# sThalham/PyraPose

Hardware: AMD Instinct MI355X
Metric: images/sec 640x480 fwd+bwd (train step: fwd + losses + bwd + clipnorm-Adam) (higher is better)
Workload: dtype bf16x3+f16c8

## Files before the change

include/pyrapose_hip.h:

```cpp
#ifndef PYRAPOSE_HIP_H
#define PYRAPOSE_HIP_H

#include <stddef.h>
#include <stdint.h>

#ifdef __cplusplus
extern "C" {
#endif

#define PP_OK 0
#define PP_ERR_ARG (-1)
#define PP_ERR_SHAPE (-2)
#define PP_ERR_ALIGN (-3)
#define PP_ERR_NOCTX (-4)
#define PP_ERR_UNSUPPORTED (-5)
#define PP_ERR_COMM (-6)

#define PP_MAX_SEG 5

typedef struct pp_ctx pp_ctx;

int pp_ctx_create(pp_ctx** out, int device, void* hip_stream);
void pp_ctx_destroy(pp_ctx* ctx);
int pp_ctx_set_stream(pp_ctx* ctx, void* hip_stream);
int pp_ctx_set_workspace(pp_ctx* ctx, void* device_buffer, size_t bytes);
int pp_row_block_list(pp_ctx* ctx, const float* x, int rows, int ld, int cols, unsigned char* flags, int* list);
int pp_row_block_list_planes(pp_ctx* ctx, const void* x_hi, const void* x_lo, int rows, int ld, int cols, unsigned char* flags, int* list);
int pp_row_block_list_planes_within(pp_ctx* ctx, const void* x_hi, const void* x_lo, int rows, int ld, int cols, const unsigned char* within,
                                    unsigned char* flags, int* list);
const char* pp_last_error_string(pp_ctx* ctx);
const char* pp_version(void);
int pp_device_info(pp_ctx* ctx, int* n_cu, char* name_host, int name_len);

typedef struct {
  int n_img;
  int n_seg;
  int h[PP_MAX_SEG];
  int w[PP_MAX_SEG];
} pp_rowspace;

typedef struct {
  pp_rowspace in;
  pp_rowspace out;
  int cin, cout;
  int kh, kw, stride;
  int pad_t, pad_l;
  int ld_x, ld_y, ld_w;
} pp_conv_desc;

int pp_conv2d_nhwc_fwd(pp_ctx* ctx, const pp_conv_desc* d, const float* x, const float* w,
                       const float* bias, const float* residual, int ld_res, int relu, float* y);

int pp_conv2d_nhwc_bwd_data(pp_ctx* ctx, const pp_conv_desc* d, const float* dy, const float* w,
                            const float* addend, int ld_add, const float* relu_src, int ld_rs, float* dx);

int pp_conv2d_nhwc_bwd_weight(pp_ctx* ctx, const pp_conv_desc* d, const float* x, const float* dy,
                              float* dw, float* dbias);

int pp_conv_split_weights_bf16x3(pp_ctx* ctx, const pp_conv_desc* d, const float* w, void* fwd_hi, void* fwd_lo,
                                 void* dgrad_hi, void* dgrad_lo);
typedef struct pp_split_job {
  const float* w;
  void* fwd_hi; void* fwd_lo; void* dg_hi; void* dg_lo;
  int taps, cin, cout, ld_w;
  int tile_begin, reserved;
} pp_split_job;
int pp_conv_split_weights_bf16x3_batch(pp_ctx* ctx, int n_jobs, const pp_split_job* jobs_dev, int total_tiles);
int pp_positive_row_blocks(pp_ctx* ctx, const pp_rowspace* rs, int A, int stride, const float* y_true, unsigned char* flags);
int pp_row_block_dilate(pp_ctx* ctx, const pp_conv_desc* d, const unsigned char* in_flags, unsigned char* out_flags);
int pp_split_planes_bf16x3(pp_ctx* ctx, size_t n, const float* src, void* hi, void* lo);
int pp_ctx_set_planes_format(pp_ctx* ctx, int fmt);
int pp_convert_planes(pp_ctx* ctx, size_t n, const void* src_hi, const void* src_lo, int src_fmt, void* dst_hi, void* dst_lo, int dst_fmt,
                      const float* scale2_dev, int scale_index, const void* relu_src_hi);
int pp_grad_scale_from_counts(pp_ctx* ctx, const int* counts_dev, int n_counts, float* scale2_dev);
int pp_grad_scale_from_counts_adj(pp_ctx* ctx, const int* counts_dev, int n_counts, float* scale2_dev, int log2_adjust);
int pp_split_planes_scaled_bf16x3(pp_ctx* ctx, size_t n, const float* src, void* hi, void* lo, const float* scale_dev);
int pp_ctx_set_grad_scale(pp_ctx* ctx, const float* scale2_dev);

typedef struct pp_conv_opts {
  void* capture_hi;
  void* capture_lo;
  const void* add_hi;
  const void* add_lo;
  const void* mask_hi;
  unsigned char* skip_flags;
  int* skip_list;
  const unsigned char* out_flags;
  int* out_list;
  int lazy_out;
  int lazy_in;
} pp_conv_opts;
#ifdef __cplusplus
static_assert(sizeof(pp_conv_opts) == 9 * sizeof(void*) + 2 * sizeof(int), "pp_conv_opts: pointers, then ints, no padding");
#else
_Static_assert(sizeof(pp_conv_opts) == 9 * sizeof(void*) + 2 * sizeof(int), "pp_conv_opts: pointers, then ints, no padding");
#endif

int pp_conv2d_nhwc_fwd_bf16x3(pp_ctx* ctx, const pp_conv_desc* d, const float* x, const void* x_hi, const void* x_lo,
                              const void* w_fwd_hi, const void* w_fwd_lo, const float* bias, const float* residual,
                              int ld_res, int relu, float* y, void* y_hi, void* y_lo, const pp_conv_opts* opts);
int pp_conv2d_nhwc_bwd_data_bf16x3(pp_ctx* ctx, const pp_conv_desc* d, const float* dy, const void* dy_hi,
                                   const void* dy_lo, const void* w_dgrad_hi, const void* w_dgrad_lo,
                                   const float* addend, int ld_add, const float* relu_src, int ld_rs, float* dx,
                                   void* dx_hi, void* dx_lo, const pp_conv_opts* opts);
int pp_conv2d_nhwc_bwd_weight_bf16x3(pp_ctx* ctx, const pp_conv_desc* d, const float* x, const float* dy,
                                     const void* x_hi, const void* x_lo, const void* dy_hi, const void* dy_lo,
                                     float* dw, float* dbias, const pp_conv_opts* opts);

typedef struct pp_comm pp_comm;
int pp_comm_available(void);
int pp_comm_unique_id(pp_ctx* ctx, void* id128);
int pp_comm_init(pp_ctx* ctx, int world, int rank, const void* id128, pp_comm** out);
int pp_comm_destroy(pp_comm* comm);
int pp_allreduce_bucket(pp_ctx* ctx, pp_comm* comm, float* buf, size_t count);
int pp_allreduce_counts(pp_ctx* ctx, pp_comm* comm, int* counts, int n);

int pp_maxpool3x3s2_fwd(pp_ctx* ctx, int n_img, int h, int w, int c, const float* x, int oh, int ow, float* y);
int pp_upsample_nearest_add_fwd(pp_ctx* ctx, int n_img, int sh, int sw, int th, int tw, int c,
                                const float* src, const float* other, float* out);
int pp_upsample_nearest_add_bwd(pp_ctx* ctx, int n_img, int sh, int sw, int th, int tw, int c,
                                const float* dtarget, const float* base, float* dsrc);
int pp_add_n(pp_ctx* ctx, size_t n, const float* a, const float* b, const float* c, float* out);
int pp_relu_fwd(pp_ctx* ctx, size_t n, const float* x, float* y);
typedef struct pp_tview {
  const float* f32;
  const void* hi;
  const void* lo;
} pp_tview;
int pp_add_n_v(pp_ctx* ctx, size_t n, const pp_tview* a, const pp_tview* b, const pp_tview* c, const pp_tview* out);
int pp_relu_fwd_v(pp_ctx* ctx, size_t n, const pp_tview* x, const pp_tview* y);
int pp_upsample_nearest_add_fwd_v(pp_ctx* ctx, int n_img, int sh, int sw, int th, int tw, int c, const pp_tview* src,
                                  const pp_tview* other, const pp_tview* out);
int pp_upsample_nearest_add_bwd_v(pp_ctx* ctx, int n_img, int sh, int sw, int th, int tw, int c, const pp_tview* dtarget,
                                  const pp_tview* base, const pp_tview* dsrc);
int pp_merge_planes_bf16x3(pp_ctx* ctx, size_t n, const void* hi, const void* lo, float* dst);
int pp_planes_stats(pp_ctx* ctx, const void* hi, const void* lo, long long rows, int ld, int cols, const unsigned char* within,
                    unsigned long long* stats5_dev);
int pp_pack_rgb_to_4(pp_ctx* ctx, size_t n_pixels, const float* x3, float* x4);
int pp_preprocess_caffe_u8(pp_ctx* ctx, int n_img, int H, int W, const int* sizes_hw_host, const unsigned char* images_u8,
                           float* x4);
int pp_warp_affine_u8(pp_ctx* ctx, int n_img, int H, int W, int channels, const double* mats_host, int interpolation, int border,
                      int cval, const unsigned char* src, unsigned char* dst);
int pp_resize_scale(int rows, int cols, int min_side, int max_side, double* scale);
int pp_resize_linear_u8(pp_ctx* ctx, int n_img, int SH, int SW, int channels, double scale, int DH, int DW, const unsigned char* src,
                        unsigned char* dst);
enum { PP_PHOTO_NONE = 0, PP_PHOTO_LUT = 1, PP_PHOTO_GRAY = 2, PP_PHOTO_HUESAT = 3, PP_PHOTO_BLEND = 4, PP_PHOTO_CONV = 5, PP_PHOTO_MEDIAN = 6,
       PP_PHOTO_BILATERAL = 7 };
typedef struct pp_photo_op {
  int kind;
  int k;
  int off0, off1;
  float f0, f1;
} pp_photo_op;
size_t pp_photo_workspace_bytes(int n_img, int H, int W);
int pp_photo_augment_u8(pp_ctx* ctx, int n_img, int H, int W, int channels, const int* op_offsets_host, const pp_photo_op* ops_host,
                        const unsigned char* pool_host, size_t pool_bytes, const unsigned char* pool_dev, const unsigned char* src,
                        unsigned char* dst, void* workspace, size_t workspace_bytes);
int pp_pack_rgb_to_4_padded(pp_ctx* ctx, int n_img, int H, int W, int Hp, int Wp, int pad, const float* x3, float* x4p);
int pp_preprocess_caffe_u8_padded(pp_ctx* ctx, int n_img, int H, int W, int Hp, int Wp, int pad, const int* sizes_hw_host,
                                  const unsigned char* images_u8, float* x4p);
int pp_stem7x7s2_fwd_bf16x3(pp_ctx* ctx, int n_img, int H, int W, int Hp, int Wp, const float* x4p, const void* w_hi,
                            const void* w_lo, int cout, const float* bias, int relu, float* y, int ld_y);

int pp_export_head(pp_ctx* ctx, const pp_rowspace* rs, int n_anchor, int n_val, const float* src, int ld,
                   int apply_sigmoid, float* out);

int pp_count_positives(pp_ctx* ctx, size_t rows_box, const float* y_box, size_t rows_cls, int c_cls,
                       const float* y_cls, size_t rows_mask, int c_mask, const float* y_mask, int* counts);
int pp_sigmoid_focal_fwd_bwd(pp_ctx* ctx, const pp_rowspace* rs, int n_anchor, int n_class,
                             const float* logits, int ld, const float* y_true, float alpha, float gamma,
                             const int* count, float loss_weight, float* loss_sum, float* dlogits);
int pp_orth_smoothl1_fwd_bwd(pp_ctx* ctx, const pp_rowspace* rs, int n_anchor, const float* pred, int ld,
                             const float* y_true, float weight, float sigma, const int* count,
                             float loss_weight, float* loss_sum, float* dpred);

typedef struct {
  long long offset;
  long long count;
// ... 118 lines not shown
```

pyrapose_amd/_lib.py:

```python
import ctypes as C
import os

_HERE = os.path.dirname(os.path.abspath(__file__))
LIB_PATH = os.path.join(_HERE, os.environ.get("PP_LIB") or "libpyrapose_hip.so")

PP_MAX_SEG = 5


class RowSpace(C.Structure):
    _fields_ = [("n_img", C.c_int), ("n_seg", C.c_int), ("h", C.c_int * PP_MAX_SEG), ("w", C.c_int * PP_MAX_SEG)]

    @classmethod
    def make(cls, n_img, shapes):
        rs = cls()
        rs.n_img = int(n_img)
        rs.n_seg = len(shapes)
        for i, (h, w) in enumerate(shapes):
            rs.h[i] = int(h)
            rs.w[i] = int(w)
        return rs

    def rows(self):
        return sum(self.n_img * self.h[i] * self.w[i] for i in range(self.n_seg))

    def shapes(self):
        return [(self.h[i], self.w[i]) for i in range(self.n_seg)]


class ConvDesc(C.Structure):
    _fields_ = [("in_", RowSpace), ("out", RowSpace), ("cin", C.c_int), ("cout", C.c_int), ("kh", C.c_int),
                ("kw", C.c_int), ("stride", C.c_int), ("pad_t", C.c_int), ("pad_l", C.c_int), ("ld_x", C.c_int),
                ("ld_y", C.c_int), ("ld_w", C.c_int)]


class ParamDesc(C.Structure):
    _fields_ = [("offset", C.c_longlong), ("count", C.c_longlong), ("ld", C.c_int), ("trainable", C.c_int),
                ("scale_off", C.c_longlong), ("l2", C.c_float)]


class SplitJob(C.Structure):
    _fields_ = [("w", C.c_void_p), ("fwd_hi", C.c_void_p), ("fwd_lo", C.c_void_p), ("dg_hi", C.c_void_p), ("dg_lo", C.c_void_p),
                ("taps", C.c_int), ("cin", C.c_int), ("cout", C.c_int), ("ld_w", C.c_int), ("tile_begin", C.c_int), ("reserved", C.c_int)]


class TView(C.Structure):
    _fields_ = [("f32", C.c_void_p), ("hi", C.c_void_p), ("lo", C.c_void_p)]


class ConvOpts(C.Structure):
    _fields_ = [("capture_hi", C.c_void_p), ("capture_lo", C.c_void_p), ("add_hi", C.c_void_p), ("add_lo", C.c_void_p),
                ("mask_hi", C.c_void_p), ("skip_flags", C.c_void_p), ("skip_list", C.c_void_p), ("out_flags", C.c_void_p),
                ("out_list", C.c_void_p), ("lazy_out", C.c_int), ("lazy_in", C.c_int)]


def _load():
    if not os.path.exists(LIB_PATH):
        raise ImportError(
            "pyrapose_amd: %s not found. Build it with `python -c 'import __graft_entry__ as g; g.build()'` "
            "or `make -C pyrapose_amd/csrc`. There is no CPU fallback." % LIB_PATH)
    try:
        return C.CDLL(LIB_PATH)
    except OSError as e:
        raise ImportError("pyrapose_amd: cannot load %s: %s" % (LIB_PATH, e))


lib = _load()
if hasattr(lib, "pp_ctx_set_split_capture"):
    raise ImportError("pyrapose_amd: %s predates pp_conv_opts (it still exports pp_ctx_set_split_capture): rebuild it" % LIB_PATH)

_p = C.c_void_p
_i = C.c_int
_f = C.c_float
_d = C.c_double
_ll = C.c_longlong
_sz = C.c_size_t

_SIGS = {
    "pp_ctx_create": (_i, [C.POINTER(_p), _i, _p]),
    "pp_ctx_destroy": (None, [_p]),
    "pp_ctx_set_stream": (_i, [_p, _p]),
    "pp_last_error_string": (C.c_char_p, [_p]),
    "pp_version": (C.c_char_p, []),
    "pp_device_info": (_i, [_p, C.POINTER(_i), C.c_char_p, _i]),
    "pp_conv2d_nhwc_fwd": (_i, [_p, C.POINTER(ConvDesc), _p, _p, _p, _p, _i, _i, _p]),
    "pp_conv2d_nhwc_bwd_data": (_i, [_p, C.POINTER(ConvDesc), _p, _p, _p, _i, _p, _i, _p]),
    "pp_conv2d_nhwc_bwd_weight": (_i, [_p, C.POINTER(ConvDesc), _p, _p, _p, _p]),
    "pp_conv_split_weights_bf16x3": (_i, [_p, C.POINTER(ConvDesc), _p, _p, _p, _p, _p]),
    "pp_split_planes_bf16x3": (_i, [_p, _sz, _p, _p, _p]),
    "pp_ctx_set_planes_format": (_i, [_p, _i]),
    "pp_convert_planes": (_i, [_p, _sz, _p, _p, _i, _p, _p, _i, _p, _i, _p]),
    "pp_split_planes_scaled_bf16x3": (_i, [_p, _sz, _p, _p, _p, _p]),
    "pp_grad_scale_from_counts": (_i, [_p, _p, _i, _p]),
    "pp_grad_scale_from_counts_adj": (_i, [_p, _p, _i, _p, _i]),
    "pp_ctx_set_grad_scale": (_i, [_p, _p]),
    "pp_planes_stats": (_i, [_p, _p, _p, _ll, _i, _i, _p, _p]),
    "pp_comm_available": (_i, []),
    "pp_comm_unique_id": (_i, [_p, _p]),
    "pp_comm_init": (_i, [_p, _i, _i, _p, C.POINTER(_p)]),
    "pp_comm_destroy": (_i, [_p]),
    "pp_allreduce_bucket": (_i, [_p, _p, _p, C.c_size_t]),
    "pp_allreduce_counts": (_i, [_p, _p, _p, _i]),
    "pp_ctx_set_workspace": (_i, [_p, _p, C.c_size_t]),
    "pp_row_block_list": (_i, [_p, _p, _i, _i, _i, _p, _p]),
    "pp_positive_row_blocks": (_i, [_p, _p, _i, _i, _p, _p]),
    "pp_row_block_dilate": (_i, [_p, _p, _p, _p]),
    "pp_row_block_list_planes": (_i, [_p, _p, _p, _i, _i, _i, _p, _p]),
    "pp_row_block_list_planes_within": (_i, [_p, _p, _p, _i, _i, _i, _p, _p, _p]),
    "pp_add_n_v": (_i, [_p, _sz, C.POINTER(TView), C.POINTER(TView), C.POINTER(TView), C.POINTER(TView)]),
    "pp_relu_fwd_v": (_i, [_p, _sz, C.POINTER(TView), C.POINTER(TView)]),
    "pp_upsample_nearest_add_fwd_v": (_i, [_p, _i, _i, _i, _i, _i, _i, C.POINTER(TView), C.POINTER(TView), C.POINTER(TView)]),
    "pp_upsample_nearest_add_bwd_v": (_i, [_p, _i, _i, _i, _i, _i, _i, C.POINTER(TView), C.POINTER(TView), C.POINTER(TView)]),
    "pp_merge_planes_bf16x3": (_i, [_p, _sz, _p, _p, _p]),
    "pp_warp_affine_u8": (_i, [_p, _i, _i, _i, _i, C.POINTER(_d), _i, _i, _i, _p, _p]),
    "pp_photo_workspace_bytes": (_sz, [_i, _i, _i]),
    "pp_photo_augment_u8": (_i, [_p, _i, _i, _i, _i, _p, _p, _p, _sz, _p, _p, _p, _p, _sz]),
    "pp_resize_scale": (_i, [_i, _i, _i, _i, C.POINTER(_d)]),
    "pp_resize_linear_u8": (_i, [_p, _i, _i, _i, _i, _d, _i, _i, _p, _p]),
    "pp_conv_split_weights_bf16x3_batch": (_i, [_p, _i, _p, _i]),
    "pp_conv2d_nhwc_fwd_bf16x3": (_i, [_p, C.POINTER(ConvDesc), _p, _p, _p, _p, _p, _p, _p, _i, _i, _p, _p, _p, C.POINTER(ConvOpts)]),
    "pp_conv2d_nhwc_bwd_data_bf16x3": (_i, [_p, C.POINTER(ConvDesc), _p, _p, _p, _p, _p, _p, _i, _p, _i, _p, _p, _p, C.POINTER(ConvOpts)]),
    "pp_conv2d_nhwc_bwd_weight_bf16x3": (_i, [_p, C.POINTER(ConvDesc), _p, _p, _p, _p, _p, _p, _p, _p, C.POINTER(ConvOpts)]),
    "pp_maxpool3x3s2_fwd": (_i, [_p, _i, _i, _i, _i, _p, _i, _i, _p]),
    "pp_upsample_nearest_add_fwd": (_i, [_p, _i, _i, _i, _i, _i, _i, _p, _p, _p]),
    "pp_upsample_nearest_add_bwd": (_i, [_p, _i, _i, _i, _i, _i, _i, _p, _p, _p]),
    "pp_add_n": (_i, [_p, _sz, _p, _p, _p, _p]),
    "pp_relu_fwd": (_i, [_p, C.c_size_t, _p, _p]),
    "pp_preprocess_caffe_u8": (_i, [_p, _i, _i, _i, C.POINTER(C.c_int), _p, _p]),
    "pp_preprocess_caffe_u8_padded": (_i, [_p, _i, _i, _i, _i, _i, _i, C.POINTER(C.c_int), _p, _p]),
    "pp_pack_rgb_to_4_padded": (_i, [_p, _i, _i, _i, _i, _i, _i, _p, _p]),
    "pp_stem7x7s2_fwd_bf16x3": (_i, [_p, _i, _i, _i, _i, _i, _p, _p, _p, _i, _p, _i, _p, _i]),
    "pp_pack_rgb_to_4": (_i, [_p, _sz, _p, _p]),
    "pp_export_head": (_i, [_p, C.POINTER(RowSpace), _i, _i, _p, _i, _i, _p]),
    "pp_count_positives": (_i, [_p, _sz, _p, _sz, _i, _p, _sz, _i, _p, _p]),
    "pp_sigmoid_focal_fwd_bwd": (_i, [_p, C.POINTER(RowSpace), _i, _i, _p, _i, _p, _f, _f, _p, _f, _p, _p]),
    "pp_orth_smoothl1_fwd_bwd": (_i, [_p, C.POINTER(RowSpace), _i, _p, _i, _p, _f, _f, _p, _f, _p, _p]),
    "pp_optimizer_create": (_i, [_p, C.POINTER(_p), C.POINTER(ParamDesc), _i, _ll]),
    "pp_optimizer_destroy": (None, [_p]),
    "pp_grad_global_norm": (_i, [_p, _p, _p, _p, _p, _p, _p]),
    "pp_adam_step_clipnorm": (_i, [_p, _p, _p, _p, _p, _p, _p, _p, _p, _f, _f, _f, _f, _f, _ll]),
    "pp_generate_base_anchors_host": (_i, [_i, C.POINTER(_f), _i, C.POINTER(_f), _i, C.POINTER(_d)]),
    "pp_anchors_shift_f64": (_i, [_p, _i, C.POINTER(_i), C.POINTER(_i), C.POINTER(_i), _i, C.POINTER(_d), _p]),
    "pp_anchors_shift_f32": (_i, [_p, _i, C.POINTER(_i), C.POINTER(_i), C.POINTER(_i), _i, C.POINTER(_d), _p]),
    "pp_compute_overlap_f64": (_i, [_p, _i, _p, _i, _p, _p]),
    "pp_compute_gt_annotations": (_i, [_p, _i, _p, _i, _p, _d, _d, _p, _p]),
    "pp_anchor_targets": (_i, [_p, _i, _p, _i, C.POINTER(_i), _p, _p, _p, _p, _p, _i, _i, C.POINTER(_i), C.POINTER(_i), _i, _d, _d,
                               _i, _i, _p, _p, _p]),
    "pp_project_box3d_host": (_i, [C.POINTER(_d), C.POINTER(_d), C.POINTER(_d), C.POINTER(_d)]),
    "pp_pil_nearest_index_host": (_i, [_i, _i, C.POINTER(_i)]),
    "pp_box3d_decode": (_i, [_p, _i, _i, _p, _p, _p]),
    "pp_score_threshold_compact": (_i, [_p, _i, _i, _i, _p, _f, _i, _p, _p]),
    "pp_filter_workspace_bytes": (_sz, [_i, _i, _i]),
    "pp_pose_error_workspace_bytes": (_sz, [_i, _i]),
    "pp_filter_detections": (_i, [_p, _i, _i, _p, _p, _p, _f, _f, _i, _p, _p, _p, _p, _p]),
    "pp_pose_add_f64": (_i, [_p, _i, _i, _p, _p, _p, _p, _p, _p, _p]),
    "pp_pose_adi_f64": (_i, [_p, _i, _i, _p, _p, _p, _p, _p, _p, _p]),
    "pp_filter_detections_batch": (_i, [_p, _i, _i, _i, _p, _p, _p, _f, _f, _i, _p, _p, _p, _p, _p]),
    "pp_render_workspace_bytes": (_sz, [_i, _i, _i, _i, _i]),
    "pp_render_depth_f32": (_i, [_p, _i, _i, _p, _i, _p, _p, _p, _p, _i, _i, _d, _d, _p, _sz, _p]),
    "pp_vsd_workspace_bytes": (_sz, [_i, _i, _i]),
    "pp_vsd_f64": (_i, [_p, _i, _i, _i, _p, _ll, _p, _p, _p, _d, _d, _i, _p, _p, _p, _p]),
    "pp_pose_reproj_f64": (_i, [_p, _i, _i, _p, _p, _p, _p, _p, _p, _p, _p]),
    "pp_pnp_ransac_workspace_bytes": (_sz, [_i, _i]),
    "pp_pnp_ransac_f64": (_i, [_p, _i, _p, _i, _p, _p, _p, _i, _d, C.c_ulonglong, _i, _p, _p, _p, _p, _p, _p]),
    "pp_cloud_from_depth_workspace_bytes": (_sz, [_i, _i]),
    "pp_cloud_from_depth_f64": (_i, [_p, _i, _i, _p, _p, _i, _i, _p, _p, _d, _d, _d, _d, _d, _i, _p, _p, _p]),
    "pp_voxel_workspace_bytes": (_sz, [_i]),
    "pp_voxel_keys_f64": (_i, [_p, _i, _p, _d, _p, _p]),
    "pp_voxel_means_f64": (_i, [_p, _i, _p, _p, _p, _i, _p, _p, _p]),
    "pp_estimate_normals_workspace_bytes": (_sz, [_i, _i]),
    "pp_estimate_normals_f64": (_i, [_p, _i, _p, _d, _i, _p, _p, _p]),
    "pp_icp_workspace_bytes": (_sz, [_i, _i]),
    "pp_icp_f64": (_i, [_p, _i, _p, _p, _i, _p, _p, _p, _p, _d, _i, _d, _d, _i, _p, _sz, _p, _p, _p, _p, _p, _p, _p]),
    "pp_vote_stats_workspace_bytes": (_sz, [_i, _i]),
    "pp_vote_stats_f64": (_i, [_p, _i, _p, _i, _p, _i, _p, _p, _i, _d, _p, _p, _p, _p, _p, _p, _p]),
    "pp_pnp_refine_weighted_workspace_bytes": (_sz, [_i, _i]),
    "pp_pnp_refine_weighted_f64": (_i, [_p, _i, _p, _i, _p, _p, _p, _p, _p, _p, _i, _d, _d, _d, _p, _p, _p, _p, _p, _p, _p, _p, _p]),
}

EXPORTS = sorted(_SIGS)

MISSING = []
for _name, (_res, _args) in _SIGS.items():
    try:
        _fn = getattr(lib, _name)
    except AttributeError:
        if not os.environ.get("PP_LIB"):
            raise
        MISSING.append(_name)
        continue
    _fn.restype = _res
    _fn.argtypes = _args


def check(rc, ctx=None, what=""):
    if rc == 0:
        return
    msg = ""
    if ctx is not None:
        s = lib.pp_last_error_string(ctx)
        msg = s.decode("utf-8", "replace") if s else ""
    if rc < 0:
        raise ValueError("%s failed (%d): %s" % (what or "pyrapose_hip", rc, msg))
    raise RuntimeError("%s failed (hipError %d): %s" % (what or "pyrapose_hip", rc, msg))
```

pyrapose_amd/csrc/conv3.hip:

```cpp
#include "conv_common.h"
#include "conv4.h"

#define PP_CAT_(a, b) a##b
#define PP_CAT(a, b) PP_CAT_(a, b)
#if PP_FMT == 1
#define PP_API(name) PP_CAT(name, _fmt1)
#else
#define PP_API(name) PP_CAT(name, _fmt0)
#endif
namespace {
#include "planes_fmt.h"

#include "conv3_shared.h"

#ifndef PP_EPI_GF
#define PP_EPI_GF 4
#endif

template <int TM, int TN, bool AP, bool OP>
__global__ __launch_bounds__(256, (TM * TN >= 8) ? 2 : ((TM * TN == 4) ? 3 : 4)) void igemm3_kernel(
    const IgemmParams p, const float* __restrict__ g_src, const uint4* __restrict__ g_ahi, const uint4* __restrict__ g_alo,
    const uint4* __restrict__ g_whi, const uint4* __restrict__ g_wlo,
    const float* __restrict__ g_bias, const float* __restrict__ g_addend, const float* __restrict__ g_mask,
    float* __restrict__ g_out, uint2* __restrict__ g_ohi, uint2* __restrict__ g_olo, int w_rows, int w_ld8) {
  constexpr int BM = 64 * TM, BN = 64 * TN, BK = 32, NO = BK / 8;
  constexpr int SMEM_U4 = 2 * NO * (BM + BN);
  __shared__ __attribute__((aligned(16))) uint4 smem[SMEM_U4];
  uint4* Ahi = smem;
  uint4* Alo = Ahi + NO * BM;
  uint4* Bhi = Alo + NO * BM;
  uint4* Blo = Bhi + NO * BN;

  const int tid = threadIdx.x, lane = tid & 63, wave = tid >> 6;
  const int wm = wave >> 1, wn = wave & 1;
  const int lb = xcd_remap((int)blockIdx.x, (int)gridDim.x);
  const int tile_n = lb % p.n_tiles_n, tile_m = lb / p.n_tiles_n;
  const int m0 = tile_m * BM, n0 = tile_n * BN;

  const int oct = tid & 3, r0 = tid >> 2;
  RowPos rows[TM];
#pragma unroll
  for (int i = 0; i < TM; ++i) rows[i] = decode_row(p, m0 + r0 + 64 * i);
  long long a_off[TM];
  bool a_ok[TM];

  const int n_taps = p.kh * p.kw;
  const int n_steps = n_taps * (p.Cred / BK);

  float4 ra[TM][2];
  uint4 rah[TM], ral[TM];
  uint4 rbh[TN], rbl[TN];
  int tap = 0, ty = 0, tx = 0, red0 = 0;

  auto set_tap = [&]() {
#pragma unroll
    for (int i = 0; i < TM; ++i) a_ok[i] = tap_offset(p, rows[i], ty, tx, &a_off[i]);
  };
  auto load_step = [&]() {
#pragma unroll
    for (int i = 0; i < TM; ++i) {
      if (AP) {
        if (a_ok[i]) {
          const long long o8 = 2 * (((a_off[i] + red0) >> 3) + oct);
          rah[i] = g_ahi[o8];
          ral[i] = g_alo[o8];
        } else {
          rah[i] = make_uint4(0u, 0u, 0u, 0u);
          ral[i] = make_uint4(0u, 0u, 0u, 0u);
        }
      } else if (a_ok[i]) {
        const float4* s4 = reinterpret_cast<const float4*>(g_src + a_off[i] + red0 + 8 * oct);
        ra[i][0] = s4[0];
        ra[i][1] = s4[1];
      } else {
        ra[i][0] = make_float4(0.f, 0.f, 0.f, 0.f);
        ra[i][1] = make_float4(0.f, 0.f, 0.f, 0.f);
      }
    }
#pragma unroll
    for (int i = 0; i < TN; ++i) {
      const int n = n0 + r0 + 64 * i;
      if (n < w_rows) {
        const long long off = ((long long)tap * w_rows + n) * w_ld8 + (red0 >> 3) + oct;
        rbh[i] = g_whi[off];
        rbl[i] = g_wlo[off];
      } else {
        rbh[i] = make_uint4(0u, 0u, 0u, 0u);
        rbl[i] = make_uint4(0u, 0u, 0u, 0u);
      }
    }
  };
  auto advance = [&]() {
    red0 += BK;
    if (red0 >= p.Cred) {
      red0 = 0;
      ++tap;
      ++tx;
      if (tx == p.kw) { tx = 0; ++ty; }
      set_tap();
    }
  };
  auto store_step = [&]() {
#pragma unroll
    for (int i = 0; i < TM; ++i) {
      uint4 hi, lo;
      if (AP) {
        hi = rah[i];
        lo = ral[i];
      } else {
        split8(ra[i][0], ra[i][1], &hi, &lo);
      }
      const int slot = oct * BM + ((r0 + 64 * i + 2 * oct) & (BM - 1));
      Ahi[slot] = hi;
      Alo[slot] = lo;
    }
#pragma unroll
    for (int i = 0; i < TN; ++i) {
      const int slot = oct * BN + ((r0 + 64 * i + 2 * oct) & (BN - 1));
      Bhi[slot] = rbh[i];
      Blo[slot] = rbl[i];
    }
  };

  floatx16 acc[TM][TN];
#pragma unroll
  for (int a = 0; a < TM; ++a)
#pragma unroll
    for (int b = 0; b < TN; ++b)
#pragma unroll
      for (int r = 0; r < 16; ++r) acc[a][b][r] = 0.f;

  const int il = lane & 31, h = lane >> 5;

  set_tap();
  load_step();
  store_step();
  __syncthreads();

  for (int step = 0; step < n_steps; ++step) {
    const bool more = step + 1 < n_steps;
    if (more) {
      advance();
      load_step();
    }
    mma_step<TM, TN, BM, BN, 0>(acc, Ahi, Alo, Bhi, Blo, wm * 32 * TM + il, wn * 32 * TN + il, h);
    __syncthreads();
    if (more) {
      store_step();
      __syncthreads();
    }
  }

  epilogue3<TM, TN, OP>(p, acc, smem, m0, n0, tid, wm, wn, il, h, g_bias, g_addend, g_mask, g_out, g_ohi, g_olo);
}

template <int TM, int TN, bool AP, bool OP, bool SC = false, bool RL = false>
__global__ __launch_bounds__(256, (TM * TN >= 8) ? 2 : ((TM * TN == 4) ? 3 : 4)) void igemm3f_kernel(
    const IgemmParams p, const void* __restrict__ g_a0, const void* __restrict__ g_a1, unsigned a_bytes,
    const void* __restrict__ g_whi, const void* __restrict__ g_wlo, unsigned w_bytes,
    const float* __restrict__ g_bias, const float* __restrict__ g_addend, const float* __restrict__ g_mask,
    float* __restrict__ g_out, uint2* __restrict__ g_ohi, uint2* __restrict__ g_olo, int w_rows, int w_ld8, int splits,
    float* __restrict__ g_ws, const int* __restrict__ g_rl = nullptr, const unsigned char* __restrict__ g_srcflags = nullptr) {
  constexpr int BM = 64 * TM, BN = 64 * TN, BK = 32, NO = BK / 8;
  constexpr int SMEM_U4 = 2 * NO * (BM + BN);
  constexpr int ES = 4;
  __shared__ __attribute__((aligned(16))) uint4 smem[SMEM_U4];
  uint4* Ahi = smem;
  uint4* Alo = Ahi + NO * BM;
  uint4* Bhi = Alo + NO * BM;
  uint4* Blo = Bhi + NO * BN;

  const int tid = threadIdx.x, lane = tid & 63, wave = tid >> 6;
  const int wm = wave >> 1, wn = wave & 1;
  int n_wg = (int)gridDim.x;
  if (RL) {
    n_wg = ((g_rl[0] + BM / 32 - 1) / (BM / 32)) * p.n_tiles_n * splits;
    if ((int)blockIdx.x >= n_wg) return;
  }
  const int lbs = xcd_remap((int)blockIdx.x, n_wg);
  const int split = lbs % splits, lb = lbs / splits;
  const int tile_n = lb % p.n_tiles_n, tile_m = lb / p.n_tiles_n;
  const int m0 = tile_m * BM, n0 = tile_n * BN;
  int rl_blk[BM / 32];
  if (RL) {
    const int count = g_rl[0];
#pragma unroll
    for (int j = 0; j < BM / 32; ++j) {
      const int e = tile_m * (BM / 32) + j;
      rl_blk[j] = e < count ? g_rl[1 + e] * 32 : ((p.M + 31) & ~31);
    }
  }
  const int oct = tid & 3, r0 = tid >> 2;
  const int n_taps = p.kh * p.kw;
  const int steps_per_tap = p.Cred / BK;
  const int all_steps = n_taps * steps_per_tap;
  const int s_begin = (int)((long long)all_steps * split / splits), s_end = (int)((long long)all_steps * (split + 1) / splits);

  const __amdgpu_buffer_rsrc_t rs_a0 = __builtin_amdgcn_make_buffer_rsrc(const_cast<void*>(g_a0), 0, a_bytes, 0x00020000);
  const __amdgpu_buffer_rsrc_t rs_a1 = __builtin_amdgcn_make_buffer_rsrc(const_cast<void*>(AP ? g_a1 : g_a0), 0, AP ? a_bytes - 16 : a_bytes, 0x00020000);
  const __amdgpu_buffer_rsrc_t rs_wh = __builtin_amdgcn_make_buffer_rsrc(const_cast<void*>(g_whi), 0, w_bytes, 0x00020000);
  const __amdgpu_buffer_rsrc_t rs_wl = __builtin_amdgcn_make_buffer_rsrc(const_cast<void*>(g_wlo), 0, w_bytes, 0x00020000);

  int a_base[TM], a_pitch[TM];
  unsigned a_valid[TM];
#pragma unroll
  for (int i = 0; i < TM; ++i) {
    const int t_row = r0 + 64 * i;
    const RowPos r = decode_row(p, RL ? rl_blk[t_row >> 5] + (t_row & 31) : m0 + t_row);
    a_base[i] = ((r.rowbase + r.ybase * r.SW + r.xbase) * p.ld_src + 8 * oct) * ES;
    a_pitch[i] = p.tsign * r.SW * p.ld_src * ES;
    unsigned v = 0;
    int t = 0;
    for (int ty = 0; ty < p.kh; ++ty)
      for (int tx = 0; tx < p.kw; ++tx, ++t) {
        const int sy = r.ybase + ty * p.tsign, sx = r.xbase + tx * p.tsign;
        bool ok = r.ok && (unsigned)sy < (unsigned)r.SH && (unsigned)sx < (unsigned)r.SW;
        if (RL && g_srcflags && ok) ok = g_srcflags[(r.rowbase + sy * r.SW + sx) >> 5] != 0;
        if (ok) v |= 1u << t;
      }
    a_valid[i] = v;
  }
  const int x_pitch = p.tsign * p.ld_src * ES;
  int b_base[TN];
#pragma unroll
  for (int i = 0; i < TN; ++i) {
    const int n = n0 + r0 + 64 * i;
    b_base[i] = n < w_rows ? (n * w_ld8 + oct) * 16 : PP_BUF_OOB;
  }
  const int b_tap = w_rows * w_ld8 * 16;

  float4 ra[TM][2];
  uint4 rah[TM], ral[TM];
  uint4 rbh[TN], rbl[TN];
  int tap = s_begin / steps_per_tap, red0 = (s_begin - tap * steps_per_tap) * BK;
  int ty = tap / p.kw, tx = tap - ty * p.kw;

  auto load_step = [&]() {
    const int a_uni = tx * x_pitch + red0 * ES;
#pragma unroll
    for (int i = 0; i < TM; ++i) {
      int vo = a_base[i] + __mul24(ty, a_pitch[i]) + a_uni;
      vo = ((a_valid[i] >> tap) & 1u) ? vo : PP_BUF_OOB;
      if (AP) {
        rah[i] = buf_load16(rs_a0, vo, 0);
        ral[i] = buf_load16(rs_a1, vo, 0);
      } else {
        const uint4 q0 = buf_load16(rs_a0, vo, 0), q1 = buf_load16(rs_a0, vo + 16, 0);
        ra[i][0] = *reinterpret_cast<const float4*>(&q0);
        ra[i][1] = *reinterpret_cast<const float4*>(&q1);
      }
    }
    const int b_uni = ((p.w_ty0 + p.w_tstep * ty) * p.w_kw + p.w_tx0 + p.w_tstep * tx) * b_tap + (red0 >> 3) * 16;
#pragma unroll
    for (int i = 0; i < TN; ++i) {
      rbh[i] = buf_load16(rs_wh, b_base[i], b_uni);
      rbl[i] = buf_load16(rs_wl, b_base[i], b_uni);
    }
  };
  auto advance = [&](bool more) {
    red0 += BK;
    const bool wrap = red0 >= p.Cred;
    red0 = wrap ? 0 : red0;
    tap += wrap ? 1 : 0;
    tx += wrap ? 1 : 0;
    const bool wx = tx == p.kw;
    tx = wx ? 0 : tx;
    ty += wx ? 1 : 0;
    red0 = more ? red0 : 0;
    tap = more ? tap : 0;
    tx = more ? tx : 0;
    ty = more ? ty : 0;
  };
  auto split_step = [&]() {
    if (!AP) {
#pragma unroll
      for (int i = 0; i < TM; ++i) split8(ra[i][0], ra[i][1], &rah[i], &ral[i]);
    }
  };
  auto store_step = [&]() {
#pragma unroll
    for (int i = 0; i < TM; ++i) {
      const int slot = oct * BM + ((r0 + 64 * i + 2 * oct) & (BM - 1));
      Ahi[slot] = rah[i];
      Alo[slot] = ral[i];
    }
#pragma unroll
    for (int i = 0; i < TN; ++i) {
      const int slot = oct * BN + ((r0 + 64 * i + 2 * oct) & (BN - 1));
      Bhi[slot] = rbh[i];
      Blo[slot] = rbl[i];
    }
  };

  floatx16 acc[TM][TN];
#pragma unroll
  for (int a = 0; a < TM; ++a)
#pragma unroll
    for (int b = 0; b < TN; ++b)
#pragma unroll
      for (int r = 0; r < 16; ++r) acc[a][b][r] = 0.f;

  const int il = lane & 31, h = lane >> 5;

  load_step();
  split_step();
  store_step();
  __syncthreads();

  for (int step = s_begin; step < s_end; ++step) {
    advance(step + 1 < s_end);
    load_step();
    __builtin_amdgcn_sched_barrier(0);
    mma_step<TM, TN, BM, BN, 2>(acc, Ahi, Alo, Bhi, Blo, wm * 32 * TM + il, wn * 32 * TN + il, h);
    split_step();
    __syncthreads();
    store_step();
    __syncthreads();
  }
  if (splits > 1) {
    float* slice = g_ws + (long long)split * (RL ? (((long long)p.M + 31) & ~31ll) : (long long)p.M) * p.ld_out;
#pragma unroll
    for (int a = 0; a < TM; ++a)
#pragma unroll
      for (int r = 0; r < 16; ++r) {
        const int trow = wm * 32 * TM + a * 32 + (r & 3) + 8 * (r >> 2) + 4 * h;
        const int m = m0 + trow;
        const bool row_ok = RL ? (rl_blk[trow >> 5] < p.M) : (m < p.M);
#pragma unroll
        for (int b = 0; b < TN; ++b) {
          const int co = n0 + wn * 32 * TN + b * 32 + il;
          if (row_ok && co < ((p.Nout + 3) & ~3)) slice[(long long)m * p.ld_out + co] = acc[a][b][r];
        }
      }
    return;
  }
  epilogue3<TM, TN, OP, PP_EPI_GF, SC, false, RL>(p, acc, smem, m0, n0, tid, wm, wn, il, h, g_bias, g_addend, g_mask, g_out, g_ohi, g_olo, rl_blk);
}

template <int TM, int TN, bool CAP, bool AP = false, bool OP = false>
__global__ __launch_bounds__(256, (TM * TN >= 8) ? 2 : ((TM * TN == 4) ? 3 : 4)) void igemm3x_kernel(
    const IgemmParams p, const void* __restrict__ g_a, const void* __restrict__ g_a1, unsigned a_bytes, const void* __restrict__ g_whi,
    const void* __restrict__ g_wlo, unsigned w_bytes, const float* __restrict__ g_bias, const float* __restrict__ g_addend,
    const float* __restrict__ g_mask, float* __restrict__ g_out, uint2* __restrict__ g_ohi, uint2* __restrict__ g_olo, int w_rows, int w_ld8,
    int splits, float* __restrict__ g_ws, void* __restrict__ g_chi, void* __restrict__ g_clo, const unsigned char* __restrict__ g_flags,
    int skip_halo) {
  static_assert(!(CAP && AP), "split capture is for f32 operands");
  constexpr int ES = 4;
  constexpr int BM = 64 * TM, BN = 64 * TN, BK = 32, NO = BK / 8;
  constexpr int AP1 = NO * BM + 1;
  constexpr int SMEM_U4 = 2 * AP1 + 2 * NO * BN;
  __shared__ __attribute__((aligned(16))) uint4 smem[SMEM_U4];
  uint4* Ahi = smem;
  uint4* Alo = Ahi + AP1;
  uint4* Bhi = Alo + AP1;
  uint4* Blo = Bhi + NO * BN;

  const int tid = threadIdx.x, lane = tid & 63, wave = tid >> 6;
  const int wm = wave >> 1, wn = wave & 1;
  const int lbs = xcd_remap((int)blockIdx.x, (int)gridDim.x);
  const int split = lbs % splits, lb = lbs / splits;
  const int tile_n = lb % p.n_tiles_n, tile_m = lb / p.n_tiles_n;
  const int m0 = p.m_off + tile_m * (BM - 2) - 1, n0 = tile_n * BN;
  const int oct = tid & 3, r0 = tid >> 2;
  const int il = lane & 31, h = lane >> 5;
  const int n_chunks = p.Cred / BK;
  const int all_groups = p.kh * n_chunks;
  const int g_begin = (int)((long long)all_groups * split / splits);
  int g_end = (int)((long long)all_groups * (split + 1) / splits);
  if (g_flags) {
    int lo = m0 - skip_halo, hi = m0 + BM - 1 + skip_halo;
    lo = lo < 0 ? 0 : lo;
    hi = hi > p.M - 1 ? p.M - 1 : hi;
    int any = 0;
    for (int b = lo >> 5; b <= (hi >> 5); ++b) any |= g_flags[b];
    g_end = any ? g_end : g_begin;
  }

  const __amdgpu_buffer_rsrc_t rs_a = __builtin_amdgcn_make_buffer_rsrc(const_cast<void*>(g_a), 0, a_bytes, 0x00020000);
  const __amdgpu_buffer_rsrc_t rs_a1 = __builtin_amdgcn_make_buffer_rsrc(const_cast<void*>(AP ? g_a1 : g_a), 0, AP ? a_bytes - 16 : a_bytes, 0x00020000);
  const __amdgpu_buffer_rsrc_t rs_wh = __builtin_amdgcn_make_buffer_rsrc(const_cast<void*>(g_whi), 0, w_bytes, 0x00020000);
  const __amdgpu_buffer_rsrc_t rs_wl = __builtin_amdgcn_make_buffer_rsrc(const_cast<void*>(g_wlo), 0, w_bytes, 0x00020000);

  int s_base[TM], s_pitch[TM];
#pragma unroll
  for (int i = 0; i < TM; ++i) {
    const int q = m0 + r0 + 64 * i;
    const RowPos r = decode_row(p, q < 0 ? 0 : q);
    const bool ok = q >= 0 && r.ok;
    const int x = r.xbase - p.off_x;
    s_base[i] = ((r.rowbase + r.ybase * r.SW + x) * p.ld_src + 8 * oct) * ES;
    int v = 0;
    for (int ty = 0; ty < p.kh; ++ty)
      if (ok && (unsigned)(r.ybase + ty * p.tsign) < (unsigned)r.SH) v |= 1 << ty;
    s_pitch[i] = (p.tsign * r.SW * p.ld_src * ES) | v;
  }
  unsigned f_valid[(TM + 1) / 2];
#pragma unroll
  for (int a = 0; a < (TM + 1) / 2; ++a) f_valid[a] = 0;
#pragma unroll
  for (int a = 0; a < TM; ++a) {
    const int q = m0 + wm * 32 * TM + a * 32 + il;
    const RowPos r = decode_row(p, q < 0 ? 0 : q);
    unsigned v = 0;
    int t = 0;
    for (int ty = 0; ty < p.kh; ++ty)
      for (int tx = 0; tx < 3; ++tx, ++t) {
        const int sy = r.ybase + ty * p.tsign, sx = r.xbase + tx * p.tsign;
        if (q >= 0 && r.ok && (unsigned)sy < (unsigned)r.SH && (unsigned)sx < (unsigned)r.SW) v |= 1u << t;
      }
    f_valid[a >> 1] |= v << (16 * (a & 1));
  }
  int b_base[TN];
#pragma unroll
  for (int i = 0; i < TN; ++i) {
    const int n = n0 + r0 + 64 * i;
    b_base[i] = n < w_rows ? (n * w_ld8 + oct) * 16 : PP_BUF_OOB;
  }
  const int b_tap = w_rows * w_ld8 * 16;

  float4 ra[TM][2];
  uint4 rah[TM], ral[TM];
  uint4 rbh[TN], rbl[TN];
  const bool ty_inner = p.x_ty_inner != 0;
  int ty = ty_inner ? g_begin % p.kh : g_begin / n_chunks;
  int chunk = ty_inner ? g_begin / p.kh : g_begin - ty * n_chunks;

  auto load_a = [&]() {
#pragma unroll
    for (int i = 0; i < TM; ++i) {
      int vo = s_base[i] + __mul24(ty, s_pitch[i] & ~15) + chunk * (BK * ES);
      vo = ((s_pitch[i] >> ty) & 1) ? vo : PP_BUF_OOB;
      if (AP) {
        rah[i] = buf_load16(rs_a, vo, 0);
        ral[i] = buf_load16(rs_a1, vo, 0);
      } else {
        const uint4 q0 = buf_load16(rs_a, vo, 0), q1 = buf_load16(rs_a, vo + 16, 0);
        ra[i][0] = *reinterpret_cast<const float4*>(&q0);
        ra[i][1] = *reinterpret_cast<const float4*>(&q1);
      }
    }
  };
  auto load_b = [&](int tx) {
    const int b_uni = ((p.w_ty0 + ty) * p.w_kw + tx) * b_tap + chunk * (BK / 8 * 16);
#pragma unroll
    for (int i = 0; i < TN; ++i) {
      rbh[i] = buf_load16(rs_wh, b_base[i], b_uni);
      rbl[i] = buf_load16(rs_wl, b_base[i], b_uni);
    }
  };
  auto split_a = [&]() {
    if (!AP) {
#pragma unroll
      for (int i = 0; i < TM; ++i) split8(ra[i][0], ra[i][1], &rah[i], &ral[i]);
    }
  };
  auto store_a = [&]() {
#pragma unroll
    for (int i = 0; i < TM; ++i) {
      const int slot = oct * BM + ((r0 + 64 * i + 2 * oct) & (BM - 1));
      Ahi[slot] = rah[i];
      Alo[slot] = ral[i];
    }
  };
  const int ty_c = -p.off_y * p.tsign;
  auto capture = [&]() {
    if constexpr (CAP) {
      const __amdgpu_buffer_rsrc_t rs_ch = __builtin_amdgcn_make_buffer_rsrc(g_chi, 0, a_bytes, 0x00020000);
      const __amdgpu_buffer_rsrc_t rs_cl = __builtin_amdgcn_make_buffer_rsrc(g_clo, 0, a_bytes - 16, 0x00020000);
      if (ty == ty_c && chunk % p.n_tiles_n == tile_n) {
#pragma unroll
        for (int i = 0; i < TM; ++i) {
          const int row = r0 + 64 * i;
          const int vo = s_base[i] + __mul24(ty, s_pitch[i] & ~15) + chunk * (BK * 4);
          const bool ok = ((s_pitch[i] >> ty) & 1) && row >= 1 && row <= BM - 2;
          const int co = ok ? vo : PP_BUF_OOB;
          buf_store16(rs_ch, rah[i], co);
          buf_store16(rs_cl, ral[i], co);
        }
      }
    }
  };
  auto store_b = [&]() {
#pragma unroll
    for (int i = 0; i < TN; ++i) {
      const int slot = oct * BN + ((r0 + 64 * i + 2 * oct) & (BN - 1));
      Bhi[slot] = rbh[i];
      Blo[slot] = rbl[i];
    }
  };

  floatx16 acc[TM][TN];
#pragma unroll
  for (int a = 0; a < TM; ++a)
#pragma unroll
    for (int b = 0; b < TN; ++b)
#pragma unroll
      for (int r = 0; r < 16; ++r) acc[a][b][r] = 0.f;

  auto mma_tile = [&](int c_ty, auto tx_c) {
    constexpr int TX = decltype(tx_c)::value;
    const int dx = p.off_x + TX * p.tsign;
    const unsigned tap_bits = (1u << (c_ty * 3 + TX)) * 0x10001u;
    unsigned okm[(TM + 1) / 2];
#pragma unroll
    for (int a = 0; a < (TM + 1) / 2; ++a) okm[a] = f_valid[a] & tap_bits;
    unsigned a_ok = 0;
#pragma unroll
    for (int a = 0; a < TM; ++a) a_ok |= (((okm[a >> 1] >> (16 * (a & 1))) & 0xffffu) != 0 ? 1u : 0u) << a;
    mma_step<TM, TN, BM, BN, 1>(acc, Ahi, Alo, Bhi, Blo, wm * 32 * TM + il + dx, wn * 32 * TN + il, h, a_ok, NO * BM);
  };

  std::integral_constant<int, 0> t0;
  std::integral_constant<int, 1> t1;
  std::integral_constant<int, 2> t2;
  if (threadIdx.x == 0) {
    Ahi[NO * BM] = make_uint4(0u, 0u, 0u, 0u);
    Alo[NO * BM] = make_uint4(0u, 0u, 0u, 0u);
  }
  load_a();
  load_b(0);
  split_a();
  store_a();
  store_b();
  __syncthreads();
  for (int g = g_begin; g < g_end; ++g) {
    const int c_ty = ty;
    capture();
    load_b(1);
    __builtin_amdgcn_sched_barrier(0);
    mma_tile(c_ty, t0);
    __syncthreads();
    store_b();
    __syncthreads();
    load_b(2);
    __builtin_amdgcn_sched_barrier(0);
    mma_tile(c_ty, t1);
    __syncthreads();
    store_b();
    __syncthreads();
    {
      const bool more = g + 1 < g_end;
      if (ty_inner) {
        ty += 1;
        const bool wt = ty == p.kh;
        ty = wt ? 0 : ty;
        chunk += wt ? 1 : 0;
      } else {
        chunk += 1;
        const bool wc = chunk == n_chunks;
        chunk = wc ? 0 : chunk;
        ty += wc ? 1 : 0;
      }
      chunk = more ? chunk : 0;
      ty = more ? ty : 0;
    }
    load_b(0);
    load_a();
    __builtin_amdgcn_sched_barrier(0);
    mma_tile(c_ty, t2);
    split_a();
    __syncthreads();
    store_b();
    store_a();
    __syncthreads();
  }
  if (splits > 1) {
    float* slice = g_ws + (long long)split * (p.M - p.m_off) * p.ld_out;
#pragma unroll
    for (int a = 0; a < TM; ++a)
#pragma unroll
      for (int r = 0; r < 16; ++r) {
        const int row = wm * 32 * TM + a * 32 + (r & 3) + 8 * (r >> 2) + 4 * h;
        const int m = m0 + row;
#pragma unroll
        for (int b = 0; b < TN; ++b) {
          const int co = n0 + wn * 32 * TN + b * 32 + il;
          if (row >= 1 && row <= BM - 2 && m < p.M && co < ((p.Nout + 3) & ~3)) slice[(long long)(m - p.m_off) * p.ld_out + co] = acc[a][b][r];
        }
      }
    return;
  }
  epilogue3<TM, TN, OP, 4, false, true>(p, acc, smem, m0, n0, tid, wm, wn, il, h, g_bias, g_addend, g_mask, g_out, g_ohi, g_olo);
}

template <bool OP, int VAR = 0, int NWM = 4>
__global__ __launch_bounds__(128 * NWM, NWM == 4 ? 1 : 2) void igemm4x_kernel(
    const IgemmParams p, const void* __restrict__ g_a, const void* __restrict__ g_a1, unsigned a_bytes, const void* __restrict__ g_whi,
    const void* __restrict__ g_wlo, unsigned w_bytes, const float* __restrict__ g_bias, const float* __restrict__ g_addend,
    const float* __restrict__ g_mask, float* __restrict__ g_out, uint2* __restrict__ g_ohi, uint2* __restrict__ g_olo, int w_rows, int w_ld8) {
  constexpr int TM = 2, TN = 2, NW = 2 * NWM, BM = 32 * TM * NWM, BN = 128, BK = 32, NO = BK / 8, ES = 4;
  constexpr int BST = NWM == 4 ? 3 : 2;
  constexpr int BI = 128 / (16 * NW);
  constexpr int A_STAGE = 8 * BM + 2, B_STAGE = 2 * NO * BN;
  __shared__ __attribute__((aligned(16))) uint4 sA0[A_STAGE];
  __shared__ __attribute__((aligned(16))) uint4 sA1[A_STAGE];
  __shared__ __attribute__((aligned(16))) uint4 sB0[B_STAGE];
  __shared__ __attribute__((aligned(16))) uint4 sB1[B_STAGE];
  __shared__ __attribute__((aligned(16))) uint4 sB2[BST == 3 ? B_STAGE : 1];
  auto stA = [&](auto k) -> uint4* {
    if constexpr (decltype(k)::value == 0) return sA0; else return sA1;
  };
  auto stB = [&](auto k) -> uint4* {
    if constexpr (decltype(k)::value == 0) return sB0; else return sB1;
  };

  const int tid = threadIdx.x, lane = tid & 63, wave = __builtin_amdgcn_readfirstlane(tid >> 6);
  const int wm = wave >> 1, wn = wave & 1;
  const int lb = xcd_remap((int)blockIdx.x, (int)gridDim.x);
  const int tile_n = lb % p.n_tiles_n, tile_m = lb / p.n_tiles_n;
  const int m0 = tile_m * (BM - 2) - 1, n0 = tile_n * BN;
  const int il = lane & 31, h = lane >> 5;
  const int n_chunks = p.Cred / BK;
  const int G = p.kh * n_chunks;

  const __amdgpu_buffer_rsrc_t rs_a = __builtin_amdgcn_make_buffer_rsrc(const_cast<void*>(g_a), 0, a_bytes, 0x00020000);
  (void)g_a1;
  const __amdgpu_buffer_rsrc_t rs_wh = __builtin_amdgcn_make_buffer_rsrc(const_cast<void*>(g_whi), 0, w_bytes, 0x00020000);
  const __amdgpu_buffer_rsrc_t rs_wl = __builtin_amdgcn_make_buffer_rsrc(const_cast<void*>(g_wlo), 0, w_bytes, 0x00020000);

  int s_base[4], s_pitch[4];
#pragma unroll
  for (int c = 0; c < 4; ++c) {
    const int j = 32 * wave + 8 * c + (lane >> 3);
    const int piece = (lane & 7) ^ ((j >> 1) & 7);
    const int q = m0 + j;
    const RowPos r = decode_row(p, q < 0 ? 0 : q);
    const bool ok = q >= 0 && r.ok;
    const int x = r.xbase - p.off_x;
    s_base[c] = (r.rowbase + r.ybase * r.SW + x) * p.ld_src * ES + 16 * piece;
    int v = 0;
    for (int ty = 0; ty < 3; ++ty)
      if (ok && (unsigned)(r.ybase + ty * p.tsign) < (unsigned)r.SH) v |= 1 << ty;
    s_pitch[c] = (p.tsign * r.SW * p.ld_src * ES) | v;
  }
  int b_dma[BI];
#pragma unroll
  for (int i = 0; i < BI; ++i) {
    const int b_row = 16 * (BI * wave + i) + (lane >> 2);
    const int b_n = n0 + b_row;
    b_dma[i] = b_n < w_rows ? (b_n * w_ld8 + ((lane & 3) ^ ((b_row >> 2) & 3))) * 16 : PP_BUF_OOB;
  }
  const int b_tap = w_rows * w_ld8 * 16;

  unsigned f_valid = 0;
#pragma unroll
  for (int a = 0; a < TM; ++a) {
    const int q = m0 + wm * 32 * TM + a * 32 + il;
    const RowPos r = decode_row(p, q < 0 ? 0 : q);
    unsigned v = 0;
    int t = 0;
    for (int ty = 0; ty < 3; ++ty)
      for (int tx = 0; tx < 3; ++tx, ++t) {
        const int sy = r.ybase + ty * p.tsign, sx = r.xbase + tx * p.tsign;
        if (q >= 0 && r.ok && (unsigned)sy < (unsigned)r.SH && (unsigned)sx < (unsigned)r.SW) v |= 1u << t;
      }
    f_valid |= v << (16 * (a & 1));
  }

  auto dma_a = [&](int g, uint4* st) {
    const int ty = g % 3, chunk = g / 3;
    uint4* const dst = st + 8 * 32 * wave;
#pragma unroll
    for (int c = 0; c < 4; ++c) {
      int vo = s_base[c] + __mul24(ty, s_pitch[c] & ~15) + chunk * (BK * ES);
      vo = ((s_pitch[c] >> ty) & 1) ? vo : PP_BUF_OOB;
      dma16(rs_a, dst + 64 * c, vo, 0);
    }
  };
  auto dma_b = [&](int g, int tx, uint4* st) {
    const int ty = g % 3, chunk = g / 3;
    const int b_uni = ((p.w_ty0 + ty) * p.w_kw + tx) * b_tap + chunk * (BK / 8 * 16);
#pragma unroll
    for (int i = 0; i < BI; ++i) {
      uint4* const hi = st + 4 * 16 * (BI * wave + i);
      dma16(rs_wh, hi, b_dma[i], b_uni);
      dma16(rs_wl, hi + NO * BN, b_dma[i], b_uni);
    }
  };

  floatx16 acc[TM][TN];
#pragma unroll
  for (int a = 0; a < TM; ++a)
#pragma unroll
    for (int b = 0; b < TN; ++b)
#pragma unroll
      for (int r = 0; r < 16; ++r) acc[a][b][r] = 0.f;

  auto mma_tile = [&](int c_ty, int TX, const uint4* Ahi, const uint4* Bhi) {
    const int dx = p.off_x + TX * p.tsign;
    const unsigned tap_bits = (1u << (c_ty * 3 + TX)) * 0x10001u;
    const unsigned okm = f_valid & tap_bits;
    unsigned a_ok = 0;
#pragma unroll
    for (int a = 0; a < TM; ++a) a_ok |= (((okm >> (16 * (a & 1))) & 0xffffu) != 0 ? 1u : 0u) << a;
    if (VAR & 2) __builtin_amdgcn_s_setprio(1);
    mma_step<TM, TN, BM, BN, (VAR & 4) ? 2 : ((VAR & 1) ? 0 : 1), 1>(acc, Ahi, Ahi, Bhi, Bhi + NO * BN, wm * 32 * TM + il + dx, wn * 32 * TN + il, h, a_ok, 8 * BM);
    if (VAR & 2) __builtin_amdgcn_s_setprio(0);
  };
  std::integral_constant<int, 0> c0;
  std::integral_constant<int, 1> c1;
  auto tap_end = [&](auto n) {
    constexpr int N = decltype(n)::value;
    if constexpr (N == 0) asm volatile("s_waitcnt vmcnt(0)" ::: "memory");
    else if constexpr (N == 2) asm volatile("s_waitcnt vmcnt(2)" ::: "memory");
    else if constexpr (N == 4) asm volatile("s_waitcnt vmcnt(4)" ::: "memory");
    else if constexpr (N == 6) asm volatile("s_waitcnt vmcnt(6)" ::: "memory");
    else static_assert(N == 0, "tap_end: count");
    __builtin_amdgcn_s_barrier();
    asm volatile("" ::: "memory");
  };
  auto group = [&](int g, auto k) {
    constexpr int K = decltype(k)::value;
    const int c_ty = g % 3;
    const int gn = g + 1 < G ? g + 1 : 0;
    uint4* const Ahi = stA(std::integral_constant<int, K & 1>{});
    if constexpr (BST == 3) {
      dma_a(gn, stA(std::integral_constant<int, (K + 1) & 1>{}));
      dma_b(g, 2, sB2);
      mma_tile(c_ty, 0, Ahi, sB0);
      tap_end(std::integral_constant<int, 6>{});
      dma_b(gn, 0, sB0);
      mma_tile(c_ty, 1, Ahi, sB1);
      tap_end(std::integral_constant<int, 2>{});
      dma_b(gn, 1, sB1);
      mma_tile(c_ty, 2, Ahi, sB2);
      tap_end(std::integral_constant<int, 2>{});
    } else {
      constexpr int U = 3 * K;
      dma_b(g, 1, stB(std::integral_constant<int, (U + 1) & 1>{}));
      dma_a(gn, stA(std::integral_constant<int, (K + 1) & 1>{}));
      mma_tile(c_ty, 0, Ahi, stB(std::integral_constant<int, U & 1>{}));
      tap_end(std::integral_constant<int, 4>{});
      dma_b(g, 2, stB(std::integral_constant<int, U & 1>{}));
      mma_tile(c_ty, 1, Ahi, stB(std::integral_constant<int, (U + 1) & 1>{}));
      tap_end(std::integral_constant<int, 0>{});
      dma_b(gn, 0, stB(std::integral_constant<int, (U + 1) & 1>{}));
      mma_tile(c_ty, 2, Ahi, stB(std::integral_constant<int, U & 1>{}));
      tap_end(std::integral_constant<int, 0>{});
    }
  };

  if (tid == 0) {
    sA0[8 * BM] = make_uint4(0u, 0u, 0u, 0u);
    sA0[8 * BM + 1] = make_uint4(0u, 0u, 0u, 0u);
    sA1[8 * BM] = make_uint4(0u, 0u, 0u, 0u);
    sA1[8 * BM + 1] = make_uint4(0u, 0u, 0u, 0u);
  }
  if ((VAR & 8) && NWM == 4 && wave >= 4) __builtin_amdgcn_s_setprio(1);
  dma_a(0, sA0);
  dma_b(0, 0, sB0);
  if constexpr (BST == 3) {
    dma_b(0, 1, sB1);
    tap_end(std::integral_constant<int, 2>{});
  } else {
    tap_end(std::integral_constant<int, 0>{});
  }
  for (int g = 0; g < G; g += 2) {
    group(g, c0);
    if (g + 1 >= G) break;
    group(g + 1, c1);
  }
  asm volatile("s_waitcnt vmcnt(0)" ::: "memory");
  __syncthreads();
  epilogue3<TM, TN, OP, 4, false, true, false, NWM, 128 * NWM, (NWM == 2 ? 1 : 0)>(p, acc, sA0, m0, n0, tid, wm, wn, il, h, g_bias, g_addend, g_mask, g_out, g_ohi, g_olo);
}

__device__ __forceinline__ void finish4(const IgemmParams& p, float4 v, long long mo, int co, bool with_addend, const float* __restrict__ g_addend,
                                        const float* __restrict__ g_mask, float* __restrict__ g_out, void* __restrict__ g_ohi,
                                        void* __restrict__ g_olo) {
  if (with_addend) {
    if (p.add_hi) {
      const float4 a = planes_ld4(p.add_hi, p.add_lo, (mo * p.ld_add + co) >> 2);
      v.x += a.x; v.y += a.y; v.z += a.z; v.w += a.w;
    } else if (g_addend) {
      const float4 a = *reinterpret_cast<const float4*>(g_addend + mo * p.ld_add + co);
      v.x += a.x; v.y += a.y; v.z += a.z; v.w += a.w;
    }
  }
  if (p.mask_hi || g_mask) {
    const float4 k = p.mask_hi ? hi_ld4(p.mask_hi, (mo * p.ld_mask + co) >> 2) : *reinterpret_cast<const float4*>(g_mask + mo * p.ld_mask + co);
    v.x = k.x > 0.f ? v.x : 0.f; v.y = k.y > 0.f ? v.y : 0.f; v.z = k.z > 0.f ? v.z : 0.f; v.w = k.w > 0.f ? v.w : 0.f;
  }
  if (p.relu) { v.x = fmaxf(v.x, 0.f); v.y = fmaxf(v.y, 0.f); v.z = fmaxf(v.z, 0.f); v.w = fmaxf(v.w, 0.f); }
  if (g_out) *reinterpret_cast<float4*>(g_out + mo * p.ld_out + co) = v;
  if (g_ohi) planes_st4(g_ohi, g_olo, (mo * p.ld_out + co) >> 2, v);
}

__global__ void class_fill_kernel(const IgemmParams p, const float* __restrict__ g_addend, const float* __restrict__ g_mask,
                                  float* __restrict__ g_out, void* __restrict__ g_ohi, void* __restrict__ g_olo) {
  const int n4 = (p.Nout + 3) >> 2;
  const long long total = (long long)p.M * n4;
  const int hw = p.seg[0].OH * p.seg[0].OW;
  for (long long i = blockIdx.x * (long long)blockDim.x + threadIdx.x; i < total; i += (long long)gridDim.x * blockDim.x) {
    const int m = (int)(i / n4), co = 4 * (int)(i - (long long)m * n4);
    const int n = m / hw, rem = m - n * hw, yq = rem / p.seg[0].OW, xq = rem - yq * p.seg[0].OW;
    const long long mo = (long long)(n * p.sc_H + 2 * yq + p.sc_cy) * p.sc_W + 2 * xq + p.sc_cx;
    finish4(p, make_float4(0.f, 0.f, 0.f, 0.f), mo, co, true, g_addend, g_mask, g_out, g_ohi, g_olo);
  }
}

__global__ void splitk_finish_kernel(const IgemmParams p, int splits, const float* __restrict__ ws, const float* __restrict__ g_bias,
                                     const float* __restrict__ g_addend, const float* __restrict__ g_mask, float* __restrict__ g_out,
                                     void* __restrict__ g_ohi, void* __restrict__ g_olo) {
  const int n4 = (p.Nout + 3) >> 2;
  const int rows = p.M - p.m_off;
  const long long total = (long long)rows * n4, slice = (long long)rows * p.ld_out;
  for (long long i = blockIdx.x * (long long)blockDim.x + threadIdx.x; i < total; i += (long long)gridDim.x * blockDim.x) {
    const int mr = (int)(i / n4), co = 4 * (int)(i - (long long)mr * n4);
    const int m = p.m_off + mr;
    const float* w = ws + (long long)mr * p.ld_out + co;
    float4 v = *reinterpret_cast<const float4*>(w);
    for (int s = 1; s < splits; ++s) {
      const float4 q = *reinterpret_cast<const float4*>(w + s * slice);
      v.x += q.x; v.y += q.y; v.z += q.z; v.w += q.w;
    }
    if (g_bias) { const float4 b = *reinterpret_cast<const float4*>(g_bias + co); v.x += b.x; v.y += b.y; v.z += b.z; v.w += b.w; }
    finish4(p, v, (long long)m, co, true, g_addend, g_mask, g_out, g_ohi, g_olo);
  }
}

__global__ void rl_splitk_finish_kernel(const IgemmParams p, int splits, const float* __restrict__ ws, const int* __restrict__ g_rl,
                                        const float* __restrict__ g_bias, const float* __restrict__ g_addend, const float* __restrict__ g_mask,
                                        float* __restrict__ g_out, void* __restrict__ g_ohi, void* __restrict__ g_olo) {
  const int j = blockIdx.x;
  if (j >= g_rl[0]) return;
  const int n4 = (p.Nout + 3) >> 2;
  const long long slice = (((long long)p.M + 31) & ~31ll) * p.ld_out;
  const int m0 = g_rl[1 + j] * 32, nr = min(32, p.M - m0);
  for (int i = threadIdx.x; i < nr * n4; i += blockDim.x) {
    const int r = i / n4, co = 4 * (i - r * n4);
    const float* w = ws + ((long long)j * 32 + r) * p.ld_out + co;
    float4 v = *reinterpret_cast<const float4*>(w);
    for (int s = 1; s < splits; ++s) {
      const float4 q = *reinterpret_cast<const float4*>(w + s * slice);
      v.x += q.x; v.y += q.y; v.z += q.z; v.w += q.w;
    }
    if (g_bias) { const float4 b = *reinterpret_cast<const float4*>(g_bias + co); v.x += b.x; v.y += b.y; v.z += b.z; v.w += b.w; }
    finish4(p, v, (long long)(m0 + r), co, true, g_addend, g_mask, g_out, g_ohi, g_olo);
  }
}

__global__ void split_planes_kernel(size_t n8, const float4* __restrict__ src, uint4* __restrict__ hi, uint4* __restrict__ lo,
                                    const float* __restrict__ scale) {
  const float sc = scale ? *scale : 1.f;
  for (size_t i = blockIdx.x * (size_t)blockDim.x + threadIdx.x; i < n8; i += (size_t)gridDim.x * blockDim.x) {
    uint4 h, l;
    float4 a = src[2 * i], b = src[2 * i + 1];
    a.x *= sc; a.y *= sc; a.z *= sc; a.w *= sc;
    b.x *= sc; b.y *= sc; b.z *= sc; b.w *= sc;
    split8(a, b, &h, &l);
    hi[2 * i] = h;
    lo[2 * i] = l;
  }
}

__global__ void grad_scale_kernel(const int* __restrict__ counts, int n_counts, float* __restrict__ scale2, int base_log2) {
  if (threadIdx.x == 0 && blockIdx.x == 0) {
    int n = 0x7fffffff;
    for (int i = 0; i < n_counts; ++i) n = counts[i] < n ? counts[i] : n;
    n = n < 1 ? 1 : n;
    int e = 0;
    while ((n >> (e + 1)) != 0) ++e;
    const float s = __uint_as_float((unsigned)(127 + base_log2 + e) << 23);
    scale2[0] = s;
    scale2[1] = 1.f / s;
  }
}

__global__ void row_block_flags_kernel(const float* __restrict__ x, int rows, int ld, int cols4, unsigned char* __restrict__ flags) {
  const int blk = blockIdx.x, r0 = blk * 32;
  const int nr = rows - r0 < 32 ? rows - r0 : 32;
  int any = 0;
  for (int i = threadIdx.x; i < nr * cols4; i += blockDim.x) {
    const int r = i / cols4, c = i - r * cols4;
    const float4 v = *reinterpret_cast<const float4*>(x + (long long)(r0 + r) * ld + 4 * c);
    any |= (v.x != 0.f) | (v.y != 0.f) | (v.z != 0.f) | (v.w != 0.f);
  }
  any = __syncthreads_or(any);
  if (threadIdx.x == 0) flags[blk] = any ? 1 : 0;
}

__global__ void row_block_flags_planes_kernel(const uint2* __restrict__ hi, const uint2* __restrict__ lo, int rows, int ld4, int cols4,
                                              unsigned char* __restrict__ flags, const unsigned char* __restrict__ within) {
  const int blk = blockIdx.x, r0 = blk * 32;
  if (within && !within[blk]) {
    if (threadIdx.x == 0) flags[blk] = 0;
    return;
  }
  const int nr = rows - r0 < 32 ? rows - r0 : 32;
  int any = 0;
  for (int i = threadIdx.x; i < nr * cols4; i += blockDim.x) {
    const int r = i / cols4, c = i - r * cols4;
    const long long o = pk4((long long)(r0 + r) * ld4 + c);
    const uint2 h = hi[o], l = lo[o];
    any |= fmt_any_nonzero(h.x | h.y, l.x | l.y) ? 1 : 0;
  }
  any = __syncthreads_or(any);
  if (threadIdx.x == 0) flags[blk] = any ? 1 : 0;
}

__global__ void row_block_compact_kernel(const unsigned char* __restrict__ flags, int n_blocks, int* __restrict__ list) {
  __shared__ int wave_cnt[4];
  __shared__ int base;
  const int tid = threadIdx.x, lane = tid & 63, wave = tid >> 6;
  if (tid == 0) base = 0;
  __syncthreads();
  for (int i0 = 0; i0 < n_blocks; i0 += 256) {
    const int i = i0 + tid;
    const bool f = i < n_blocks && flags[i] != 0;
    const unsigned long long m = __ballot(f);
    const int before = __popcll(m & ((1ull << lane) - 1ull));
    if (lane == 0) wave_cnt[wave] = __popcll(m);
    __syncthreads();
    int off = base;
    for (int w = 0; w < wave; ++w) off += wave_cnt[w];
    if (f) list[1 + off + before] = i;
    __syncthreads();
    if (tid == 0) base += wave_cnt[0] + wave_cnt[1] + wave_cnt[2] + wave_cnt[3];
    __syncthreads();
  }
  if (tid == 0) list[0] = base;
}

}
extern "C" int PP_API(pp_row_block_list)(pp_ctx* ctx, const float* x, int rows, int ld, int cols, unsigned char* flags, int* list) {
  PP_REQUIRE_CTX(ctx);
  PP_CHECK_ARG(ctx, x && flags && list && rows > 0 && cols > 0 && cols <= ld && ld % 4 == 0 && pp_is_aligned16(x), PP_ERR_ARG,
               "pp_row_block_list: bad tensor (ld %% 4 == 0, 16-byte aligned)");
  const int nb = (rows + 31) / 32, cols4 = (cols + 3) / 4;
  PP_CHECK_ARG(ctx, 4 * cols4 <= ld, PP_ERR_SHAPE, "pp_row_block_list: cols rounded up to 4 exceed ld");
  hipLaunchKernelGGL(row_block_flags_kernel, dim3((unsigned)nb), dim3(256), 0, ctx->stream, x, rows, ld, cols4, flags);
  hipLaunchKernelGGL(row_block_compact_kernel, dim3(1), dim3(256), 0, ctx->stream, (const unsigned char*)flags, nb, list);
  PP_CHECK_LAUNCH(ctx, "pp_row_block_list");
  return PP_OK;
}
namespace {

}
extern "C" int PP_API(pp_row_block_list_planes_within)(pp_ctx* ctx, const void* x_hi, const void* x_lo, int rows, int ld, int cols,
                                               const unsigned char* within, unsigned char* flags, int* list);
namespace {
}
extern "C" int PP_API(pp_row_block_list_planes)(pp_ctx* ctx, const void* x_hi, const void* x_lo, int rows, int ld, int cols, unsigned char* flags,
                                        int* list) {
  return PP_API(pp_row_block_list_planes_within)(ctx, x_hi, x_lo, rows, ld, cols, nullptr, flags, list);
}
namespace {

}
extern "C" int PP_API(pp_row_block_list_planes_within)(pp_ctx* ctx, const void* x_hi, const void* x_lo, int rows, int ld, int cols,
                                               const unsigned char* within, unsigned char* flags, int* list) {
  PP_REQUIRE_CTX(ctx);
  PP_CHECK_ARG(ctx, x_hi && x_lo && flags && list && rows > 0 && cols > 0 && cols <= ld && ld % 8 == 0 && pp_is_packed(x_hi, x_lo), PP_ERR_ARG,
               "pp_row_block_list_planes: bad tensor (ld %% 8 == 0, packed planes)");
  const int nb = (rows + 31) / 32, cols4 = (cols + 3) / 4;
  PP_CHECK_ARG(ctx, 4 * cols4 <= ld, PP_ERR_SHAPE, "pp_row_block_list_planes: cols rounded up to 4 exceed ld");
  hipLaunchKernelGGL(row_block_flags_planes_kernel, dim3((unsigned)nb), dim3(256), 0, ctx->stream, (const uint2*)x_hi, (const uint2*)x_lo, rows,
                     ld / 4, cols4, flags, within);
  hipLaunchKernelGGL(row_block_compact_kernel, dim3(1), dim3(256), 0, ctx->stream, (const unsigned char*)flags, nb, list);
  PP_CHECK_LAUNCH(ctx, "pp_row_block_list_planes");
  return PP_OK;
}
namespace {

static int split_planes_impl(pp_ctx* ctx, size_t n, const float* src, void* hi, void* lo, const float* scale);
}
extern "C" int PP_API(pp_split_planes_bf16x3)(pp_ctx* ctx, size_t n, const float* src, void* hi, void* lo) {
  return split_planes_impl(ctx, n, src, hi, lo, nullptr);
}
namespace {
}
extern "C" int PP_API(pp_split_planes_scaled_bf16x3)(pp_ctx* ctx, size_t n, const float* src, void* hi, void* lo, const float* scale_dev) {
  return split_planes_impl(ctx, n, src, hi, lo, scale_dev);
}
namespace {
}
extern "C" int PP_API(pp_grad_scale_from_counts_adj)(pp_ctx* ctx, const int* counts_dev, int n_counts, float* scale2_dev, int log2_adjust) {
  PP_REQUIRE_CTX(ctx);
  PP_CHECK_ARG(ctx, counts_dev && scale2_dev && n_counts >= 1 && n_counts <= 16 && log2_adjust >= -16 && log2_adjust <= 16, PP_ERR_ARG,
               "pp_grad_scale_from_counts: bad arguments");
  static const int base_log2 = []() { const char* e = getenv("PP_GSCALE_LOG2"); const int v = e ? atoi(e) : 8; return v < -20 ? -20 : (v > 30 ? 30 : v); }();
  hipLaunchKernelGGL(grad_scale_kernel, dim3(1), dim3(64), 0, ctx->stream, counts_dev, n_counts, scale2_dev, base_log2 + log2_adjust);
  PP_CHECK_LAUNCH(ctx, "pp_grad_scale_from_counts");
  return PP_OK;
}
extern "C" int PP_API(pp_grad_scale_from_counts)(pp_ctx* ctx, const int* counts_dev, int n_counts, float* scale2_dev) {
  return PP_API(pp_grad_scale_from_counts_adj)(ctx, counts_dev, n_counts, scale2_dev, 0);
}
namespace {
static int split_planes_impl(pp_ctx* ctx, size_t n, const float* src, void* hi, void* lo, const float* scale) {
  PP_REQUIRE_CTX(ctx);
  PP_CHECK_ARG(ctx, src && hi && lo && n % 8 == 0, PP_ERR_ARG, "pp_split_planes_bf16x3: n must be a multiple of 8");
  PP_CHECK_ARG(ctx, pp_is_aligned16(src) && pp_is_packed(hi, lo), PP_ERR_ALIGN, "pp_split_planes_bf16x3: alignment / packed planes (lo = hi + 16 bytes)");
  if (n == 0) return PP_OK;
  size_t blocks = (n / 8 + 255) / 256;
  const size_t cap = (size_t)(ctx->n_cu > 0 ? ctx->n_cu : 256) * 8;
  if (blocks > cap) blocks = cap;
  hipLaunchKernelGGL(split_planes_kernel, dim3((unsigned)blocks), dim3(256), 0, ctx->stream, n / 8, (const float4*)src, (uint4*)hi, (uint4*)lo, scale);
  PP_CHECK_LAUNCH(ctx, "pp_split_planes_bf16x3");
  return PP_OK;
}

__device__ __forceinline__ void split_weights_tile(int tap, int ci0, int co0, int cin, int cout, int ld_w, const float* __restrict__ w,
                                                   unsigned short* __restrict__ fwd_hi, unsigned short* __restrict__ fwd_lo, int cout_rows,
                                                   unsigned short* __restrict__ dg_hi, unsigned short* __restrict__ dg_lo, int dg_ld) {
  __shared__ unsigned short t_hi[32][33], t_lo[32][33];
  const int tx = threadIdx.x, ty = threadIdx.y;
  for (int j = ty; j < 32; j += 8) {
    const int ci = ci0 + j, co = co0 + tx;
    float v = 0.f;
    if (ci < cin && co < cout) v = w[((long long)tap * cin + ci) * ld_w + co];
    unsigned short uh, ul;
    fmt_encode_weight(v, &uh, &ul);
    t_hi[j][tx] = uh;
    t_lo[j][tx] = ul;
    if (dg_hi && ci < cin && co < dg_ld) {
      const long long o = ((long long)tap * cin + ci) * dg_ld + co;
      dg_hi[o] = uh;
      dg_lo[o] = ul;
    }
  }
  __syncthreads();
  if (fwd_hi) {
    for (int j = ty; j < 32; j += 8) {
      const int co = co0 + j, ci = ci0 + tx;
      if (co < cout_rows && ci < cin) {
        const long long o = ((long long)tap * cout_rows + co) * cin + ci;
        fwd_hi[o] = t_hi[tx][j];
        fwd_lo[o] = t_lo[tx][j];
      }
    }
  }
}

__global__ void split_weights_kernel(int taps, int cin, int cout, int ld_w, const float* __restrict__ w,
                                     unsigned short* __restrict__ fwd_hi, unsigned short* __restrict__ fwd_lo, int cout_rows,
                                     unsigned short* __restrict__ dg_hi, unsigned short* __restrict__ dg_lo, int dg_ld) {
  split_weights_tile(blockIdx.z, blockIdx.y * 32, blockIdx.x * 32, cin, cout, ld_w, w, fwd_hi, fwd_lo, cout_rows, dg_hi, dg_lo, dg_ld);
}

__global__ void split_weights_batch_kernel(int n_jobs, const pp_split_job* __restrict__ jobs) {
  int lo = 0, hi = n_jobs - 1;
  while (lo < hi) {
    const int mid = (lo + hi + 1) >> 1;
    if (jobs[mid].tile_begin <= (int)blockIdx.x) lo = mid; else hi = mid - 1;
  }
  const pp_split_job j = jobs[lo];
  const int dg_ld = (j.cout + 31) / 32 * 32;
  const int tiles_co = dg_ld / 32, tiles_ci = j.cin / 32;
  int t = (int)blockIdx.x - j.tile_begin;
  const int co_t = t % tiles_co;
  t /= tiles_co;
  const int ci_t = t % tiles_ci, tap = t / tiles_ci;
  split_weights_tile(tap, ci_t * 32, co_t * 32, j.cin, j.cout, j.ld_w, j.w, (unsigned short*)j.fwd_hi, (unsigned short*)j.fwd_lo, j.cout,
                     (unsigned short*)j.dg_hi, (unsigned short*)j.dg_lo, dg_ld);
}

}
extern "C" int PP_API(pp_conv_split_weights_bf16x3_batch)(pp_ctx* ctx, int n_jobs, const pp_split_job* jobs_dev, int total_tiles) {
  PP_REQUIRE_CTX(ctx);
  PP_CHECK_ARG(ctx, n_jobs >= 0 && total_tiles >= 0 && (n_jobs == 0 || jobs_dev), PP_ERR_ARG, "pp_conv_split_weights_bf16x3_batch: bad arguments");
  if (n_jobs == 0 || total_tiles == 0) return PP_OK;
  hipLaunchKernelGGL(split_weights_batch_kernel, dim3((unsigned)total_tiles), dim3(32, 8), 0, ctx->stream, n_jobs, jobs_dev);
  PP_CHECK_LAUNCH(ctx, "pp_conv_split_weights_bf16x3_batch");
  return PP_OK;
}
namespace {

}
extern "C" int PP_API(pp_conv_split_weights_bf16x3)(pp_ctx* ctx, const pp_conv_desc* d, const float* w, void* fwd_hi, void* fwd_lo,
                                            void* dg_hi, void* dg_lo) {
  PP_REQUIRE_CTX(ctx);
  int rc = check_desc(ctx, d, "pp_conv_split_weights_bf16x3");
  if (rc) return rc;
  PP_CHECK_ARG(ctx, w && ((fwd_hi && fwd_lo) || (dg_hi && dg_lo)), PP_ERR_ARG, "pp_conv_split_weights_bf16x3: null tensor");
  PP_CHECK_ARG(ctx, d->cin % 32 == 0, PP_ERR_SHAPE, "pp_conv_split_weights_bf16x3: cin %d must be a multiple of 32", d->cin);
  const int taps = d->kh * d->kw;
  const int dg_ld = (d->cout + 31) / 32 * 32;
  dim3 grid((unsigned)((dg_ld + 31) / 32), (unsigned)((d->cin + 31) / 32), (unsigned)taps);
  hipLaunchKernelGGL(split_weights_kernel, grid, dim3(32, 8), 0, ctx->stream, taps, d->cin, d->cout, d->ld_w, w,
                     (unsigned short*)fwd_hi, (unsigned short*)fwd_lo, d->cout, (unsigned short*)dg_hi, (unsigned short*)dg_lo, dg_ld);
  PP_CHECK_LAUNCH(ctx, "pp_conv_split_weights_bf16x3");
  return PP_OK;
}
namespace {

static bool igemm3_fast_ok(const IgemmParams& p, bool planes, int w_rows, int w_ld8) {
  static const bool fast_on = []() { const char* e = getenv("PP_CONV3_FAST"); return !(e && e[0] == '0'); }();
  const long long a_bytes = p.src_rows * (long long)p.ld_src * 4;
  (void)planes;
  const long long w_bytes = (long long)p.w_taps * w_rows * w_ld8 * 16;
  int max_sw = 0;
  for (int i = 0; i < p.n_seg; ++i) max_sw = p.seg[i].SW > max_sw ? p.seg[i].SW : max_sw;
  return fast_on && p.div == 1 && p.kh * p.kw <= 31 && a_bytes < (1ll << 31) && w_bytes < (1ll << 31) &&
         (long long)max_sw * p.ld_src * 4 < (1ll << 23) && p.src_rows > 0;
}

static bool igemm3x_ok(const IgemmParams& p, bool planes_in, bool planes_out, int w_rows, int w_ld8) {
  static const bool x_on = []() { const char* e = getenv("PP_CONV3_XREUSE"); return !(e && e[0] == '0'); }();
  bool same = x_on && igemm3_fast_ok(p, planes_in, w_rows, w_ld8) && !p.sc_on && p.kw == 3 && p.mul == 1 && p.div == 1 &&
              (p.src != nullptr || planes_in) && (!planes_in || p.ld_src % 8 == 0) && p.w_tstep == 1 && p.w_tx0 == 0;
  (void)planes_out;
  for (int i = 0; i < p.n_seg && same; ++i)
    same = p.seg[i].OH == p.seg[i].SH && p.seg[i].OW == p.seg[i].SW && p.seg[i].row_begin == p.seg[i].src_row_begin;
  return same;
}

__global__ void rl_dilate_kernel(const IgemmParams p, const unsigned char* __restrict__ in_flags, unsigned char* __restrict__ out_flags,
                                 int n_blocks) {
  const int b = blockIdx.x * blockDim.x + threadIdx.x;
  if (b >= n_blocks) return;
  const int r_lo = 32 * b, r_hi = min(32 * b + 31, p.M - 1);
  int any = 0;
  for (int s = 0; s < p.n_seg; ++s) {
    const int seg_lo = p.seg[s].row_begin, seg_hi = (s + 1 < p.n_seg ? p.seg[s + 1].row_begin : p.M) - 1;
    if (r_hi < seg_lo || r_lo > seg_hi) continue;
    const int W = p.seg[s].OW;
    for (int j = -1; j <= 1; ++j) {
      int lo = r_lo - 1 + j * W, hi = r_hi + 1 + j * W;
      lo = lo < 0 ? 0 : lo;
      hi = hi > p.M - 1 ? p.M - 1 : hi;
      for (int q = lo >> 5; q <= (hi >> 5); ++q) any |= in_flags[q];
    }
  }
  out_flags[b] = any ? 1 : 0;
}

__global__ void rl_fill_kernel(const IgemmParams p, const unsigned char* __restrict__ live, const float* __restrict__ g_addend,
                               const float* __restrict__ g_mask, float* __restrict__ g_out, void* __restrict__ g_ohi, void* __restrict__ g_olo) {
  const int b = blockIdx.x;
  if (live[b]) return;
  const int n4 = (p.Nout + 3) >> 2;
  const int r0 = 32 * b, nr = min(32, p.M - r0);
  if (g_ohi && !g_out && !g_addend && p.Nout == p.ld_out && (p.ld_out & 7) == 0 && (p.add_hi == nullptr || (p.ld_add & 7) == 0) &&
      (p.mask_hi == nullptr || (p.ld_mask & 7) == 0)) {
    const int n8 = nr * (p.ld_out >> 3);
    uint4* dst = reinterpret_cast<uint4*>(g_ohi) + 2 * (long long)r0 * (p.ld_out >> 3);
    const uint4 z4 = make_uint4(0u, 0u, 0u, 0u);
    for (int i = threadIdx.x; i < n8; i += blockDim.x) {
      uint4 oh = z4, ol = z4;
      if (p.add_hi) {
        const int r = i / (p.ld_out >> 3), g8 = i - r * (p.ld_out >> 3);
        const uint4* a = reinterpret_cast<const uint4*>(p.add_hi) + 2 * ((long long)(r0 + r) * (p.ld_add >> 3) + g8);
        oh = a[0];
        ol = a[1];
        if (p.mask_hi) {
          const uint4 k = reinterpret_cast<const uint4*>(p.mask_hi)[2 * ((long long)(r0 + r) * (p.ld_mask >> 3) + g8)];
          const unsigned kk[4] = {k.x, k.y, k.z, k.w};
          unsigned hh[4] = {oh.x, oh.y, oh.z, oh.w}, ll[4] = {ol.x, ol.y, ol.z, ol.w};
#pragma unroll
          for (int j = 0; j < 4; ++j) {
            const unsigned lo_ok = ((kk[j] & 0x8000u) == 0u && (kk[j] & 0x7fffu) != 0u) ? 0x0000ffffu : 0u;
            const unsigned hi_ok = ((kk[j] & 0x80000000u) == 0u && (kk[j] & 0x7fff0000u) != 0u) ? 0xffff0000u : 0u;
            hh[j] &= (lo_ok | hi_ok);
            ll[j] &= (lo_ok | hi_ok);
          }
          oh = make_uint4(hh[0], hh[1], hh[2], hh[3]);
          ol = make_uint4(ll[0], ll[1], ll[2], ll[3]);
        }
      }
      dst[2 * i] = oh;
      dst[2 * i + 1] = ol;
    }
    return;
  }
  for (int i = threadIdx.x; i < nr * n4; i += blockDim.x) {
    const int r = i / n4, co = 4 * (i - r * n4);
    const long long m = r0 + r;
    const float4 z = make_float4(0.f, 0.f, 0.f, 0.f);
    if (g_addend || p.add_hi) {
      finish4(p, z, m, co, true, g_addend, g_mask, g_out, g_ohi, g_olo);
    } else {
      if (g_out) *reinterpret_cast<float4*>(g_out + m * p.ld_out + co) = z;
      if (g_ohi) {
        reinterpret_cast<uint2*>(g_ohi)[pk4((m * p.ld_out + co) >> 2)] = make_uint2(0u, 0u);
        reinterpret_cast<uint2*>(g_olo)[pk4((m * p.ld_out + co) >> 2)] = make_uint2(0u, 0u);
      }
    }
  }
}

__global__ void row_block_compact_kernel(const unsigned char* __restrict__ flags, int n_blocks, int* __restrict__ list);

template <int TM, int TN>
static void launch_igemm3_rowlist(hipStream_t st, IgemmParams& p, const void* ahi, const void* alo, const void* whi, const void* wlo, int w_rows,
                                  int w_ld8, void* ohi, void* olo, const unsigned char* dy_flags, unsigned char* out_flags, int* out_list,
                                  float* ws, size_t ws_bytes, bool fill = true) {
  constexpr int BM = 64 * TM, BN = 64 * TN;
  const int nb = (p.M + 31) / 32;
  static const int want_splits = []() { const char* e = getenv("PP_SPARSE_DGRAD_SPLITS"); return e ? atoi(e) : 2; }();
  const int n_steps = p.kh * p.kw * (p.Cred / 32);
  int splits = 1;
  if (ws && want_splits > 1 && (ohi || p.out)) {
    const long long slice_bytes = (long long)nb * 32 * p.ld_out * 4;
    splits = want_splits;
    while (splits > 1 && (n_steps / splits < 24 || slice_bytes * splits > (long long)ws_bytes)) --splits;
  }
  if (dy_flags) hipLaunchKernelGGL(rl_dilate_kernel, dim3((unsigned)((nb + 255) / 256)), dim3(256), 0, st, p, dy_flags, out_flags, nb);
  hipLaunchKernelGGL(row_block_compact_kernel, dim3(1), dim3(256), 0, st, (const unsigned char*)out_flags, nb, out_list);
  p.n_tiles_n = (p.Nout + BN - 1) / BN;
  const int n_tiles_m = (nb + BM / 32 - 1) / (BM / 32);
  const long long a_bytes = p.src_rows * (long long)p.ld_src * 4, w_bytes = (long long)p.w_taps * w_rows * w_ld8 * 16;
  const dim3 grid((unsigned)(n_tiles_m * p.n_tiles_n * splits));
  if (ahi && !ohi)
    hipLaunchKernelGGL((igemm3f_kernel<TM, TN, true, false, false, true>), grid, dim3(256), 0, st, p, ahi, alo, (unsigned)a_bytes, whi, wlo,
                       (unsigned)w_bytes, p.bias, p.addend, p.mask_src, p.out, (uint2*)nullptr, (uint2*)nullptr, w_rows, w_ld8, splits,
                       splits > 1 ? ws : (float*)nullptr, (const int*)out_list, dy_flags);
  else if (ahi)
    hipLaunchKernelGGL((igemm3f_kernel<TM, TN, true, true, false, true>), grid, dim3(256), 0, st, p, ahi, alo, (unsigned)a_bytes, whi, wlo,
                       (unsigned)w_bytes, p.bias, p.addend, p.mask_src, p.out, (uint2*)ohi, (uint2*)olo, w_rows, w_ld8, splits,
                       splits > 1 ? ws : (float*)nullptr, (const int*)out_list, dy_flags);
  else
    hipLaunchKernelGGL((igemm3f_kernel<TM, TN, false, false, false, true>), grid, dim3(256), 0, st, p, (const void*)p.src, nullptr,
                       (unsigned)a_bytes, whi, wlo, (unsigned)w_bytes, p.bias, p.addend, p.mask_src, p.out, (uint2*)nullptr, (uint2*)nullptr,
                       w_rows, w_ld8, splits, splits > 1 ? ws : (float*)nullptr, (const int*)out_list, dy_flags);
  if (splits > 1)
    hipLaunchKernelGGL(rl_splitk_finish_kernel, dim3((unsigned)nb), dim3(256), 0, st, p, splits, (const float*)ws, (const int*)out_list, p.bias,
                       p.addend, p.mask_src, p.out, ohi, olo);
  const bool in_place = (ohi != nullptr && p.add_hi == (const void*)ohi && p.ld_add == p.ld_out && !p.out && !p.addend && !p.mask_hi &&
                         !p.mask_src && !p.relu) ||
                        (p.out != nullptr && p.addend == p.out && p.ld_add == p.ld_out && !ohi && !p.add_hi && !p.mask_hi && !p.mask_src && !p.relu);
  if (fill && !in_place)
    hipLaunchKernelGGL(rl_fill_kernel, dim3((unsigned)nb), dim3(256), 0, st, p, (const unsigned char*)out_flags, p.addend, p.mask_src, p.out, ohi,
                       olo);
}

static void split_capture_pass(hipStream_t st, const IgemmParams& p, void* chi, void* clo) {
  const size_t n8 = (size_t)(p.src_rows * (long long)p.ld_src / 8);
  size_t blocks = (n8 + 255) / 256;
  if (blocks > 8192) blocks = 8192;
  hipLaunchKernelGGL(split_planes_kernel, dim3((unsigned)blocks), dim3(256), 0, st, n8, (const float4*)p.src, (uint4*)chi, (uint4*)clo, (const float*)nullptr);
}

template <int TM, int TN>
static void launch_igemm3(hipStream_t st, IgemmParams& p, const void* ahi, const void* alo, const void* whi, const void* wlo, int w_rows,
                          int w_ld8, void* ohi, void* olo, int splits, float* ws, void* chi = nullptr, void* clo = nullptr,
                          const unsigned char* flags = nullptr, float* ws_any = nullptr, size_t ws_any_bytes = 0, int n_cu = 256) {
  constexpr int BM = 64 * TM, BN = 64 * TN;
  p.n_tiles_n = (p.Nout + BN - 1) / BN;
  const int n_tiles_m = (p.M + BM - 1) / BM;
  const dim3 grid((unsigned)(n_tiles_m * p.n_tiles_n * splits));
  const bool fast = igemm3_fast_ok(p, ahi != nullptr, w_rows, w_ld8);
  const long long a_bytes = p.src_rows * (long long)p.ld_src * 4;
  const long long w_bytes = (long long)p.w_taps * w_rows * w_ld8 * 16;
  if (p.sc_on) {
    if (ahi)
      hipLaunchKernelGGL((igemm3f_kernel<TM, TN, true, true, true>), grid, dim3(256), 0, st, p, ahi, alo, (unsigned)a_bytes, whi, wlo,
                         (unsigned)w_bytes, p.bias, p.addend, p.mask_src, p.out, (uint2*)ohi, (uint2*)olo, w_rows, w_ld8, 1, nullptr);
    else
      hipLaunchKernelGGL((igemm3f_kernel<TM, TN, false, false, true>), grid, dim3(256), 0, st, p, (const void*)p.src, nullptr, (unsigned)a_bytes,
                         whi, wlo, (unsigned)w_bytes, p.bias, p.addend, p.mask_src, p.out, (uint2*)nullptr, (uint2*)nullptr, w_rows, w_ld8, 1,
                         nullptr);
    return;
  }
  {
    if (igemm3x_ok(p, ahi != nullptr, ohi != nullptr, w_rows, w_ld8) && (TM <= 2 || (ahi != nullptr && !chi))) {
      const int n_tiles_mx = (p.M + BM - 3) / (BM - 2);
      int skip_halo = 0;
      for (int i = 0; i < p.n_seg; ++i) skip_halo = p.seg[i].SW + 1 > skip_halo ? p.seg[i].SW + 1 : skip_halo;
      const dim3 gridx((unsigned)(n_tiles_mx * p.n_tiles_n * splits));
      static const int x_order = []() { const char* e = getenv("PP_CONV3_X_ORDER"); return e ? atoi(e) : 1; }();
      p.x_ty_inner = x_order;
      const bool op = ohi != nullptr && splits == 1;
      if constexpr (TM <= 2) {
        if (chi) {
          hipLaunchKernelGGL((igemm3x_kernel<TM, TN, true>), gridx, dim3(256), 0, st, p, (const void*)p.src, nullptr, (unsigned)a_bytes, whi, wlo,
                             (unsigned)w_bytes, p.bias, p.addend, p.mask_src, p.out, (uint2*)nullptr, (uint2*)nullptr, w_rows, w_ld8, splits,
                             ws, chi, clo, flags, skip_halo);
          return;
        }
      }
      if constexpr (TM == 2 && TN == 2) {
        const char* const dma_env = getenv("PP_CONV3_DMA");
        const bool dma_on = !(dma_env && dma_env[0] == '0');
        if (dma_on && ahi && op && !flags && splits == 1 && p.kh == 3 && x_order == 1 && w_rows % 128 == 0 && p.Cred % 32 == 0) {
          constexpr int BM4 = 256;
          const int n_tiles_m4 = (p.M + BM4 - 3) / (BM4 - 2);
          const int ntn = (p.Nout + 127) / 128;
          static const int dma_min = []() { const char* e = getenv("PP_CONV3_DMA_MIN"); return e ? atoi(e) : 512; }();
          static const int dma_frac = []() { const char* e = getenv("PP_CONV3_DMA_FRAC"); return e ? atoi(e) : 1000; }();
          const int n_blk = n_tiles_m4 * ntn;
          const bool one_and_a_bit = n_blk > n_cu && n_blk < 2 * n_cu && (n_blk - n_cu) * 100 >= dma_frac * n_cu;
          if (n_blk >= dma_min || one_and_a_bit) {
            static const bool tail_on = []() { const char* e = getenv("PP_CONV3_DMA_TAIL"); return !(e && e[0] == '0'); }();
            int full_rt = n_tiles_m4;
            const int rounds = (n_tiles_m4 * ntn) / n_cu;
            static const int tail_frac = []() { const char* e = getenv("PP_CONV3_DMA_TAIL_FRAC"); return e ? atoi(e) : 60; }();
            const int last = (n_tiles_m4 * ntn) % n_cu;
            if (tail_on && last != 0 && last * 100 < tail_frac * n_cu && rounds >= 2 && ws_any != nullptr) full_rt = rounds * n_cu / ntn;
            const int m_split = full_rt * (BM4 - 2);
            int tail_splits = 0;
            if (full_rt < n_tiles_m4) {
              const int rem = p.M - m_split;
              const int n_rt = (rem + BM - 3) / (BM - 2);
              const int groups = p.kh * (p.Cred / 32);
              int sp = (3 * n_cu + n_rt * ntn - 1) / (n_rt * ntn);
              while (sp > 1 && (groups / sp < 4 || (size_t)sp * rem * p.ld_out * 4 > ws_any_bytes)) --sp;
              if (sp > 1) tail_splits = sp;
              else full_rt = n_tiles_m4;
            }
            p.n_tiles_n = ntn;
            const char* const e_var = getenv("PP_CONV3_DMA_VAR");
            const int var = e_var ? atoi(e_var) : 1;
            auto go4 = [&](auto v) {
              hipLaunchKernelGGL((igemm4x_kernel<true, decltype(v)::value>), dim3((unsigned)(full_rt * ntn)), dim3(512), 0, st, p, ahi, alo,
                                 (unsigned)a_bytes, whi, wlo, (unsigned)w_bytes, p.bias, p.addend, p.mask_src, p.out, (uint2*)ohi, (uint2*)olo, w_rows,
                                 w_ld8);
            };
            if (var == 0) go4(std::integral_constant<int, 0>{});
            else if (var == 2) go4(std::integral_constant<int, 2>{});
            else if (var == 3) go4(std::integral_constant<int, 3>{});
            else if (var == 4) go4(std::integral_constant<int, 4>{});
            else if (var == 9) go4(std::integral_constant<int, 9>{});
            else go4(std::integral_constant<int, 1>{});
            if (tail_splits > 1) {
              IgemmParams q = p;
              q.m_off = full_rt * (BM4 - 2);
              const int rem = q.M - q.m_off;
              const int n_rt = (rem + BM - 3) / (BM - 2);
              hipLaunchKernelGGL((igemm3x_kernel<TM, TN, false, true, false>), dim3((unsigned)(n_rt * ntn * tail_splits)), dim3(256), 0, st, q, ahi,
                                 alo, (unsigned)a_bytes, whi, wlo, (unsigned)w_bytes, q.bias, q.addend, q.mask_src, q.out, (uint2*)nullptr,
                                 (uint2*)nullptr, w_rows, w_ld8, tail_splits, ws_any, nullptr, nullptr, (const unsigned char*)nullptr, skip_halo);
              const long long total = (long long)rem * ((q.Nout + 3) >> 2);
              long long blocks = (total + 255) / 256;
              if (blocks > (long long)n_cu * 8) blocks = (long long)n_cu * 8;
              hipLaunchKernelGGL(splitk_finish_kernel, dim3((unsigned)blocks), dim3(256), 0, st, q, tail_splits, (const float*)ws_any, q.bias, q.addend,
                                 q.mask_src, q.out, ohi, olo);
            }
            return;
          }
          const char* const e_dma2 = getenv("PP_CONV3_DMA2");
          const bool dma2_on = e_dma2 && e_dma2[0] == '1';
          static const int dma2_min = []() { const char* e = getenv("PP_CONV3_DMA2_MIN"); return e ? atoi(e) : 512; }();
          if (dma2_on && n_tiles_mx * ntn >= dma2_min) {
            p.n_tiles_n = ntn;
            hipLaunchKernelGGL((igemm4x_kernel<true, 1, 2>), dim3((unsigned)(n_tiles_mx * ntn)), dim3(256), 0, st, p, ahi, alo, (unsigned)a_bytes, whi,
                               wlo, (unsigned)w_bytes, p.bias, p.addend, p.mask_src, p.out, (uint2*)ohi, (uint2*)olo, w_rows, w_ld8);
            return;
          }
        }
      }
      if (ahi && op)
        hipLaunchKernelGGL((igemm3x_kernel<TM, TN, false, true, true>), gridx, dim3(256), 0, st, p, ahi, alo, (unsigned)a_bytes, whi, wlo,
                           (unsigned)w_bytes, p.bias, p.addend, p.mask_src, p.out, (uint2*)ohi, (uint2*)olo, w_rows, w_ld8, splits, ws, nullptr,
                           nullptr, flags, skip_halo);
      else if (ahi)
        hipLaunchKernelGGL((igemm3x_kernel<TM, TN, false, true, false>), gridx, dim3(256), 0, st, p, ahi, alo, (unsigned)a_bytes, whi, wlo,
                           (unsigned)w_bytes, p.bias, p.addend, p.mask_src, p.out, (uint2*)nullptr, (uint2*)nullptr, w_rows, w_ld8, splits, ws,
                           nullptr, nullptr, flags, skip_halo);
      else if constexpr (TM <= 2) {
        if (op)
          hipLaunchKernelGGL((igemm3x_kernel<TM, TN, false, false, true>), gridx, dim3(256), 0, st, p, (const void*)p.src, nullptr,
                             (unsigned)a_bytes, whi, wlo, (unsigned)w_bytes, p.bias, p.addend, p.mask_src, p.out, (uint2*)ohi, (uint2*)olo,
                             w_rows, w_ld8, splits, ws, nullptr, nullptr, flags, skip_halo);
        else
          hipLaunchKernelGGL((igemm3x_kernel<TM, TN, false>), gridx, dim3(256), 0, st, p, (const void*)p.src, nullptr, (unsigned)a_bytes, whi,
                             wlo, (unsigned)w_bytes, p.bias, p.addend, p.mask_src, p.out, (uint2*)nullptr, (uint2*)nullptr, w_rows, w_ld8, splits,
                             ws, nullptr, nullptr, flags, skip_halo);
      }
      return;
    }
  }
  if (chi) split_capture_pass(st, p, chi, clo);
  if (splits > 1) ohi = olo = nullptr;
  auto go = [&](auto ap, auto op) {
    constexpr bool AP = decltype(ap)::value, OP = decltype(op)::value;
    if (fast)
      hipLaunchKernelGGL((igemm3f_kernel<TM, TN, AP, OP>), grid, dim3(256), 0, st, p, AP ? ahi : (const void*)p.src, AP ? alo : nullptr,
                         (unsigned)a_bytes, whi, wlo, (unsigned)w_bytes, p.bias, p.addend, p.mask_src, p.out, (uint2*)ohi, (uint2*)olo,
                         w_rows, w_ld8, splits, ws);
    else
      hipLaunchKernelGGL((igemm3_kernel<TM, TN, AP, OP>), grid, dim3(256), 0, st, p, p.src, (const uint4*)(AP ? ahi : nullptr),
                         (const uint4*)(AP ? alo : nullptr), (const uint4*)whi, (const uint4*)wlo, p.bias, p.addend, p.mask_src, p.out,
                         (uint2*)ohi, (uint2*)olo, w_rows, w_ld8);
  };
  if (ahi && ohi) go(std::true_type{}, std::true_type{});
  else if (ahi) go(std::true_type{}, std::false_type{});
  else if (ohi) go(std::false_type{}, std::true_type{});
  else go(std::false_type{}, std::false_type{});
}

static void pick_tile3(const pp_ctx* ctx, int M, int Nout, int ld_out, int n_steps, bool may_split, bool x_ok, int* tm, int* tn, int* splits) {
  static const int cand[5][2] = {{4, 2}, {2, 2}, {1, 2}, {2, 1}, {1, 1}};
  static const double eff[5] = {1.1, 1.0, 0.9, 0.9, 0.8};
  static const int slots[5] = {2, 3, 4, 4, 4};
  static const int split_cand[8] = {1, 2, 3, 4, 6, 8, 12, 16};
  const int cus = ctx->n_cu > 0 ? ctx->n_cu : 256;
  const long long ws_bytes = (long long)ctx->ws_bytes;
  double best = 1e300;
  *splits = 1;
  for (int i = 0; i < 5; ++i) {
    const int bm = 64 * cand[i][0], bn = 64 * cand[i][1];
    const long long blocks = (long long)((M + bm - 1) / bm) * ((Nout + bn - 1) / bn);
    for (int si = 0; si < (may_split ? 8 : 1); ++si) {
      const int sp = split_cand[si];
      if (sp > 1 && (n_steps / sp < 8 || (long long)sp * M * ld_out * 4 > ws_bytes)) break;
      const double steps = (double)((n_steps + sp - 1) / sp) + 8.0;
      double t = est_rounds(blocks * sp, slots[i], cus) * steps * cand[i][0] * cand[i][1] / eff[i];
      if (sp > 1) {
        const double us = (double)M * Nout * (8.0 * sp + 12.0) / 4.0e6 + 4.0;
        t += us / 2.1 * 4.0;
      }
      if (t < best * 0.97) {
        best = t;
        *tm = cand[i][0];
        *tn = cand[i][1];
        *splits = sp;
      }
    }
  }
  static const bool x4 = []() { const char* e = getenv("PP_CONV3_X4"); return e && e[0] == '1'; }();
  if (x_ok && *tm == 4 && *splits == 1 && !x4) {
    *tm = 2;
    *tn = 2;
  }
  const char* e = getenv("PP_CONV3_TILE");
  if (e && e[0] && e[1] == ',' && e[2]) {
    *tm = e[0] - '0';
    *tn = e[2] - '0';
  }
  if (const char* es = getenv("PP_CONV3_SPLITS")) {
    const int v = atoi(es);
    if (v >= 1 && (v == 1 || (may_split && n_steps / v >= 1 && (long long)v * M * ld_out * 4 <= ws_bytes))) *splits = v;
  }
}

static void dispatch3(pp_ctx* ctx, IgemmParams& p, const void* ahi, const void* alo, const void* whi, const void* wlo, int w_rows,
                      int w_ld8, void* ohi, void* olo, void* chi = nullptr, void* clo = nullptr, const unsigned char* flags = nullptr) {
  int tm, tn, splits;
  const int n_steps = p.kh * p.kw * (p.Cred / 32);
  {
    const char* const e_on = getenv("PP_CONV4P");
    const char* const e_nst = getenv("PP_CONV4P_NST");
    const char* const e_sp = getenv("PP_CONV4P_SPLITS");
    const bool p_on = e_on && e_on[0] == '1';
    const int p_nst = e_nst && atoi(e_nst) == 3 ? 3 : 4;
    const int p_splits = e_sp ? atoi(e_sp) : 0;
    const long long a_bytes = p.src_rows * (long long)p.ld_src * 4, w_bytes = (long long)p.w_taps * w_rows * w_ld8 * 16;
    if (p_on && p.kh == 1 && p.kw == 1 && ahi && !chi && !flags && !p.sc_on && p.div == 1 && p.Cred % 32 == 0 && p.ld_src % 8 == 0 &&
        a_bytes < (1ll << 31) && w_bytes < (1ll << 31) && p.src_rows > 0 && (ohi || p.out)) {
      const int n_cu = ctx->n_cu > 0 ? ctx->n_cu : 256;
      const long long tiles = (long long)((p.M + 127) / 128) * ((p.Nout + 127) / 128);
      int sp = 1;
      if (tiles * 4 < (long long)n_cu * 3 && ctx->ws != nullptr) {
        sp = (int)(n_cu / tiles);
        while (sp > 1 && (n_steps / sp < 4 || (long long)sp * p.M * p.ld_out * 4 > (long long)ctx->ws_bytes)) --sp;
      }
      if (p_splits >= 1 && (p_splits == 1 || (ctx->ws != nullptr && n_steps / p_splits >= 1 && (long long)p_splits * p.M * p.ld_out * 4 <= (long long)ctx->ws_bytes)))
        sp = p_splits;
      if (getenv("PP_CONV_DEBUG"))
        fprintf(stderr, "igemm4p M %d N %d steps %d -> %lld tiles x %d splits on %d CUs, %d stages\n", p.M, p.Nout, n_steps, tiles, sp, n_cu, p_nst);
      PP_API(pp4_launch_igemm4p)(ctx->stream, p, ahi, whi, wlo, w_rows, w_ld8, ohi, olo, sp, sp > 1 ? ctx->ws : nullptr, n_cu, p_nst);
      if (sp > 1) {
        const long long total = (long long)p.M * ((p.Nout + 3) >> 2);
        long long blocks = (total + 255) / 256;
        if (blocks > (long long)n_cu * 8) blocks = (long long)n_cu * 8;
        hipLaunchKernelGGL(splitk_finish_kernel, dim3((unsigned)blocks), dim3(256), 0, ctx->stream, p, sp, ctx->ws, p.bias, p.addend, p.mask_src, p.out,
                           ohi, olo);
      }
      return;
    }
  }
  const bool may_split = ctx->ws != nullptr && (ohi || p.out != nullptr) && !p.sc_on && igemm3_fast_ok(p, ahi != nullptr, w_rows, w_ld8);
  pick_tile3(ctx, p.M, p.Nout, p.ld_out, n_steps, may_split, igemm3x_ok(p, ahi != nullptr, ohi != nullptr, w_rows, w_ld8), &tm, &tn, &splits);
  if (getenv("PP_CONV_DEBUG"))
    fprintf(stderr, "igemm3 M %d N %d steps %d -> tile %dx%d splits %d (may_split %d: ws %d planes_out %d out %d)\n", p.M, p.Nout, n_steps, 64 * tm,
            64 * tn, splits, (int)may_split, (int)(ctx->ws != nullptr), (int)(ohi != nullptr), (int)(p.out != nullptr));
  float* ws = splits > 1 ? ctx->ws : nullptr;
  if (tm == 4) launch_igemm3<4, 2>(ctx->stream, p, ahi, alo, whi, wlo, w_rows, w_ld8, ohi, olo, splits, ws, chi, clo, flags);
  else if (tm == 2 && tn == 2)
    launch_igemm3<2, 2>(ctx->stream, p, ahi, alo, whi, wlo, w_rows, w_ld8, ohi, olo, splits, ws, chi, clo, flags, ctx->ws, (size_t)ctx->ws_bytes,
                        ctx->n_cu > 0 ? ctx->n_cu : 256);
  else if (tm == 1 && tn == 2) launch_igemm3<1, 2>(ctx->stream, p, ahi, alo, whi, wlo, w_rows, w_ld8, ohi, olo, splits, ws, chi, clo, flags);
  else if (tm == 2 && tn == 1) launch_igemm3<2, 1>(ctx->stream, p, ahi, alo, whi, wlo, w_rows, w_ld8, ohi, olo, splits, ws, chi, clo, flags);
  else launch_igemm3<1, 1>(ctx->stream, p, ahi, alo, whi, wlo, w_rows, w_ld8, ohi, olo, splits, ws, chi, clo, flags);
  if (splits > 1) {
    const long long total = (long long)p.M * ((p.Nout + 3) >> 2);
    long long blocks = (total + 255) / 256;
    const long long cap = (long long)(ctx->n_cu > 0 ? ctx->n_cu : 256) * 8;
    if (blocks > cap) blocks = cap;
    hipLaunchKernelGGL(splitk_finish_kernel, dim3((unsigned)blocks), dim3(256), 0, ctx->stream, p, splits, ctx->ws, p.bias, p.addend, p.mask_src,
                       p.out, ohi, olo);
  }
}

}
extern "C" int PP_API(pp_conv2d_nhwc_fwd_bf16x3)(pp_ctx* ctx, const pp_conv_desc* d, const float* x, const void* x_hi, const void* x_lo,
                                         const void* w_hi, const void* w_lo, const float* bias, const float* residual, int ld_res,
                                         int relu, float* y, void* y_hi, void* y_lo, const pp_conv_opts* opts) {
  PP_REQUIRE_CTX(ctx);
  int rc = pp_conv_opts_take(ctx, opts, PP_OPT_CAPTURE | PP_OPT_ADD | PP_OPT_OUT, "pp_conv2d_nhwc_fwd_bf16x3");
  if (rc) return rc;
  void *const chi = opts->capture_hi, *const clo = opts->capture_lo;
  const void *const ep_ah = opts->add_hi, *const ep_al = opts->add_lo;
  rc = check_desc(ctx, d, "pp_conv2d_nhwc_fwd_bf16x3");
  PP_CHECK_ARG(ctx, !(ep_ah && residual), PP_ERR_ARG, "pp_conv2d_nhwc_fwd_bf16x3: residual given both as f32 and as planes");
  PP_CHECK_ARG(ctx, !ep_ah || (ld_res % 4 == 0 && ld_res >= ((d->cout + 3) & ~3)), PP_ERR_SHAPE, "pp_conv2d_nhwc_fwd_bf16x3: residual planes");
  if (rc) return rc;
  PP_CHECK_ARG(ctx, !chi || (x && !x_hi && pp_is_packed(chi, clo)), PP_ERR_ARG, "pp_conv2d_nhwc_fwd_bf16x3: split capture needs the f32 operand");
  PP_CHECK_ARG(ctx, (x || (x_hi && x_lo)) && w_hi && w_lo && (y || (y_hi && y_lo)), PP_ERR_ARG, "pp_conv2d_nhwc_fwd_bf16x3: null tensor");
  PP_CHECK_ARG(ctx, (x_hi == nullptr) == (x_lo == nullptr), PP_ERR_ARG, "pp_conv2d_nhwc_fwd_bf16x3: x_hi and x_lo go together");
  PP_CHECK_ARG(ctx, d->cin % 32 == 0 && d->ld_x % 8 == 0, PP_ERR_SHAPE, "pp_conv2d_nhwc_fwd_bf16x3: cin %d must be a multiple of 32, ld_x of 8", d->cin);
  PP_CHECK_ARG(ctx, pp_is_packed(x_hi, x_lo) && pp_is_packed(y_hi, y_lo), PP_ERR_ALIGN,
               "pp_conv2d_nhwc_fwd_bf16x3: planes must be packed (lo = hi + 16 bytes, 16-byte aligned)");
  PP_CHECK_ARG(ctx, !y_hi || (d->cout % 8 == 0 && d->ld_y % 8 == 0), PP_ERR_SHAPE, "pp_conv2d_nhwc_fwd_bf16x3: output planes need cout, ld_y %% 8 == 0");
  PP_CHECK_ARG(ctx, !ep_ah || (ld_res % 8 == 0 && d->cout % 8 == 0), PP_ERR_SHAPE, "pp_conv2d_nhwc_fwd_bf16x3: residual planes need cout, ld_res %% 8 == 0");
  PP_CHECK_ARG(ctx, (!x || pp_is_aligned16(x)) && pp_is_aligned16(w_hi) && pp_is_aligned16(w_lo) && (!y || pp_is_aligned16(y)), PP_ERR_ALIGN,
               "pp_conv2d_nhwc_fwd_bf16x3: tensors must be 16-byte aligned");
  PP_CHECK_ARG(ctx, !residual || (ld_res % 4 == 0 && ld_res >= ((d->cout + 3) & ~3) && pp_is_aligned16(residual)), PP_ERR_SHAPE,
               "pp_conv2d_nhwc_fwd_bf16x3: residual");
  PP_CHECK_ARG(ctx, !bias || pp_is_aligned16(bias), PP_ERR_ALIGN, "pp_conv2d_nhwc_fwd_bf16x3: bias alignment");
  IgemmParams p;
  memset(&p, 0, sizeof(p));
  p.src = x; p.out = y; p.bias = bias; p.addend = residual; p.mask_src = nullptr;
  p.add_hi = ep_ah; p.add_lo = ep_al;
  p.ld_src = d->ld_x; p.ld_w = d->ld_w; p.ld_out = d->ld_y; p.ld_add = ld_res; p.ld_mask = 0;
  p.relu = relu;
  p.n_seg = d->in.n_seg;
  fill_segs(ctx, d, true, p.seg, &p.M, &p.src_rows);
  p.Cred = d->cin; p.Nout = d->cout; p.w_tap_rows = d->cin;
  p.kh = d->kh; p.kw = d->kw;
  p.mul = d->stride; p.tsign = 1; p.off_y = -d->pad_t; p.off_x = -d->pad_l; p.div = 1;
  p.w_ty0 = 0; p.w_tx0 = 0; p.w_tstep = 1; p.w_kw = d->kw; p.w_taps = d->kh * d->kw;
  PP_CHECK_ARG(ctx, (y_hi == nullptr) == (y_lo == nullptr) && (!y_hi || (d->ld_y % 4 == 0 && pp_is_aligned16(y_hi) && pp_is_aligned16(y_lo))),
               PP_ERR_ARG, "pp_conv2d_nhwc_fwd_bf16x3: output planes");
  if (opts->out_flags) {
    bool ok = x_hi != nullptr && ((y != nullptr) != (y_hi != nullptr)) && !chi && !residual && !ep_ah && d->stride == 1 && d->kh == 3 && d->kw == 3 && d->pad_t == 1 &&
              d->pad_l == 1 && igemm3_fast_ok(p, true, d->cout, d->cin / 8);
    for (int i = 0; i < p.n_seg && ok; ++i)
      ok = p.seg[i].OH == p.seg[i].SH && p.seg[i].OW == p.seg[i].SW && p.seg[i].row_begin == p.seg[i].src_row_begin;
    PP_CHECK_ARG(ctx, ok, PP_ERR_SHAPE, "pp_conv2d_nhwc_fwd_bf16x3: out_flags needs a 3x3 stride-1 'same' conv on plane-stored input");
    launch_igemm3_rowlist<2, 2>(ctx->stream, p, x_hi, x_lo, w_hi, w_lo, d->cout, d->cin / 8, y_hi, y_lo, nullptr,
                                const_cast<unsigned char*>(opts->out_flags) , opts->out_list, ctx->ws,
                                ctx->ws_bytes, false);
    PP_CHECK_LAUNCH(ctx, "pp_conv2d_nhwc_fwd_bf16x3");
    return PP_OK;
  }
  dispatch3(ctx, p, x_hi, x_lo, w_hi, w_lo, d->cout, d->cin / 8, y_hi, y_lo, chi, clo);
  PP_CHECK_LAUNCH(ctx, "pp_conv2d_nhwc_fwd_bf16x3");
  return PP_OK;
}
namespace {

}
extern "C" int PP_API(pp_row_block_dilate)(pp_ctx* ctx, const pp_conv_desc* d, const unsigned char* in_flags, unsigned char* out_flags) {
  PP_REQUIRE_CTX(ctx);
  int rc = check_desc(ctx, d, "pp_row_block_dilate");
  if (rc) return rc;
  PP_CHECK_ARG(ctx, in_flags && out_flags && in_flags != out_flags, PP_ERR_ARG, "pp_row_block_dilate: two distinct flag buffers");
  IgemmParams p;
  memset(&p, 0, sizeof(p));
  p.n_seg = d->in.n_seg;
  fill_segs(ctx, d, true, p.seg, &p.M, &p.src_rows);
  bool same = d->stride == 1 && d->kh == 3 && d->kw == 3;
  for (int i = 0; i < p.n_seg && same; ++i) same = p.seg[i].OH == p.seg[i].SH && p.seg[i].OW == p.seg[i].SW && p.seg[i].row_begin == p.seg[i].src_row_begin;
  PP_CHECK_ARG(ctx, same, PP_ERR_SHAPE, "pp_row_block_dilate: 3x3 stride-1 conv on an unchanged grid");
  const int nb = (p.M + 31) / 32;
  hipLaunchKernelGGL(rl_dilate_kernel, dim3((unsigned)((nb + 255) / 256)), dim3(256), 0, ctx->stream, p, in_flags, out_flags, nb);
  PP_CHECK_LAUNCH(ctx, "pp_row_block_dilate");
  return PP_OK;
}
namespace {

}
extern "C" int PP_API(pp_stem7x7s2_fwd_bf16x3)(pp_ctx* ctx, int n_img, int H, int W, int Hp, int Wp, const float* x4p, const void* w_hi,
                                       const void* w_lo, int cout, const float* bias, int relu, float* y, int ld_y) {
  PP_REQUIRE_CTX(ctx);
  PP_CHECK_ARG(ctx, x4p && w_hi && w_lo && y && pp_is_aligned16(x4p) && pp_is_aligned16(y) && pp_is_aligned16(w_hi) && pp_is_aligned16(w_lo),
               PP_ERR_ARG, "pp_stem7x7s2_fwd_bf16x3: null / unaligned tensor");
  PP_CHECK_ARG(ctx, n_img > 0 && H > 0 && W > 0 && Hp >= H + 6 && Wp >= W + 8 && Wp % 2 == 0 && cout > 0 && ld_y % 4 == 0 && ld_y >= ((cout + 3) & ~3),
               PP_ERR_SHAPE, "pp_stem7x7s2_fwd_bf16x3: bad geometry");
  const int OH = (H + 6 - 7) / 2 + 1, OW = (W + 6 - 7) / 2 + 1;
  IgemmParams p;
  memset(&p, 0, sizeof(p));
  p.src = x4p; p.out = y; p.bias = bias;
  p.ld_src = 4; p.ld_out = ld_y;
  p.relu = relu;
  p.n_seg = 1;
  p.seg[0].row_begin = 0; p.seg[0].src_row_begin = 0;
  p.seg[0].OH = OH; p.seg[0].OW = OW; p.seg[0].SH = Hp; p.seg[0].SW = Wp;
  p.M = n_img * OH * OW;
  p.src_rows = (long long)n_img * Hp * Wp;
  p.Cred = 32; p.Nout = cout; p.w_tap_rows = 32;
  p.kh = 7; p.kw = 1;
  p.mul = 2; p.tsign = 1; p.off_y = 0; p.off_x = 0; p.div = 1;
  p.w_ty0 = 0; p.w_tx0 = 0; p.w_tstep = 1; p.w_kw = 1; p.w_taps = 7;
  PP_CHECK_ARG(ctx, igemm3_fast_ok(p, false, cout, 4), PP_ERR_SHAPE, "pp_stem7x7s2_fwd_bf16x3: frame too large for 31-bit offsets");
  dispatch3(ctx, p, nullptr, nullptr, w_hi, w_lo, cout, 4, nullptr, nullptr);
  PP_CHECK_LAUNCH(ctx, "pp_stem7x7s2_fwd_bf16x3");
  return PP_OK;
}
namespace {

}
extern "C" int PP_API(pp_conv2d_nhwc_bwd_data_bf16x3)(pp_ctx* ctx, const pp_conv_desc* d, const float* dy, const void* dy_hi, const void* dy_lo,
                                              const void* w_hi, const void* w_lo, const float* addend, int ld_add,
                                              const float* relu_src, int ld_rs, float* dx, void* dx_hi, void* dx_lo,
                                              const pp_conv_opts* opts) {
  PP_REQUIRE_CTX(ctx);
  int rc = pp_conv_opts_take(ctx, opts, PP_OPT_CAPTURE | PP_OPT_ADD | PP_OPT_MASK | PP_OPT_SKIP | PP_OPT_LAZY_OUT | PP_OPT_LAZY_IN,
                             "pp_conv2d_nhwc_bwd_data_bf16x3");
  if (rc) return rc;
  void *const chi = opts->capture_hi, *const clo = opts->capture_lo;
  unsigned char* const skip_flags = opts->skip_flags;
  const bool skip_scratch_ok = skip_flags != nullptr && opts->skip_list != nullptr;
  const void *const ep_ah = opts->add_hi, *const ep_al = opts->add_lo, *const ep_mh = opts->mask_hi;
  rc = check_desc(ctx, d, "pp_conv2d_nhwc_bwd_data_bf16x3");
  PP_CHECK_ARG(ctx, !(ep_ah && addend) && !(ep_mh && relu_src), PP_ERR_ARG,
               "pp_conv2d_nhwc_bwd_data_bf16x3: addend / relu_src given both as f32 and as planes");
  PP_CHECK_ARG(ctx, (!ep_ah || (ld_add >= d->cin && ld_add % 4 == 0)) && (!ep_mh || (ld_rs >= d->cin && ld_rs % 4 == 0)), PP_ERR_SHAPE,
               "pp_conv2d_nhwc_bwd_data_bf16x3: addend / relu_src planes");
  if (rc) return rc;
  PP_CHECK_ARG(ctx, !chi || (dy && !dy_hi && pp_is_packed(chi, clo)), PP_ERR_ARG, "pp_conv2d_nhwc_bwd_data_bf16x3: split capture needs the f32 operand");
  PP_CHECK_ARG(ctx, (dy || (dy_hi && dy_lo)) && w_hi && w_lo && (dx || (dx_hi && dx_lo)), PP_ERR_ARG, "pp_conv2d_nhwc_bwd_data_bf16x3: null tensor");
  PP_CHECK_ARG(ctx, (dy_hi == nullptr) == (dy_lo == nullptr) && d->ld_y % 8 == 0, PP_ERR_ARG, "pp_conv2d_nhwc_bwd_data_bf16x3: planes / ld_y");
  PP_CHECK_ARG(ctx, pp_is_packed(dy_hi, dy_lo) && pp_is_packed(dx_hi, dx_lo), PP_ERR_ALIGN,
               "pp_conv2d_nhwc_bwd_data_bf16x3: planes must be packed (lo = hi + 16 bytes, 16-byte aligned)");
  PP_CHECK_ARG(ctx, (!dx_hi || (d->cin % 8 == 0 && d->ld_x % 8 == 0)) && (!ep_ah || ld_add % 8 == 0) && (!ep_mh || ld_rs % 8 == 0), PP_ERR_SHAPE,
               "pp_conv2d_nhwc_bwd_data_bf16x3: planes need channel counts and leading dimensions %% 8 == 0");
  const int cred = (d->cout + 31) / 32 * 32;
  PP_CHECK_ARG(ctx, d->cin % 16 == 0 && d->ld_y >= cred && d->ld_y % 4 == 0, PP_ERR_SHAPE,
               "pp_conv2d_nhwc_bwd_data_bf16x3: dy needs ld_y >= %d (cout rounded up to 32, zero padded)", cred);
  PP_CHECK_ARG(ctx, (!dy || pp_is_aligned16(dy)) && pp_is_aligned16(w_hi) && pp_is_aligned16(w_lo) && (!dx || pp_is_aligned16(dx)), PP_ERR_ALIGN,
               "pp_conv2d_nhwc_bwd_data_bf16x3: tensors must be 16-byte aligned");
  PP_CHECK_ARG(ctx, (!addend || (ld_add >= d->cin && ld_add % 4 == 0 && pp_is_aligned16(addend))) &&
                        (!relu_src || (ld_rs >= d->cin && ld_rs % 4 == 0 && pp_is_aligned16(relu_src))),
               PP_ERR_SHAPE, "pp_conv2d_nhwc_bwd_data_bf16x3: addend / relu_src");
  IgemmParams p;
  memset(&p, 0, sizeof(p));
  p.src = dy; p.out = dx; p.bias = nullptr; p.addend = addend; p.mask_src = relu_src;
  p.add_hi = ep_ah; p.add_lo = ep_al; p.mask_hi = ep_mh;
  p.ld_src = d->ld_y; p.ld_w = d->ld_w; p.ld_out = d->ld_x; p.ld_add = ld_add; p.ld_mask = ld_rs;
  p.relu = 0;
  p.n_seg = d->in.n_seg;
  fill_segs(ctx, d, false, p.seg, &p.M, &p.src_rows);
  p.Cred = cred; p.Nout = d->cin; p.w_tap_rows = d->cin;
  p.kh = d->kh; p.kw = d->kw;
  p.mul = 1; p.tsign = -1; p.off_y = d->pad_t; p.off_x = d->pad_l; p.div = d->stride;
  p.w_ty0 = 0; p.w_tx0 = 0; p.w_tstep = 1; p.w_kw = d->kw; p.w_taps = d->kh * d->kw;
  PP_CHECK_ARG(ctx, (dx_hi == nullptr) == (dx_lo == nullptr) && (!dx_hi || (d->ld_x % 4 == 0 && pp_is_aligned16(dx_hi) && pp_is_aligned16(dx_lo))),
               PP_ERR_ARG, "pp_conv2d_nhwc_bwd_data_bf16x3: output planes");
  static const bool s2_classes = []() { const char* e = getenv("PP_CONV3_S2CLASSES"); return !(e && e[0] == '0'); }();
  const bool all_f32 = dy && dx && !dy_hi && !dx_hi, all_planes = dy_hi && dx_hi && !dx;
  static const int rl_mode = []() { const char* e = getenv("PP_SPARSE_DGRAD"); return e ? atoi(e) : 22; }();
  bool rl_ok = skip_flags && skip_scratch_ok && rl_mode && (all_f32 || all_planes) && !chi && d->stride == 1 && d->kh == 3 && d->kw == 3 &&
               d->pad_t == 1 && d->pad_l == 1 && p.bias == nullptr && igemm3_fast_ok(p, all_planes, d->cin, cred / 8);
  for (int i = 0; i < p.n_seg && rl_ok; ++i)
    rl_ok = p.seg[i].OH == p.seg[i].SH && p.seg[i].OW == p.seg[i].SW && p.seg[i].row_begin == p.seg[i].src_row_begin;
  PP_CHECK_ARG(ctx, !opts->lazy_in || rl_ok, PP_ERR_ARG,
               "pp_conv2d_nhwc_bwd_data_bf16x3: dy was declared lazy (unwritten outside its flagged blocks) but the listed-block launch "
               "does not apply to this call");
  if (skip_scratch_ok && !rl_ok)
    PP_HIP(ctx, hipMemsetAsync(skip_flags + (p.M + 31) / 32, 1, (size_t)((p.M + 31) / 32), ctx->stream));
  if (d->stride == 2 && s2_classes && (all_f32 || all_planes) && d->in.n_seg == 1) {
    IgemmParams q = p;
    q.div = 1;
    const int H = d->in.h[0], W = d->in.w[0];
    bool ok = true;
    IgemmParams cls[4];
    for (int c = 0; c < 4 && ok; ++c) {
      const int cy = c >> 1, cx = c & 1;
      IgemmParams& r = cls[c];
      r = q;
      const int ty0 = (cy + d->pad_t) & 1, tx0 = (cx + d->pad_l) & 1;
      r.kh = ty0 < d->kh ? (d->kh - ty0 + 1) / 2 : 0;
      r.kw = tx0 < d->kw ? (d->kw - tx0 + 1) / 2 : 0;
      r.off_y = (cy + d->pad_t - ty0) / 2;
      r.off_x = (cx + d->pad_l - tx0) / 2;
      r.w_ty0 = ty0; r.w_tx0 = tx0; r.w_tstep = 2; r.w_kw = d->kw;
      if (r.kh == 0 || r.kw == 0) r.kh = r.kw = 0;
      r.seg[0].OH = (H - cy + 1) / 2;
      r.seg[0].OW = (W - cx + 1) / 2;
      r.M = d->in.n_img * r.seg[0].OH * r.seg[0].OW;
      r.sc_on = 1; r.sc_H = H; r.sc_W = W; r.sc_cy = cy; r.sc_cx = cx;
      if (r.M > 0 && r.kh > 0 && !(igemm3_fast_ok(r, all_planes, d->cin, cred / 8) && r.M < (1 << 24))) ok = false;
    }
    if (ok) {
      if (chi) split_capture_pass(ctx->stream, p, chi, clo);
      for (int c = 0; c < 4; ++c) {
        if (cls[c].M <= 0) continue;
        if (cls[c].kh > 0) {
          dispatch3(ctx, cls[c], dy_hi, dy_lo, w_hi, w_lo, d->cin, cred / 8, dx_hi, dx_lo);
        } else {
          const long long total = (long long)cls[c].M * ((cls[c].Nout + 3) >> 2);
          long long blocks = (total + 255) / 256;
          const long long cap = (long long)(ctx->n_cu > 0 ? ctx->n_cu : 256) * 8;
          if (blocks > cap) blocks = cap;
          hipLaunchKernelGGL(class_fill_kernel, dim3((unsigned)blocks), dim3(256), 0, ctx->stream, cls[c], addend, relu_src, dx, dx_hi, dx_lo);
        }
      }
      PP_CHECK_LAUNCH(ctx, "pp_conv2d_nhwc_bwd_data_bf16x3");
      return PP_OK;
    }
  }
  if (rl_ok) {
    const int nb = (p.M + 31) / 32;
    unsigned char* out_flags = skip_flags + nb;
    int* out_list = opts->skip_list + nb + 1;
    if (rl_mode == 22)
      launch_igemm3_rowlist<2, 2>(ctx->stream, p, dy_hi, dy_lo, w_hi, w_lo, d->cin, cred / 8, dx_hi, dx_lo, skip_flags, out_flags, out_list, ctx->ws,
                                  ctx->ws_bytes, !opts->lazy_out);
    else
      launch_igemm3_rowlist<1, 2>(ctx->stream, p, dy_hi, dy_lo, w_hi, w_lo, d->cin, cred / 8, dx_hi, dx_lo, skip_flags, out_flags, out_list, ctx->ws,
                                  ctx->ws_bytes, !opts->lazy_out);
    PP_CHECK_LAUNCH(ctx, "pp_conv2d_nhwc_bwd_data_bf16x3");
    return PP_OK;
  }
  dispatch3(ctx, p, dy_hi, dy_lo, w_hi, w_lo, d->cin, cred / 8, dx_hi, dx_lo, chi, clo, skip_flags);
  PP_CHECK_LAUNCH(ctx, "pp_conv2d_nhwc_bwd_data_bf16x3");
  return PP_OK;
}
namespace {

typedef short shortx4 __attribute__((ext_vector_type(4)));


template <int TM, int TN, bool AP>
__global__ __launch_bounds__(256, (TM * TN == 4) ? 2 : 3) void wgrad3_kernel(const Wgrad3Params p, const float* __restrict__ g_src,
                                                                            const float* __restrict__ g_dy,
                                                                            const uint4* __restrict__ g_xhi, const uint4* __restrict__ g_xlo,
                                                                            const uint4* __restrict__ g_dhi, const uint4* __restrict__ g_dlo,
                                                                            float* __restrict__ g_dw, float* __restrict__ g_dbias) {
  constexpr int BM = 64 * TM, BN = 64 * TN, BK = 32;
  constexpr int PA = BM + 32, PB = BN + 32;
  __shared__ __attribute__((aligned(16))) unsigned short smem[2 * BK * (PA + PB)];
  unsigned short* Xhi = smem;
  unsigned short* Xlo = Xhi + BK * PA;
  unsigned short* Ghi = Xlo + BK * PA;
  unsigned short* Glo = Ghi + BK * PB;

  const int tid = threadIdx.x, lane = tid & 63, wave = tid >> 6;
  const float inv_g = p.inv_scale ? *p.inv_scale : 1.f;
  const int wm = wave >> 1, wn = wave & 1;
  int b = xcd_remap((int)blockIdx.x, (int)gridDim.x);
  const int tile_n = b % p.n_tiles_n;
  b /= p.n_tiles_n;
  const int tile_k = b % p.n_tiles_k;
  const int split = b / p.n_tiles_k;
  const int tap = tile_k / p.k_tiles_per_tap;
  const int ci0 = (tile_k - tap * p.k_tiles_per_tap) * BM;
  const int ty = tap / p.kw, tx = tap - ty * p.kw;
  const int n0 = tile_n * BN;
  const int m_begin = split * p.rows_per_split;
  const int m_end = min(p.M, m_begin + p.rows_per_split);
  const int n_steps = (m_end - m_begin + BK - 1) / BK;

  const int prow = tid >> 3, q8 = tid & 7;
  constexpr int QA = BM / 32, QB = BN / 32;
  struct WRow { int m, n, y, x, seg_end, sb, OH, OW, SH, SW; } w;
  auto decode = [&](int m) {
    w.m = m;
    int rbeg = p.seg[0].row_begin;
    w.sb = p.seg[0].src_row_begin; w.OH = p.seg[0].OH; w.OW = p.seg[0].OW; w.SH = p.seg[0].SH; w.SW = p.seg[0].SW;
    w.seg_end = p.n_seg > 1 ? p.seg[1].row_begin : p.M;
    for (int s = 1; s < p.n_seg; ++s) {
      if (m >= p.seg[s].row_begin) {
        rbeg = p.seg[s].row_begin; w.sb = p.seg[s].src_row_begin; w.OH = p.seg[s].OH; w.OW = p.seg[s].OW;
        w.SH = p.seg[s].SH; w.SW = p.seg[s].SW;
        w.seg_end = (s + 1 < p.n_seg) ? p.seg[s + 1].row_begin : p.M;
      }
    }
    const int local = m < p.M ? m - rbeg : 0;
    const int hw = w.OH * w.OW;
    w.n = local / hw;
    const int rem = local - w.n * hw;
    w.y = rem / w.OW;
    w.x = rem - w.y * w.OW;
  };
  decode(m_begin + prow);

  constexpr int OA = (BM / 64 > 0) ? BM / 64 : 1, OB = (BN / 64 > 0) ? BN / 64 : 1;
  float4 ra[QA], rb[QB];
  uint4 pah[OA], pal[OA], pbh[OB], pbl[OB];
  float4 bsum[QB];
#pragma unroll
  for (int j = 0; j < QB; ++j) bsum[j] = make_float4(0.f, 0.f, 0.f, 0.f);
  const bool do_bias = (g_dbias != nullptr) && (tile_k == 0);

  auto load_step = [&]() {
    const int sy = w.y * p.stride + ty - p.pad_t;
    const int sx = w.x * p.stride + tx - p.pad_l;
    const bool in_rng = w.m < m_end;
    const bool ok = in_rng && ((unsigned)sy < (unsigned)w.SH) && ((unsigned)sx < (unsigned)w.SW);
    const long long xrow = (long long)(w.sb + w.n * w.SH * w.SW + sy * w.SW + sx) * p.ld_src + ci0;
    if (AP) {
#pragma unroll
      for (int j = 0; j < OA; ++j) {
        const long long o8 = 2 * ((xrow >> 3) + q8 + 8 * j);
        pah[j] = ok ? g_xhi[o8] : make_uint4(0u, 0u, 0u, 0u);
        pal[j] = ok ? g_xlo[o8] : make_uint4(0u, 0u, 0u, 0u);
      }
#pragma unroll
      for (int j = 0; j < OB; ++j) {
        const int c = n0 + 8 * (q8 + 8 * j);
        const bool okb = in_rng && c < p.ld_dy;
        const long long o8 = 2 * ((((long long)w.m * p.ld_dy + n0) >> 3) + q8 + 8 * j);
        pbh[j] = okb ? g_dhi[o8] : make_uint4(0u, 0u, 0u, 0u);
        pbl[j] = okb ? g_dlo[o8] : make_uint4(0u, 0u, 0u, 0u);
      }
    } else {
      const float* src = g_src + xrow;
#pragma unroll
      for (int j = 0; j < QA; ++j)
        ra[j] = ok ? *reinterpret_cast<const float4*>(src + 4 * (q8 + 8 * j)) : make_float4(0.f, 0.f, 0.f, 0.f);
      const float* dyr = g_dy + (long long)w.m * p.ld_dy + n0;
#pragma unroll
      for (int j = 0; j < QB; ++j) {
        const int c = n0 + 4 * (q8 + 8 * j);
        rb[j] = (in_rng && c < p.ld_dy) ? *reinterpret_cast<const float4*>(dyr + 4 * (q8 + 8 * j)) : make_float4(0.f, 0.f, 0.f, 0.f);
      }
    }
    const int m2 = w.m + BK;
    if (m2 >= w.seg_end) {
      decode(m2);
    } else {
      w.m = m2;
      w.x += BK;
      while (w.x >= w.OW) { w.x -= w.OW; ++w.y; }
      while (w.y >= w.OH) { w.y -= w.OH; ++w.n; }
    }
  };
  auto store_step = [&]() {
    if (AP) {
#pragma unroll
      for (int j = 0; j < OA; ++j) {
        const int off = prow * PA + 8 * (q8 + 8 * j);
        if (8 * (q8 + 8 * j) < BM) {
          *reinterpret_cast<uint4*>(Xhi + off) = pah[j];
          *reinterpret_cast<uint4*>(Xlo + off) = pal[j];
        }
      }
#pragma unroll
      for (int j = 0; j < OB; ++j) {
        const int off = prow * PB + 8 * (q8 + 8 * j);
        if (8 * (q8 + 8 * j) < BN) {
          *reinterpret_cast<uint4*>(Ghi + off) = pbh[j];
          *reinterpret_cast<uint4*>(Glo + off) = pbl[j];
          if (do_bias) {
            const unsigned int hw[4] = {pbh[j].x, pbh[j].y, pbh[j].z, pbh[j].w}, lw[4] = {pbl[j].x, pbl[j].y, pbl[j].z, pbl[j].w};
            float v[8];
#pragma unroll
            for (int e = 0; e < 4; ++e) fmt_value2(hw[e], lw[e], &v[2 * e], &v[2 * e + 1]);
            bsum[2 * j].x += v[0]; bsum[2 * j].y += v[1]; bsum[2 * j].z += v[2]; bsum[2 * j].w += v[3];
            bsum[2 * j + 1].x += v[4]; bsum[2 * j + 1].y += v[5]; bsum[2 * j + 1].z += v[6]; bsum[2 * j + 1].w += v[7];
          }
        }
      }
      return;
    }
#pragma unroll
    for (int j = 0; j < QA; ++j) {
      uint2 hi, lo;
      split4(ra[j], &hi, &lo);
      const int off = prow * PA + 4 * (q8 + 8 * j);
      *reinterpret_cast<uint2*>(Xhi + off) = hi;
      *reinterpret_cast<uint2*>(Xlo + off) = lo;
    }
// ... 511 lines not shown
```

pyrapose_amd/csrc/ctx.hip:

```cpp
#include <stdlib.h>

#include "pp_internal.h"

extern "C" const char* pp_version(void) { return "pyrapose_hip 0.7 (gfx950; convolutions on packed planes in two formats -- bf16 pairs / bf16x3 and P16 / f16c8 (f16 + block-scaled e5m2 MFMA) -- and exact f32 MFMA; sparse 3D-box backward, pose tail, device augmentation)"; }

extern "C" int pp_ctx_create(pp_ctx** out, int device, void* hip_stream) {
  if (!out) return PP_ERR_ARG;
  *out = nullptr;
  int n_dev = 0;
  hipError_t e = hipGetDeviceCount(&n_dev);
  if (e != hipSuccess) return (int)e;
  if (device < 0 || device >= n_dev) return PP_ERR_ARG;
  pp_ctx* c = (pp_ctx*)calloc(1, sizeof(pp_ctx));
  if (!c) return PP_ERR_ARG;
  c->device = device;
  c->stream = (hipStream_t)hip_stream;
  hipDeviceProp_t prop;
  e = hipGetDeviceProperties(&prop, device);
  if (e != hipSuccess) {
    free(c);
    return (int)e;
  }
  c->n_cu = prop.multiProcessorCount;
  snprintf(c->name, sizeof(c->name), "%s (%s)", prop.name, prop.gcnArchName);
  c->err[0] = 0;
  *out = c;
  return PP_OK;
}

extern "C" void pp_ctx_destroy(pp_ctx* ctx) { free(ctx); }

extern "C" int pp_ctx_set_stream(pp_ctx* ctx, void* hip_stream) {
  PP_REQUIRE_CTX(ctx);
  ctx->stream = (hipStream_t)hip_stream;
  return PP_OK;
}

extern "C" int pp_ctx_set_workspace(pp_ctx* ctx, void* zeroed, size_t bytes) {
  PP_REQUIRE_CTX(ctx);
  PP_CHECK_ARG(ctx, (zeroed == nullptr) == (bytes == 0) && pp_is_aligned16(zeroed), PP_ERR_ARG, "pp_ctx_set_workspace: bad buffer");
  ctx->ws = (float*)zeroed;
  ctx->ws_bytes = bytes;
  return PP_OK;
}

extern "C" int pp_ctx_set_planes_format(pp_ctx* ctx, int fmt) {
  PP_REQUIRE_CTX(ctx);
  PP_CHECK_ARG(ctx, fmt == 0 || fmt == 1, PP_ERR_ARG, "pp_ctx_set_planes_format: 0 (bf16 pairs) or 1 (P16)");
  ctx->planes_fmt = fmt;
  return PP_OK;
}

extern "C" int pp_ctx_set_grad_scale(pp_ctx* ctx, const float* scale2_dev) {
  PP_REQUIRE_CTX(ctx);
  ctx->grad_scale = scale2_dev;
  return PP_OK;
}

extern "C" const char* pp_last_error_string(pp_ctx* ctx) { return ctx ? ctx->err : "no context"; }

extern "C" int pp_device_info(pp_ctx* ctx, int* n_cu, char* name, int name_len) {
  PP_REQUIRE_CTX(ctx);
  if (n_cu) *n_cu = ctx->n_cu;
  if (name && name_len > 0) {
    strncpy(name, ctx->name, (size_t)name_len - 1);
    name[name_len - 1] = 0;
  }
  return PP_OK;
}
```

pyrapose_amd/csrc/pp_internal.h:

```cpp
#pragma once
#include <hip/hip_runtime.h>
#include <stdarg.h>
#include <stdio.h>
#include <string.h>

#include "pyrapose_hip.h"

struct pp_ctx {
  int device;
  hipStream_t stream;
  int n_cu;
  char name[128];
  char err[512];
  float* ws;
  size_t ws_bytes;
  int planes_fmt;
  const float* grad_scale;
};

static inline int pp_fail(pp_ctx* ctx, int code, const char* fmt, ...) {
  if (ctx) {
    va_list ap;
    va_start(ap, fmt);
    vsnprintf(ctx->err, sizeof(ctx->err), fmt, ap);
    va_end(ap);
  }
  return code;
}

#define PP_REQUIRE_CTX(ctx) \
  do {                      \
    if (!(ctx)) return PP_ERR_NOCTX; \
  } while (0)

#define PP_CHECK_ARG(ctx, cond, code, ...)            \
  do {                                                \
    if (!(cond)) return pp_fail(ctx, code, __VA_ARGS__); \
  } while (0)

#define PP_CHECK_LAUNCH(ctx, what)                                                   \
  do {                                                                               \
    hipError_t e__ = hipGetLastError();                                              \
    if (e__ != hipSuccess)                                                           \
      return pp_fail(ctx, (int)e__, "%s: launch failed: %s", what, hipGetErrorString(e__)); \
  } while (0)

#define PP_HIP(ctx, call)                                                                        \
  do {                                                                                           \
    hipError_t e__ = (call);                                                                     \
    if (e__ != hipSuccess) return pp_fail(ctx, (int)e__, "%s: %s", #call, hipGetErrorString(e__)); \
  } while (0)

static inline long long pp_rowspace_rows(const pp_rowspace* rs) {
  long long r = 0;
  for (int s = 0; s < rs->n_seg; ++s) r += (long long)rs->n_img * rs->h[s] * rs->w[s];
  return r;
}

static inline int pp_rowspace_ok(const pp_rowspace* rs) {
  if (rs->n_img <= 0 || rs->n_seg <= 0 || rs->n_seg > PP_MAX_SEG) return 0;
  for (int s = 0; s < rs->n_seg; ++s)
    if (rs->h[s] <= 0 || rs->w[s] <= 0) return 0;
  return pp_rowspace_rows(rs) < (1ll << 31);
}

static inline int pp_is_aligned16(const void* p) { return (((uintptr_t)p) & 15u) == 0; }
static inline int pp_is_packed(const void* hi, const void* lo) {
  return (hi == nullptr && lo == nullptr) || (hi != nullptr && (const char*)lo == (const char*)hi + 16 && pp_is_aligned16(hi));
}

enum { PP_OPT_CAPTURE = 1, PP_OPT_ADD = 2, PP_OPT_MASK = 4, PP_OPT_SKIP = 8, PP_OPT_LAZY_OUT = 16, PP_OPT_LAZY_IN = 32, PP_OPT_OUT = 64 };
static inline int pp_conv_opts_take(pp_ctx* ctx, const pp_conv_opts*& o, unsigned takes, const char* who) {
  static const pp_conv_opts none = {};
  if (!o) o = &none;
  const struct { unsigned group; bool set; const char* name; } fields[] = {
      {PP_OPT_CAPTURE, o->capture_hi != nullptr, "capture_hi"}, {PP_OPT_CAPTURE, o->capture_lo != nullptr, "capture_lo"},
      {PP_OPT_ADD, o->add_hi != nullptr, "add_hi"},             {PP_OPT_ADD, o->add_lo != nullptr, "add_lo"},
      {PP_OPT_MASK, o->mask_hi != nullptr, "mask_hi"},          {PP_OPT_SKIP, o->skip_flags != nullptr, "skip_flags"},
      {PP_OPT_SKIP, o->skip_list != nullptr, "skip_list"},      {PP_OPT_OUT, o->out_flags != nullptr, "out_flags"},
      {PP_OPT_OUT, o->out_list != nullptr, "out_list"},         {PP_OPT_LAZY_OUT, o->lazy_out != 0, "lazy_out"},
      {PP_OPT_LAZY_IN, o->lazy_in != 0, "lazy_in"}};
  for (const auto& f : fields) PP_CHECK_ARG(ctx, !f.set || (takes & f.group), PP_ERR_ARG, "%s: pp_conv_opts.%s is not an option of this call", who, f.name);
  PP_CHECK_ARG(ctx, (o->capture_hi == nullptr) == (o->capture_lo == nullptr) && pp_is_aligned16(o->capture_hi) && pp_is_aligned16(o->capture_lo),
               PP_ERR_ARG, "%s: pp_conv_opts.capture_hi and capture_lo go together, 16-byte aligned", who);
  PP_CHECK_ARG(ctx, (o->add_hi == nullptr) == (o->add_lo == nullptr), PP_ERR_ARG, "%s: pp_conv_opts.add_hi and add_lo go together", who);
  PP_CHECK_ARG(ctx, pp_is_packed(o->add_hi, o->add_lo) && pp_is_aligned16(o->mask_hi), PP_ERR_ALIGN,
               "%s: pp_conv_opts epilogue planes must be packed (lo = hi + 16 bytes) and 16-byte aligned", who);
  PP_CHECK_ARG(ctx, (o->out_flags == nullptr) == (o->out_list == nullptr), PP_ERR_ARG, "%s: pp_conv_opts.out_flags and out_list go together", who);
  PP_CHECK_ARG(ctx, !(o->lazy_out || o->lazy_in) || (o->skip_flags && o->skip_list), PP_ERR_ARG,
               "%s: pp_conv_opts.lazy_out / lazy_in go with skip_flags and skip_list", who);
  return PP_OK;
}
```

pyrapose_amd/ops.py:

```python
import ctypes as C

import numpy as np
import torch

from ._lib import ConvDesc, ConvOpts, ParamDesc, RowSpace, TView, check, lib


def _ptr(t):
    if t is None:
        return None
    assert t.is_cuda, "pyrapose_amd ops need device tensors"
    return C.c_void_p(t.data_ptr())


class Context:

    def __init__(self, device=0, stream=None):
        if not torch.cuda.is_available():
            raise RuntimeError("pyrapose_amd: no GPU visible (torch.cuda.is_available() is False); "
                               "the HIP path has no CPU fallback")
        self.device = int(device)
        torch.cuda.set_device(self.device)
        self.handle = C.c_void_p()
        s = stream if stream is not None else torch.cuda.current_stream(self.device)
# ... 7 lines not shown
        for c in (self, self._twin):
            if c is not None:
                c.stream = stream
                check(lib.pp_ctx_set_stream(c.handle, C.c_void_p(stream.cuda_stream)), c.handle, "pp_ctx_set_stream")

    def twin(self, fmt):
        if int(fmt) == self.planes_fmt:
            return self
        if self._twin is None:
            t = Context(self.device, self.stream)
            set_planes_format(t, fmt)
            t._twin = self
            ws = getattr(self, "workspace", None)
            t.workspace = ws
            if ws is not None:
                check(lib.pp_ctx_set_workspace(t.handle, _ptr(ws), ws.numel() * 4), t.handle, "pp_ctx_set_workspace")
            self._twin = t
        assert self._twin.planes_fmt == int(fmt)
        return self._twin

    def set_workspace(self, nbytes):
        self.workspace = torch.empty((int(nbytes) // 4,), dtype=torch.float32, device="cuda:%d" % self.device) if nbytes else None
        for c in (self, self._twin):
            if c is not None:
                c.workspace = self.workspace
                check(lib.pp_ctx_set_workspace(c.handle, _ptr(self.workspace), (int(nbytes) // 4) * 4 if nbytes else 0), c.handle,
                      "pp_ctx_set_workspace")

    def device_info(self):
        n = C.c_int(0)
        buf = C.create_string_buffer(128)
        check(lib.pp_device_info(self.handle, C.byref(n), buf, 128), self.handle)
        return n.value, buf.value.decode()

    def close(self):
        t, self._twin = self._twin, None
        if t is not None and t.handle:
            t._twin = None
            t.close()
        if self.handle:
            lib.pp_ctx_destroy(self.handle)
            self.handle = C.c_void_p()


def make_conv_desc(n_img, in_shapes, out_shapes, cin, cout, k, stride, pad_t, pad_l, ld_x, ld_y, ld_w):
    d = ConvDesc()
    d.in_ = RowSpace.make(n_img, in_shapes)
    d.out = RowSpace.make(n_img, out_shapes)
    d.cin, d.cout, d.kh, d.kw, d.stride = cin, cout, k, k, stride
    d.pad_t, d.pad_l, d.ld_x, d.ld_y, d.ld_w = pad_t, pad_l, ld_x, ld_y, ld_w
    return d


def conv_fwd(ctx, d, x, w, bias, residual, relu, y):
    ld_res = residual.stride(0) if residual is not None else 0
    check(lib.pp_conv2d_nhwc_fwd(ctx.handle, C.byref(d), _ptr(x), _ptr(w), _ptr(bias), _ptr(residual), ld_res,
                                 int(bool(relu)), _ptr(y)), ctx.handle, "pp_conv2d_nhwc_fwd")


def conv_bwd_data(ctx, d, dy, w, addend, relu_src, dx):
    ld_add = addend.stride(0) if addend is not None else 0
    ld_rs = relu_src.stride(0) if relu_src is not None else 0
    check(lib.pp_conv2d_nhwc_bwd_data(ctx.handle, C.byref(d), _ptr(dy), _ptr(w), _ptr(addend), ld_add, _ptr(relu_src),
                                      ld_rs, _ptr(dx)), ctx.handle, "pp_conv2d_nhwc_bwd_data")


def conv_bwd_weight(ctx, d, x, dy, dw, dbias):
    check(lib.pp_conv2d_nhwc_bwd_weight(ctx.handle, C.byref(d), _ptr(x), _ptr(dy), _ptr(dw), _ptr(dbias)), ctx.handle,
          "pp_conv2d_nhwc_bwd_weight")


def conv_split_weights3(ctx, d, w, fwd_hi, fwd_lo, dg_hi, dg_lo):
    check(lib.pp_conv_split_weights_bf16x3(ctx.handle, C.byref(d), _ptr(w), _ptr(fwd_hi), _ptr(fwd_lo), _ptr(dg_hi), _ptr(dg_lo)),
          ctx.handle, "pp_conv_split_weights_bf16x3")


class SplitWeightsBatch(object):

    def __init__(self, jobs):
        from ._lib import SplitJob
        jobs = list(jobs)
        arr = (SplitJob * max(len(jobs), 1))()
        tiles = 0
        self._keep = jobs
        for i, (d, w, fh, fl, dh, dl) in enumerate(jobs):
            if d.cin % 32:
                raise ValueError("SplitWeightsBatch: cin %d must be a multiple of 32" % d.cin)
            j = arr[i]
            j.w, j.fwd_hi, j.fwd_lo, j.dg_hi, j.dg_lo = [(t.data_ptr() if t is not None else None) for t in (w, fh, fl, dh, dl)]
            j.taps, j.cin, j.cout, j.ld_w, j.tile_begin = d.kh * d.kw, d.cin, d.cout, d.ld_w, tiles
            tiles += j.taps * (d.cin // 32) * ((d.cout + 31) // 32)
        self.n, self.tiles = len(jobs), tiles
        host = torch.frombuffer(bytearray(bytes(arr)), dtype=torch.uint8)
        self.table = host.cuda()

    def run(self, ctx):
        check(lib.pp_conv_split_weights_bf16x3_batch(ctx.handle, self.n, _ptr(self.table), self.tiles), ctx.handle,
              "pp_conv_split_weights_bf16x3_batch")


def new_planes(rows, ld, device="cuda", fill=0):
    assert ld % 8 == 0, ld
    base = torch.full((rows, ld // 8, 2, 8), fill, dtype=torch.int16, device=device)
    return base[:, :, 0, :], base[:, :, 1, :]


def planes_ld(planes):
    return planes[0].stride(0) // 2


def set_planes_format(ctx, fmt):
    check(lib.pp_ctx_set_planes_format(ctx.handle, int(fmt)), ctx.handle, "pp_ctx_set_planes_format")
    ctx.planes_fmt = int(fmt)


def convert_planes(ctx, src, src_fmt, dst, dst_fmt, scale2=None, scale_index=0, relu_src_hi=None):
    n = src[0].numel()
    check(lib.pp_convert_planes(ctx.handle, n, _ptr(src[0]), _ptr(src[1]), int(src_fmt), _ptr(dst[0]), _ptr(dst[1]), int(dst_fmt), _ptr(scale2),
                                int(scale_index), _ptr(relu_src_hi)), ctx.handle, "pp_convert_planes")


def planes_to_f32(planes, fmt=0):
    hi, lo = planes
    rows = hi.shape[0]
    if fmt == 0:
        return (hi.contiguous().view(torch.bfloat16).float() + lo.contiguous().view(torch.bfloat16).float()).reshape(rows, -1)
    rem = (lo.contiguous().to(torch.int32) & 0xff00).to(torch.int16).view(torch.float16).float() / 4096.0
    return (hi.contiguous().view(torch.float16).float() + rem).reshape(rows, -1)


def weight_planes_to_f32(hi, lo, fmt=0):
    if fmt == 0:
        return hi.contiguous().view(torch.bfloat16).float() + lo.contiguous().view(torch.bfloat16).float()
    rem = ((lo.contiguous().to(torch.int32) & 0xff) << 8).to(torch.int16).view(torch.float16).float() / 4096.0
    return hi.contiguous().view(torch.float16).float() + rem


def split_planes3(ctx, src, hi, lo, scale=None):
    if scale is None:
        check(lib.pp_split_planes_bf16x3(ctx.handle, src.numel(), _ptr(src), _ptr(hi), _ptr(lo)), ctx.handle, "pp_split_planes_bf16x3")
    else:
        check(lib.pp_split_planes_scaled_bf16x3(ctx.handle, src.numel(), _ptr(src), _ptr(hi), _ptr(lo), _ptr(scale)), ctx.handle,
              "pp_split_planes_scaled_bf16x3")


def grad_scale_from_counts(ctx, counts, scale2, log2_adjust=0):
    check(lib.pp_grad_scale_from_counts_adj(ctx.handle, _ptr(counts), int(counts.numel()), _ptr(scale2), int(log2_adjust)), ctx.handle,
          "pp_grad_scale_from_counts")


def set_grad_scale(ctx, scale2):
    ctx._grad_scale_keep = scale2
    check(lib.pp_ctx_set_grad_scale(ctx.handle, _ptr(scale2)), ctx.handle, "pp_ctx_set_grad_scale")


def row_block_list(ctx, x, cols, flags=None, blocks=None):
    rows, ld = x.shape
    nb = (rows + 31) // 32
    if flags is None:
        flags = torch.zeros((2 * nb,), dtype=torch.uint8, device=x.device)
    if blocks is None:
        blocks = torch.zeros((2 * (nb + 1),), dtype=torch.int32, device=x.device)
    check(lib.pp_row_block_list(ctx.handle, _ptr(x), rows, x.stride(0), int(cols), _ptr(flags), _ptr(blocks)), ctx.handle, "pp_row_block_list")
    return flags, blocks


def row_block_list_planes(ctx, planes, cols, flags, blocks, within=None):
    hi, lo = planes
    rows = hi.shape[0]
    if within is not None:
        assert within.dtype == torch.uint8 and within.is_contiguous() and within.numel() >= (rows + 31) // 32
        check(lib.pp_row_block_list_planes_within(ctx.handle, _ptr(hi), _ptr(lo), rows, planes_ld(planes), int(cols), _ptr(within), _ptr(flags),
                                                  _ptr(blocks)), ctx.handle, "pp_row_block_list_planes_within")
    else:
        check(lib.pp_row_block_list_planes(ctx.handle, _ptr(hi), _ptr(lo), rows, planes_ld(planes), int(cols), _ptr(flags), _ptr(blocks)),
              ctx.handle, "pp_row_block_list_planes")
    return flags, blocks


def tview(t=None, planes=None):
    v = TView()
    v.f32 = t.data_ptr() if t is not None else None
    v.hi = planes[0].data_ptr() if planes is not None else None
    v.lo = planes[1].data_ptr() if planes is not None else None
    v._keep = (t, planes)
    return v


def _numel(v):
    t, planes = v._keep
    return (t if t is not None else planes[0]).numel()


def add_n_v(ctx, a, b, c, out):
    null = TView()
    check(lib.pp_add_n_v(ctx.handle, _numel(a), C.byref(a), C.byref(b if b is not None else null), C.byref(c if c is not None else null),
                         C.byref(out)), ctx.handle, "pp_add_n_v")


def relu_fwd_v(ctx, x, y):
    check(lib.pp_relu_fwd_v(ctx.handle, _numel(x), C.byref(x), C.byref(y)), ctx.handle, "pp_relu_fwd_v")


def upsample_add_fwd_v(ctx, n_img, sh, sw, th, tw, c, src, other, out):
    null = TView()
    check(lib.pp_upsample_nearest_add_fwd_v(ctx.handle, n_img, sh, sw, th, tw, c, C.byref(src), C.byref(other if other is not None else null),
                                            C.byref(out)), ctx.handle, "pp_upsample_nearest_add_fwd_v")


def upsample_add_bwd_v(ctx, n_img, sh, sw, th, tw, c, dtarget, base, dsrc):
    null = TView()
    check(lib.pp_upsample_nearest_add_bwd_v(ctx.handle, n_img, sh, sw, th, tw, c, C.byref(dtarget), C.byref(base if base is not None else null),
                                            C.byref(dsrc)), ctx.handle, "pp_upsample_nearest_add_bwd_v")


def merge_planes3(ctx, planes, dst):
    check(lib.pp_merge_planes_bf16x3(ctx.handle, dst.numel(), _ptr(planes[0]), _ptr(planes[1]), _ptr(dst)), ctx.handle, "pp_merge_planes_bf16x3")


def planes_stats(ctx, planes, cols, stats, within=None):
    hi, lo = planes
    check(lib.pp_planes_stats(ctx.handle, _ptr(hi), _ptr(lo), int(hi.shape[0]), planes_ld(planes), int(cols), _ptr(within), _ptr(stats)), ctx.handle,
          "pp_planes_stats")
    return stats


def positive_row_blocks(ctx, rs, n_anchor, y_true, flags):
    check(lib.pp_positive_row_blocks(ctx.handle, C.byref(rs), int(n_anchor), int(y_true.shape[-1]), _ptr(y_true), _ptr(flags)), ctx.handle,
          "pp_positive_row_blocks")
    return flags


def row_block_dilate(ctx, d, in_flags, out_flags):
    check(lib.pp_row_block_dilate(ctx.handle, C.byref(d), _ptr(in_flags), _ptr(out_flags)), ctx.handle, "pp_row_block_dilate")
    return out_flags


def _conv_opts(capture=None, add=None, mask_hi=None, skip=None, out=None, lazy_out=False, lazy_in=False):
    if capture is None and add is None and mask_hi is None and skip is None and out is None and not (lazy_out or lazy_in):
        return None
    o = ConvOpts()
    o.capture_hi, o.capture_lo = map(_ptr, capture or (None, None))
    o.add_hi, o.add_lo = map(_ptr, add or (None, None))
    o.mask_hi = _ptr(mask_hi)
    o.skip_flags, o.skip_list = map(_ptr, skip or (None, None))
    o.out_flags, o.out_list = map(_ptr, out or (None, None))
    o.lazy_out, o.lazy_in = int(bool(lazy_out)), int(bool(lazy_in))
    return C.byref(o)


def conv_fwd3(ctx, d, x, w_hi, w_lo, bias, residual, relu, y, x_planes=None, y_planes=None, x_capture=None, res_planes=None,
              out_blocks=None):
    ld_res = residual.stride(0) if residual is not None else (planes_ld(res_planes) if res_planes is not None else 0)
    xh, xl = x_planes if x_planes is not None else (None, None)
    yh, yl = y_planes if y_planes is not None else (None, None)
    check(lib.pp_conv2d_nhwc_fwd_bf16x3(ctx.handle, C.byref(d), _ptr(x), _ptr(xh), _ptr(xl), _ptr(w_hi), _ptr(w_lo), _ptr(bias),
                                        _ptr(residual), ld_res, int(bool(relu)), _ptr(y), _ptr(yh), _ptr(yl),
                                        _conv_opts(capture=x_capture, add=res_planes, out=out_blocks)), ctx.handle,
          "pp_conv2d_nhwc_fwd_bf16x3")


def conv_bwd_data3(ctx, d, dy, w_hi, w_lo, addend, relu_src, dx, dy_planes=None, dx_planes=None, dy_capture=None, dy_skip=None,
                   addend_planes=None, relu_src_hi=None, lazy_out=False, lazy_in=False):
    ld_add = addend.stride(0) if addend is not None else (planes_ld(addend_planes) if addend_planes is not None else 0)
    ld_rs = relu_src.stride(0) if relu_src is not None else (relu_src_hi.stride(0) // 2 if relu_src_hi is not None else 0)
    dh, dl = dy_planes if dy_planes is not None else (None, None)
    xh, xl = dx_planes if dx_planes is not None else (None, None)
    check(lib.pp_conv2d_nhwc_bwd_data_bf16x3(ctx.handle, C.byref(d), _ptr(dy), _ptr(dh), _ptr(dl), _ptr(w_hi), _ptr(w_lo), _ptr(addend),
                                             ld_add, _ptr(relu_src), ld_rs, _ptr(dx), _ptr(xh), _ptr(xl),
                                             _conv_opts(capture=dy_capture, add=addend_planes, mask_hi=relu_src_hi, skip=dy_skip,
                                                        lazy_out=lazy_out, lazy_in=lazy_in)), ctx.handle,
          "pp_conv2d_nhwc_bwd_data_bf16x3")


def conv_bwd_weight3(ctx, d, x, dy, dw, dbias, x_planes=None, dy_planes=None, dy_skip=None, lazy_in=False):
    xh, xl = x_planes if x_planes is not None else (None, None)
    dh, dl = dy_planes if dy_planes is not None else (None, None)
    check(lib.pp_conv2d_nhwc_bwd_weight_bf16x3(ctx.handle, C.byref(d), _ptr(x), _ptr(dy), _ptr(xh), _ptr(xl), _ptr(dh), _ptr(dl),
                                               _ptr(dw), _ptr(dbias), _conv_opts(skip=dy_skip, lazy_in=lazy_in)), ctx.handle,
          "pp_conv2d_nhwc_bwd_weight_bf16x3")


def maxpool3x3s2(ctx, n_img, h, w, c, x, oh, ow, y):
    check(lib.pp_maxpool3x3s2_fwd(ctx.handle, n_img, h, w, c, _ptr(x), oh, ow, _ptr(y)), ctx.handle, "pp_maxpool3x3s2_fwd")


def upsample_add_fwd(ctx, n_img, sh, sw, th, tw, c, src, other, out):
    check(lib.pp_upsample_nearest_add_fwd(ctx.handle, n_img, sh, sw, th, tw, c, _ptr(src), _ptr(other), _ptr(out)),
          ctx.handle, "pp_upsample_nearest_add_fwd")


def upsample_add_bwd(ctx, n_img, sh, sw, th, tw, c, dtarget, base, dsrc):
    check(lib.pp_upsample_nearest_add_bwd(ctx.handle, n_img, sh, sw, th, tw, c, _ptr(dtarget), _ptr(base), _ptr(dsrc)),
          ctx.handle, "pp_upsample_nearest_add_bwd")


def add_n(ctx, a, b, c, out):
    check(lib.pp_add_n(ctx.handle, a.numel(), _ptr(a), _ptr(b), _ptr(c), _ptr(out)), ctx.handle, "pp_add_n")


def relu_fwd(ctx, x, y):
    check(lib.pp_relu_fwd(ctx.handle, x.numel(), _ptr(x), _ptr(y)), ctx.handle, "pp_relu_fwd")


def warp_affine_u8(ctx, images_u8, matrices, interpolation="linear", border="replicate", cval=0, out=None):
    B, H, W = images_u8.shape[:3]
# ... 503 lines not shown
```

Baseline: 617.2.

## Fuse split-K reduction and row-block compaction into producer kernels via atomic tickets

Adds per-tile atomic ticket counters so the last split-K workgroup to arrive sums the partial slices and applies the epilogue itself, removing the separate reduction kernel launch. The row-block flag kernels likewise compact the block list in their last-arriving workgroup, and the per-class fill launches in the backward-data pass are batched into one 2D launch. This cuts launch count and a round trip through the workspace, at the cost of release/acquire fences, atomics, a serial tail in the last workgroup, and a ticket buffer that must be reset back to zero.

```diff
diff --git a/include/pyrapose_hip.h b/include/pyrapose_hip.h
--- a/include/pyrapose_hip.h
+++ b/include/pyrapose_hip.h
@@ -24,6 +24,7 @@
 void pp_ctx_destroy(pp_ctx* ctx);
 int pp_ctx_set_stream(pp_ctx* ctx, void* hip_stream);
 int pp_ctx_set_workspace(pp_ctx* ctx, void* device_buffer, size_t bytes);
+int pp_ctx_tickets(pp_ctx* ctx, int* count, int* nonzero);
 int pp_row_block_list(pp_ctx* ctx, const float* x, int rows, int ld, int cols, unsigned char* flags, int* list);
 int pp_row_block_list_planes(pp_ctx* ctx, const void* x_hi, const void* x_lo, int rows, int ld, int cols, unsigned char* flags, int* list);
 int pp_row_block_list_planes_within(pp_ctx* ctx, const void* x_hi, const void* x_lo, int rows, int ld, int cols, const unsigned char* within,
diff --git a/pyrapose_amd/_lib.py b/pyrapose_amd/_lib.py
--- a/pyrapose_amd/_lib.py
+++ b/pyrapose_amd/_lib.py
@@ -101,6 +101,7 @@
     "pp_allreduce_bucket": (_i, [_p, _p, _p, C.c_size_t]),
     "pp_allreduce_counts": (_i, [_p, _p, _p, _i]),
     "pp_ctx_set_workspace": (_i, [_p, _p, C.c_size_t]),
+    "pp_ctx_tickets": (_i, [_p, C.POINTER(_i), C.POINTER(_i)]),
     "pp_row_block_list": (_i, [_p, _p, _i, _i, _i, _p, _p]),
     "pp_positive_row_blocks": (_i, [_p, _p, _i, _i, _p, _p]),
     "pp_row_block_dilate": (_i, [_p, _p, _p, _p]),
diff --git a/pyrapose_amd/csrc/conv3.hip b/pyrapose_amd/csrc/conv3.hip
--- a/pyrapose_amd/csrc/conv3.hip
+++ b/pyrapose_amd/csrc/conv3.hip
@@ -154,13 +154,70 @@
   epilogue3<TM, TN, OP>(p, acc, smem, m0, n0, tid, wm, wn, il, h, g_bias, g_addend, g_mask, g_out, g_ohi, g_olo);
 }
 
-template <int TM, int TN, bool AP, bool OP, bool SC = false, bool RL = false>
+__device__ __forceinline__ bool arrive_last(int* __restrict__ counter, int n, volatile int* flag_lds, int tid) {
+  asm volatile("s_waitcnt vmcnt(0)" ::: "memory");
+  __syncthreads();
+  if (tid == 0) {
+    __builtin_amdgcn_fence(__ATOMIC_RELEASE, "agent");
+    asm volatile("s_waitcnt vmcnt(0)" ::: "memory");
+    const int t = __hip_atomic_fetch_add(counter, 1, __ATOMIC_RELAXED, __HIP_MEMORY_SCOPE_AGENT);
+    const int last = t == n - 1;
+    if (last) {
+      __hip_atomic_store(counter, 0, __ATOMIC_RELAXED, __HIP_MEMORY_SCOPE_AGENT);
+      __builtin_amdgcn_fence(__ATOMIC_ACQUIRE, "agent");
+      asm volatile("s_waitcnt vmcnt(0)" ::: "memory");
+    }
+    *flag_lds = last;
+  }
+  __syncthreads();
+  return *flag_lds != 0;
+}
+
+__device__ __forceinline__ void finish4(const IgemmParams& p, float4 v, long long mo, int co, bool with_addend, const float* __restrict__ g_addend,
+                                        const float* __restrict__ g_mask, float* __restrict__ g_out, void* __restrict__ g_ohi,
+                                        void* __restrict__ g_olo);
+
+template <int KIND, int BM, int BN>
+__device__ __forceinline__ void splitk_combine_tile(const IgemmParams& p, int splits, const float* g_ws, long long slice, int* __restrict__ g_tk,
+                                                    int tile, volatile int* flag_lds, int tid, int m0, int n0, const int* rl_blk,
+                                                    const float* __restrict__ g_bias, const float* __restrict__ g_addend,
+                                                    const float* __restrict__ g_mask, float* __restrict__ g_out, void* g_ohi, void* g_olo) {
+  if (!arrive_last(g_tk + tile, splits, flag_lds, tid)) return;
+  constexpr int N4 = BN / 4;
+  const int nout4 = (p.Nout + 3) & ~3;
+#pragma unroll
+  for (int j = 0; j < BM / 32; ++j) {
+    const int blk0 = KIND == 2 ? rl_blk[j] : 0;
+    for (int i = tid; i < 32 * N4; i += 256) {
+      const int r = 32 * j + i / N4, co = n0 + 4 * (i % N4);
+      long long mo = (long long)m0 + r, srow = mo;
+      bool ok = co < nout4;
+      if (KIND == 1) {
+        ok = ok && r >= 1 && r <= BM - 2;
+        srow = mo - p.m_off;
+      }
+      if (KIND == 2) mo = (long long)blk0 + (r & 31);
+      if (!ok || mo >= p.M) continue;
+      const float* w = g_ws + srow * p.ld_out + co;
+      float4 v = *reinterpret_cast<const float4*>(w);
+      for (int s = 1; s < splits; ++s) {
+        const float4 q = *reinterpret_cast<const float4*>(w + s * slice);
+        v.x += q.x; v.y += q.y; v.z += q.z; v.w += q.w;
+      }
+      if (g_bias) { const float4 b = *reinterpret_cast<const float4*>(g_bias + co); v.x += b.x; v.y += b.y; v.z += b.z; v.w += b.w; }
+      finish4(p, v, mo, co, true, g_addend, g_mask, g_out, g_ohi, g_olo);
+    }
+  }
+}
+
+template <int TM, int TN, bool AP, bool OP, bool SC = false, bool RL = false, bool IF = false>
 __global__ __launch_bounds__(256, (TM * TN >= 8) ? 2 : ((TM * TN == 4) ? 3 : 4)) void igemm3f_kernel(
     const IgemmParams p, const void* __restrict__ g_a0, const void* __restrict__ g_a1, unsigned a_bytes,
     const void* __restrict__ g_whi, const void* __restrict__ g_wlo, unsigned w_bytes,
     const float* __restrict__ g_bias, const float* __restrict__ g_addend, const float* __restrict__ g_mask,
     float* __restrict__ g_out, uint2* __restrict__ g_ohi, uint2* __restrict__ g_olo, int w_rows, int w_ld8, int splits,
-    float* __restrict__ g_ws, const int* __restrict__ g_rl = nullptr, const unsigned char* __restrict__ g_srcflags = nullptr) {
+    float* __restrict__ g_ws, const int* __restrict__ g_rl = nullptr, const unsigned char* __restrict__ g_srcflags = nullptr,
+    int* __restrict__ g_tk = nullptr) {
   constexpr int BM = 64 * TM, BN = 64 * TN, BK = 32, NO = BK / 8;
   constexpr int SMEM_U4 = 2 * NO * (BM + BN);
   constexpr int ES = 4;
@@ -318,7 +375,8 @@
     __syncthreads();
   }
   if (splits > 1) {
-    float* slice = g_ws + (long long)split * (RL ? (((long long)p.M + 31) & ~31ll) : (long long)p.M) * p.ld_out;
+    const long long slice_elems = (RL ? (((long long)p.M + 31) & ~31ll) : (long long)p.M) * p.ld_out;
+    float* slice = g_ws + (long long)split * slice_elems;
 #pragma unroll
     for (int a = 0; a < TM; ++a)
 #pragma unroll
@@ -332,18 +390,21 @@
           if (row_ok && co < ((p.Nout + 3) & ~3)) slice[(long long)m * p.ld_out + co] = acc[a][b][r];
         }
       }
+    if constexpr (IF)
+      splitk_combine_tile<RL ? 2 : 0, BM, BN>(p, splits, g_ws, slice_elems, g_tk, lb, reinterpret_cast<volatile int*>(smem), tid, m0, n0, rl_blk,
+                                              g_bias, g_addend, g_mask, g_out, g_ohi, g_olo);
     return;
   }
-  epilogue3<TM, TN, OP, PP_EPI_GF, SC, false, RL>(p, acc, smem, m0, n0, tid, wm, wn, il, h, g_bias, g_addend, g_mask, g_out, g_ohi, g_olo, rl_blk);
-}
-
-template <int TM, int TN, bool CAP, bool AP = false, bool OP = false>
+  if constexpr (!IF) epilogue3<TM, TN, OP, PP_EPI_GF, SC, false, RL>(p, acc, smem, m0, n0, tid, wm, wn, il, h, g_bias, g_addend, g_mask, g_out, g_ohi, g_olo, rl_blk);
+}
+
+template <int TM, int TN, bool CAP, bool AP = false, bool OP = false, bool IF = false>
 __global__ __launch_bounds__(256, (TM * TN >= 8) ? 2 : ((TM * TN == 4) ? 3 : 4)) void igemm3x_kernel(
     const IgemmParams p, const void* __restrict__ g_a, const void* __restrict__ g_a1, unsigned a_bytes, const void* __restrict__ g_whi,
     const void* __restrict__ g_wlo, unsigned w_bytes, const float* __restrict__ g_bias, const float* __restrict__ g_addend,
     const float* __restrict__ g_mask, float* __restrict__ g_out, uint2* __restrict__ g_ohi, uint2* __restrict__ g_olo, int w_rows, int w_ld8,
     int splits, float* __restrict__ g_ws, void* __restrict__ g_chi, void* __restrict__ g_clo, const unsigned char* __restrict__ g_flags,
-    int skip_halo) {
+    int skip_halo, int* __restrict__ g_tk = nullptr) {
   static_assert(!(CAP && AP), "split capture is for f32 operands");
   constexpr int ES = 4;
   constexpr int BM = 64 * TM, BN = 64 * TN, BK = 32, NO = BK / 8;
@@ -565,7 +626,8 @@
     __syncthreads();
   }
   if (splits > 1) {
-    float* slice = g_ws + (long long)split * (p.M - p.m_off) * p.ld_out;
+    const long long slice_elems = (long long)(p.M - p.m_off) * p.ld_out;
+    float* slice = g_ws + (long long)split * slice_elems;
 #pragma unroll
     for (int a = 0; a < TM; ++a)
 #pragma unroll
@@ -578,9 +640,12 @@
           if (row >= 1 && row <= BM - 2 && m < p.M && co < ((p.Nout + 3) & ~3)) slice[(long long)(m - p.m_off) * p.ld_out + co] = acc[a][b][r];
         }
       }
+    if constexpr (IF)
+      splitk_combine_tile<1, BM, BN>(p, splits, g_ws, slice_elems, g_tk, lb, reinterpret_cast<volatile int*>(smem), tid, m0, n0, nullptr, g_bias,
+                                     g_addend, g_mask, g_out, g_ohi, g_olo);
     return;
   }
-  epilogue3<TM, TN, OP, 4, false, true>(p, acc, smem, m0, n0, tid, wm, wn, il, h, g_bias, g_addend, g_mask, g_out, g_ohi, g_olo);
+  if constexpr (!IF) epilogue3<TM, TN, OP, 4, false, true>(p, acc, smem, m0, n0, tid, wm, wn, il, h, g_bias, g_addend, g_mask, g_out, g_ohi, g_olo);
 }
 
 template <bool OP, int VAR = 0, int NWM = 4>
@@ -786,15 +851,19 @@
   if (g_ohi) planes_st4(g_ohi, g_olo, (mo * p.ld_out + co) >> 2, v);
 }
 
-__global__ void class_fill_kernel(const IgemmParams p, const float* __restrict__ g_addend, const float* __restrict__ g_mask,
+struct ClassGeo {
+  int M[3], OH[3], OW[3], cy[3], cx[3];
+};
+__global__ void class_fill_kernel(const IgemmParams p, const ClassGeo g, const float* __restrict__ g_addend, const float* __restrict__ g_mask,
                                   float* __restrict__ g_out, void* __restrict__ g_ohi, void* __restrict__ g_olo) {
+  const int c = blockIdx.y;
   const int n4 = (p.Nout + 3) >> 2;
-  const long long total = (long long)p.M * n4;
-  const int hw = p.seg[0].OH * p.seg[0].OW;
+  const long long total = (long long)g.M[c] * n4;
+  const int OW = g.OW[c], hw = g.OH[c] * OW, cy = g.cy[c], cx = g.cx[c];
   for (long long i = blockIdx.x * (long long)blockDim.x + threadIdx.x; i < total; i += (long long)gridDim.x * blockDim.x) {
     const int m = (int)(i / n4), co = 4 * (int)(i - (long long)m * n4);
-    const int n = m / hw, rem = m - n * hw, yq = rem / p.seg[0].OW, xq = rem - yq * p.seg[0].OW;
-    const long long mo = (long long)(n * p.sc_H + 2 * yq + p.sc_cy) * p.sc_W + 2 * xq + p.sc_cx;
+    const int n = m / hw, rem = m - n * hw, yq = rem / OW, xq = rem - yq * OW;
+    const long long mo = (long long)(n * p.sc_H + 2 * yq + cy) * p.sc_W + 2 * xq + cx;
     finish4(p, make_float4(0.f, 0.f, 0.f, 0.f), mo, co, true, g_addend, g_mask, g_out, g_ohi, g_olo);
   }
 }
@@ -867,43 +936,11 @@
   }
 }
 
-__global__ void row_block_flags_kernel(const float* __restrict__ x, int rows, int ld, int cols4, unsigned char* __restrict__ flags) {
-  const int blk = blockIdx.x, r0 = blk * 32;
-  const int nr = rows - r0 < 32 ? rows - r0 : 32;
-  int any = 0;
-  for (int i = threadIdx.x; i < nr * cols4; i += blockDim.x) {
-    const int r = i / cols4, c = i - r * cols4;
-    const float4 v = *reinterpret_cast<const float4*>(x + (long long)(r0 + r) * ld + 4 * c);
-    any |= (v.x != 0.f) | (v.y != 0.f) | (v.z != 0.f) | (v.w != 0.f);
-  }
-  any = __syncthreads_or(any);
-  if (threadIdx.x == 0) flags[blk] = any ? 1 : 0;
-}
-
-__global__ void row_block_flags_planes_kernel(const uint2* __restrict__ hi, const uint2* __restrict__ lo, int rows, int ld4, int cols4,
-                                              unsigned char* __restrict__ flags, const unsigned char* __restrict__ within) {
-  const int blk = blockIdx.x, r0 = blk * 32;
-  if (within && !within[blk]) {
-    if (threadIdx.x == 0) flags[blk] = 0;
-    return;
-  }
-  const int nr = rows - r0 < 32 ? rows - r0 : 32;
-  int any = 0;
-  for (int i = threadIdx.x; i < nr * cols4; i += blockDim.x) {
-    const int r = i / cols4, c = i - r * cols4;
-    const long long o = pk4((long long)(r0 + r) * ld4 + c);
-    const uint2 h = hi[o], l = lo[o];
-    any |= fmt_any_nonzero(h.x | h.y, l.x | l.y) ? 1 : 0;
-  }
-  any = __syncthreads_or(any);
-  if (threadIdx.x == 0) flags[blk] = any ? 1 : 0;
-}
-
-__global__ void row_block_compact_kernel(const unsigned char* __restrict__ flags, int n_blocks, int* __restrict__ list) {
-  __shared__ int wave_cnt[4];
-  __shared__ int base;
+__device__ __forceinline__ void compact_blocks(const unsigned char* flags, int n_blocks, int* __restrict__ list, int* sh) {
+  int* wave_cnt = sh;
+  int* base = sh + 4;
   const int tid = threadIdx.x, lane = tid & 63, wave = tid >> 6;
-  if (tid == 0) base = 0;
+  if (tid == 0) *base = 0;
   __syncthreads();
   for (int i0 = 0; i0 < n_blocks; i0 += 256) {
     const int i = i0 + tid;
@@ -912,14 +949,61 @@
     const int before = __popcll(m & ((1ull << lane) - 1ull));
     if (lane == 0) wave_cnt[wave] = __popcll(m);
     __syncthreads();
-    int off = base;
+    int off = *base;
     for (int w = 0; w < wave; ++w) off += wave_cnt[w];
     if (f) list[1 + off + before] = i;
     __syncthreads();
-    if (tid == 0) base += wave_cnt[0] + wave_cnt[1] + wave_cnt[2] + wave_cnt[3];
+    if (tid == 0) *base += wave_cnt[0] + wave_cnt[1] + wave_cnt[2] + wave_cnt[3];
     __syncthreads();
   }
-  if (tid == 0) list[0] = base;
+  if (tid == 0) list[0] = *base;
+}
+
+__global__ void row_block_flags_kernel(const float* __restrict__ x, int rows, int ld, int cols4, unsigned char* flags, int* __restrict__ g_tk,
+                                       int* __restrict__ list) {
+  __shared__ int sh[8];
+  const int blk = blockIdx.x, r0 = blk * 32;
+  const int nr = rows - r0 < 32 ? rows - r0 : 32;
+  int any = 0;
+  for (int i = threadIdx.x; i < nr * cols4; i += blockDim.x) {
+    const int r = i / cols4, c = i - r * cols4;
+    const float4 v = *reinterpret_cast<const float4*>(x + (long long)(r0 + r) * ld + 4 * c);
+    any |= (v.x != 0.f) | (v.y != 0.f) | (v.z != 0.f) | (v.w != 0.f);
+  }
+  any = __syncthreads_or(any);
+  if (threadIdx.x == 0) flags[blk] = any ? 1 : 0;
+  if (g_tk && arrive_last(g_tk, (int)gridDim.x, sh + 5, (int)threadIdx.x)) compact_blocks(flags, (int)gridDim.x, list, sh);
+}
+
+__global__ void row_block_flags_planes_kernel(const uint2* __restrict__ hi, const uint2* __restrict__ lo, int rows, int ld4, int cols4,
+                                              unsigned char* flags, const unsigned char* __restrict__ within, int* __restrict__ g_tk,
+                                              int* __restrict__ list) {
+  __shared__ int sh[8];
+  const int blk = blockIdx.x, r0 = blk * 32;
+  int any = 0;
+  if (!(within && !within[blk])) {
+    const int nr = rows - r0 < 32 ? rows - r0 : 32;
+    for (int i = threadIdx.x; i < nr * cols4; i += blockDim.x) {
+      const int r = i / cols4, c = i - r * cols4;
+      const long long o = pk4((long long)(r0 + r) * ld4 + c);
+      const uint2 h = hi[o], l = lo[o];
+      any |= fmt_any_nonzero(h.x | h.y, l.x | l.y) ? 1 : 0;
+    }
+    any = __syncthreads_or(any);
+  }
+  if (threadIdx.x == 0) flags[blk] = any ? 1 : 0;
+  if (g_tk && arrive_last(g_tk, (int)gridDim.x, sh + 5, (int)threadIdx.x)) compact_blocks(flags, (int)gridDim.x, list, sh);
+}
+
+__global__ void row_block_compact_kernel(const unsigned char* __restrict__ flags, int n_blocks, int* __restrict__ list) {
+  __shared__ int sh[8];
+  compact_blocks(flags, n_blocks, list, sh);
+}
+
+static int* inline_tickets(pp_ctx* ctx, long long n) {
+  const char* const e = getenv("PP_CONV3_INLINE_FINISH");
+  if (e && e[0] == '0') return nullptr;
+  return pp_tickets(ctx, n);
 }
 
 }
@@ -929,8 +1013,9 @@
                "pp_row_block_list: bad tensor (ld %% 4 == 0, 16-byte aligned)");
   const int nb = (rows + 31) / 32, cols4 = (cols + 3) / 4;
   PP_CHECK_ARG(ctx, 4 * cols4 <= ld, PP_ERR_SHAPE, "pp_row_block_list: cols rounded up to 4 exceed ld");
-  hipLaunchKernelGGL(row_block_flags_kernel, dim3((unsigned)nb), dim3(256), 0, ctx->stream, x, rows, ld, cols4, flags);
-  hipLaunchKernelGGL(row_block_compact_kernel, dim3(1), dim3(256), 0, ctx->stream, (const unsigned char*)flags, nb, list);
+  int* const tk = inline_tickets(ctx, 1);
+  hipLaunchKernelGGL(row_block_flags_kernel, dim3((unsigned)nb), dim3(256), 0, ctx->stream, x, rows, ld, cols4, flags, tk, list);
+  if (!tk) hipLaunchKernelGGL(row_block_compact_kernel, dim3(1), dim3(256), 0, ctx->stream, (const unsigned char*)flags, nb, list);
   PP_CHECK_LAUNCH(ctx, "pp_row_block_list");
   return PP_OK;
 }
@@ -955,9 +1040,10 @@
                "pp_row_block_list_planes: bad tensor (ld %% 8 == 0, packed planes)");
   const int nb = (rows + 31) / 32, cols4 = (cols + 3) / 4;
   PP_CHECK_ARG(ctx, 4 * cols4 <= ld, PP_ERR_SHAPE, "pp_row_block_list_planes: cols rounded up to 4 exceed ld");
+  int* const tk = inline_tickets(ctx, 1);
   hipLaunchKernelGGL(row_block_flags_planes_kernel, dim3((unsigned)nb), dim3(256), 0, ctx->stream, (const uint2*)x_hi, (const uint2*)x_lo, rows,
-                     ld / 4, cols4, flags, within);
-  hipLaunchKernelGGL(row_block_compact_kernel, dim3(1), dim3(256), 0, ctx->stream, (const unsigned char*)flags, nb, list);
+                     ld / 4, cols4, flags, within, tk, list);
+  if (!tk) hipLaunchKernelGGL(row_block_compact_kernel, dim3(1), dim3(256), 0, ctx->stream, (const unsigned char*)flags, nb, list);
   PP_CHECK_LAUNCH(ctx, "pp_row_block_list_planes");
   return PP_OK;
 }
@@ -1106,13 +1192,13 @@
   return same;
 }
 
-__global__ void rl_dilate_kernel(const IgemmParams p, const unsigned char* __restrict__ in_flags, unsigned char* __restrict__ out_flags,
-                                 int n_blocks) {
+__global__ void rl_dilate_kernel(const IgemmParams p, const unsigned char* __restrict__ in_flags, unsigned char* out_flags, int n_blocks,
+                                 int* __restrict__ g_tk = nullptr, int* __restrict__ list = nullptr) {
+  __shared__ int sh[8];
   const int b = blockIdx.x * blockDim.x + threadIdx.x;
-  if (b >= n_blocks) return;
   const int r_lo = 32 * b, r_hi = min(32 * b + 31, p.M - 1);
   int any = 0;
-  for (int s = 0; s < p.n_seg; ++s) {
+  for (int s = 0; s < p.n_seg && b < n_blocks; ++s) {
     const int seg_lo = p.seg[s].row_begin, seg_hi = (s + 1 < p.n_seg ? p.seg[s + 1].row_begin : p.M) - 1;
     if (r_hi < seg_lo || r_lo > seg_hi) continue;
     const int W = p.seg[s].OW;
@@ -1123,7 +1209,8 @@
       for (int q = lo >> 5; q <= (hi >> 5); ++q) any |= in_flags[q];
     }
   }
-  out_flags[b] = any ? 1 : 0;
+  if (b < n_blocks) out_flags[b] = any ? 1 : 0;
+  if (g_tk && arrive_last(g_tk, (int)gridDim.x, sh + 5, (int)threadIdx.x)) compact_blocks(out_flags, n_blocks, list, sh);
 }
 
 __global__ void rl_fill_kernel(const IgemmParams p, const unsigned char* __restrict__ live, const float* __restrict__ g_addend,
@@ -1180,15 +1267,14 @@
   }
 }
 
-__global__ void row_block_compact_kernel(const unsigned char* __restrict__ flags, int n_blocks, int* __restrict__ list);
-
 template <int TM, int TN>
 static void launch_igemm3_rowlist(hipStream_t st, IgemmParams& p, const void* ahi, const void* alo, const void* whi, const void* wlo, int w_rows,
                                   int w_ld8, void* ohi, void* olo, const unsigned char* dy_flags, unsigned char* out_flags, int* out_list,
-                                  float* ws, size_t ws_bytes, bool fill = true) {
+                                  float* ws, size_t ws_bytes, bool fill = true, int* tk = nullptr) {
   constexpr int BM = 64 * TM, BN = 64 * TN;
   const int nb = (p.M + 31) / 32;
-  static const int want_splits = []() { const char* e = getenv("PP_SPARSE_DGRAD_SPLITS"); return e ? atoi(e) : 2; }();
+  const char* const e_splits = getenv("PP_SPARSE_DGRAD_SPLITS");
+  const int want_splits = e_splits ? atoi(e_splits) : 2;
   const int n_steps = p.kh * p.kw * (p.Cred / 32);
   int splits = 1;
   if (ws && want_splits > 1 && (ohi || p.out)) {
@@ -1196,25 +1282,31 @@
     splits = want_splits;
     while (splits > 1 && (n_steps / splits < 24 || slice_bytes * splits > (long long)ws_bytes)) --splits;
   }
-  if (dy_flags) hipLaunchKernelGGL(rl_dilate_kernel, dim3((unsigned)((nb + 255) / 256)), dim3(256), 0, st, p, dy_flags, out_flags, nb);
-  hipLaunchKernelGGL(row_block_compact_kernel, dim3(1), dim3(256), 0, st, (const unsigned char*)out_flags, nb, out_list);
+  if (dy_flags) hipLaunchKernelGGL(rl_dilate_kernel, dim3((unsigned)((nb + 255) / 256)), dim3(256), 0, st, p, dy_flags, out_flags, nb, tk, out_list);
+  if (!dy_flags || !tk) hipLaunchKernelGGL(row_block_compact_kernel, dim3(1), dim3(256), 0, st, (const unsigned char*)out_flags, nb, out_list);
   p.n_tiles_n = (p.Nout + BN - 1) / BN;
   const int n_tiles_m = (nb + BM / 32 - 1) / (BM / 32);
   const long long a_bytes = p.src_rows * (long long)p.ld_src * 4, w_bytes = (long long)p.w_taps * w_rows * w_ld8 * 16;
   const dim3 grid((unsigned)(n_tiles_m * p.n_tiles_n * splits));
-  if (ahi && !ohi)
-    hipLaunchKernelGGL((igemm3f_kernel<TM, TN, true, false, false, true>), grid, dim3(256), 0, st, p, ahi, alo, (unsigned)a_bytes, whi, wlo,
-                       (unsigned)w_bytes, p.bias, p.addend, p.mask_src, p.out, (uint2*)nullptr, (uint2*)nullptr, w_rows, w_ld8, splits,
-                       splits > 1 ? ws : (float*)nullptr, (const int*)out_list, dy_flags);
-  else if (ahi)
-    hipLaunchKernelGGL((igemm3f_kernel<TM, TN, true, true, false, true>), grid, dim3(256), 0, st, p, ahi, alo, (unsigned)a_bytes, whi, wlo,
-                       (unsigned)w_bytes, p.bias, p.addend, p.mask_src, p.out, (uint2*)ohi, (uint2*)olo, w_rows, w_ld8, splits,
-                       splits > 1 ? ws : (float*)nullptr, (const int*)out_list, dy_flags);
-  else
-    hipLaunchKernelGGL((igemm3f_kernel<TM, TN, false, false, false, true>), grid, dim3(256), 0, st, p, (const void*)p.src, nullptr,
-                       (unsigned)a_bytes, whi, wlo, (unsigned)w_bytes, p.bias, p.addend, p.mask_src, p.out, (uint2*)nullptr, (uint2*)nullptr,
-                       w_rows, w_ld8, splits, splits > 1 ? ws : (float*)nullptr, (const int*)out_list, dy_flags);
-  if (splits > 1)
+  float* const ws_arg = splits > 1 ? ws : (float*)nullptr;
+  auto go = [&](auto inl) {
+    constexpr bool IF = decltype(inl)::value;
+    if (ahi && !ohi)
+      hipLaunchKernelGGL((igemm3f_kernel<TM, TN, true, false, false, true, IF>), grid, dim3(256), 0, st, p, ahi, alo, (unsigned)a_bytes, whi, wlo,
+                         (unsigned)w_bytes, p.bias, p.addend, p.mask_src, p.out, (uint2*)nullptr, (uint2*)nullptr, w_rows, w_ld8, splits, ws_arg,
+                         (const int*)out_list, dy_flags, tk);
+    else if (ahi)
+      hipLaunchKernelGGL((igemm3f_kernel<TM, TN, true, !IF, false, true, IF>), grid, dim3(256), 0, st, p, ahi, alo, (unsigned)a_bytes, whi, wlo,
+                         (unsigned)w_bytes, p.bias, p.addend, p.mask_src, p.out, (uint2*)ohi, (uint2*)olo, w_rows, w_ld8, splits, ws_arg,
+                         (const int*)out_list, dy_flags, tk);
+    else
+      hipLaunchKernelGGL((igemm3f_kernel<TM, TN, false, false, false, true, IF>), grid, dim3(256), 0, st, p, (const void*)p.src, nullptr,
+                         (unsigned)a_bytes, whi, wlo, (unsigned)w_bytes, p.bias, p.addend, p.mask_src, p.out, (uint2*)nullptr, (uint2*)nullptr,
+                         w_rows, w_ld8, splits, ws_arg, (const int*)out_list, dy_flags, tk);
+  };
+  if (splits > 1 && tk) go(std::true_type{});
+  else go(std::false_type{});
+  if (splits > 1 && !tk)
     hipLaunchKernelGGL(rl_splitk_finish_kernel, dim3((unsigned)nb), dim3(256), 0, st, p, splits, (const float*)ws, (const int*)out_list, p.bias,
                        p.addend, p.mask_src, p.out, ohi, olo);
   const bool in_place = (ohi != nullptr && p.add_hi == (const void*)ohi && p.ld_add == p.ld_out && !p.out && !p.addend && !p.mask_hi &&
@@ -1233,10 +1325,12 @@
 }
 
 template <int TM, int TN>
-static void launch_igemm3(hipStream_t st, IgemmParams& p, const void* ahi, const void* alo, const void* whi, const void* wlo, int w_rows,
+static bool launch_igemm3(hipStream_t st, IgemmParams& p, const void* ahi, const void* alo, const void* whi, const void* wlo, int w_rows,
                           int w_ld8, void* ohi, void* olo, int splits, float* ws, void* chi = nullptr, void* clo = nullptr,
-                          const unsigned char* flags = nullptr, float* ws_any = nullptr, size_t ws_any_bytes = 0, int n_cu = 256) {
+                          const unsigned char* flags = nullptr, float* ws_any = nullptr, size_t ws_any_bytes = 0, int n_cu = 256,
+                          int* tk = nullptr) {
   constexpr int BM = 64 * TM, BN = 64 * TN;
+  const bool inl = splits > 1 && tk != nullptr;
   p.n_tiles_n = (p.Nout + BN - 1) / BN;
   const int n_tiles_m = (p.M + BM - 1) / BM;
   const dim3 grid((unsigned)(n_tiles_m * p.n_tiles_n * splits));
@@ -1251,7 +1345,7 @@
       hipLaunchKernelGGL((igemm3f_kernel<TM, TN, false, false, true>), grid, dim3(256), 0, st, p, (const void*)p.src, nullptr, (unsigned)a_bytes,
                          whi, wlo, (unsigned)w_bytes, p.bias, p.addend, p.mask_src, p.out, (uint2*)nullptr, (uint2*)nullptr, w_rows, w_ld8, 1,
                          nullptr);
-    return;
+    return false;
   }
   {
     if (igemm3x_ok(p, ahi != nullptr, ohi != nullptr, w_rows, w_ld8) && (TM <= 2 || (ahi != nullptr && !chi))) {
@@ -1264,10 +1358,15 @@
       const bool op = ohi != nullptr && splits == 1;
       if constexpr (TM <= 2) {
         if (chi) {
-          hipLaunchKernelGGL((igemm3x_kernel<TM, TN, true>), gridx, dim3(256), 0, st, p, (const void*)p.src, nullptr, (unsigned)a_bytes, whi, wlo,
-                             (unsigned)w_bytes, p.bias, p.addend, p.mask_src, p.out, (uint2*)nullptr, (uint2*)nullptr, w_rows, w_ld8, splits,
-                             ws, chi, clo, flags, skip_halo);
-          return;
+          if (inl)
+            hipLaunchKernelGGL((igemm3x_kernel<TM, TN, true, false, false, true>), gridx, dim3(256), 0, st, p, (const void*)p.src, nullptr,
+                               (unsigned)a_bytes, whi, wlo, (unsigned)w_bytes, p.bias, p.addend, p.mask_src, p.out, (uint2*)ohi, (uint2*)olo, w_rows,
+                               w_ld8, splits, ws, chi, clo, flags, skip_halo, tk);
+          else
+            hipLaunchKernelGGL((igemm3x_kernel<TM, TN, true>), gridx, dim3(256), 0, st, p, (const void*)p.src, nullptr, (unsigned)a_bytes, whi, wlo,
+                               (unsigned)w_bytes, p.bias, p.addend, p.mask_src, p.out, (uint2*)nullptr, (uint2*)nullptr, w_rows, w_ld8, splits,
+                               ws, chi, clo, flags, skip_halo);
+          return inl;
         }
       }
       if constexpr (TM == 2 && TN == 2) {
@@ -1318,16 +1417,22 @@
               q.m_off = full_rt * (BM4 - 2);
               const int rem = q.M - q.m_off;
               const int n_rt = (rem + BM - 3) / (BM - 2);
-              hipLaunchKernelGGL((igemm3x_kernel<TM, TN, false, true, false>), dim3((unsigned)(n_rt * ntn * tail_splits)), dim3(256), 0, st, q, ahi,
-                                 alo, (unsigned)a_bytes, whi, wlo, (unsigned)w_bytes, q.bias, q.addend, q.mask_src, q.out, (uint2*)nullptr,
-                                 (uint2*)nullptr, w_rows, w_ld8, tail_splits, ws_any, nullptr, nullptr, (const unsigned char*)nullptr, skip_halo);
-              const long long total = (long long)rem * ((q.Nout + 3) >> 2);
-              long long blocks = (total + 255) / 256;
-              if (blocks > (long long)n_cu * 8) blocks = (long long)n_cu * 8;
-              hipLaunchKernelGGL(splitk_finish_kernel, dim3((unsigned)blocks), dim3(256), 0, st, q, tail_splits, (const float*)ws_any, q.bias, q.addend,
-                                 q.mask_src, q.out, ohi, olo);
+              if (tk) {
+                hipLaunchKernelGGL((igemm3x_kernel<TM, TN, false, true, false, true>), dim3((unsigned)(n_rt * ntn * tail_splits)), dim3(256), 0, st, q,
+                                   ahi, alo, (unsigned)a_bytes, whi, wlo, (unsigned)w_bytes, q.bias, q.addend, q.mask_src, q.out, (uint2*)ohi,
+                                   (uint2*)olo, w_rows, w_ld8, tail_splits, ws_any, nullptr, nullptr, (const unsigned char*)nullptr, skip_halo, tk);
+              } else {
+                hipLaunchKernelGGL((igemm3x_kernel<TM, TN, false, true, false>), dim3((unsigned)(n_rt * ntn * tail_splits)), dim3(256), 0, st, q, ahi,
+                                   alo, (unsigned)a_bytes, whi, wlo, (unsigned)w_bytes, q.bias, q.addend, q.mask_src, q.out, (uint2*)nullptr,
+                                   (uint2*)nullptr, w_rows, w_ld8, tail_splits, ws_any, nullptr, nullptr, (const unsigned char*)nullptr, skip_halo);
+                const long long total = (long long)rem * ((q.Nout + 3) >> 2);
+                long long blocks = (total + 255) / 256;
+                if (blocks > (long long)n_cu * 8) blocks = (long long)n_cu * 8;
+                hipLaunchKernelGGL(splitk_finish_kernel, dim3((unsigned)blocks), dim3(256), 0, st, q, tail_splits, (const float*)ws_any, q.bias,
+                                   q.addend, q.mask_src, q.out, ohi, olo);
+              }
             }
-            return;
+            return false;
           }
           const char* const e_dma2 = getenv("PP_CONV3_DMA2");
           const bool dma2_on = e_dma2 && e_dma2[0] == '1';
@@ -1336,7 +1441,7 @@
             p.n_tiles_n = ntn;
             hipLaunchKernelGGL((igemm4x_kernel<true, 1, 2>), dim3((unsigned)(n_tiles_mx * ntn)), dim3(256), 0, st, p, ahi, alo, (unsigned)a_bytes, whi,
                                wlo, (unsigned)w_bytes, p.bias, p.addend, p.mask_src, p.out, (uint2*)ohi, (uint2*)olo, w_rows, w_ld8);
-            return;
+            return false;
           }
         }
       }
@@ -1344,12 +1449,20 @@
         hipLaunchKernelGGL((igemm3x_kernel<TM, TN, false, true, true>), gridx, dim3(256), 0, st, p, ahi, alo, (unsigned)a_bytes, whi, wlo,
                            (unsigned)w_bytes, p.bias, p.addend, p.mask_src, p.out, (uint2*)ohi, (uint2*)olo, w_rows, w_ld8, splits, ws, nullptr,
                            nullptr, flags, skip_halo);
+      else if (ahi && inl)
+        hipLaunchKernelGGL((igemm3x_kernel<TM, TN, false, true, false, true>), gridx, dim3(256), 0, st, p, ahi, alo, (unsigned)a_bytes, whi, wlo,
+                           (unsigned)w_bytes, p.bias, p.addend, p.mask_src, p.out, (uint2*)ohi, (uint2*)olo, w_rows, w_ld8, splits, ws, nullptr,
+                           nullptr, flags, skip_halo, tk);
       else if (ahi)
         hipLaunchKernelGGL((igemm3x_kernel<TM, TN, false, true, false>), gridx, dim3(256), 0, st, p, ahi, alo, (unsigned)a_bytes, whi, wlo,
                            (unsigned)w_bytes, p.bias, p.addend, p.mask_src, p.out, (uint2*)nullptr, (uint2*)nullptr, w_rows, w_ld8, splits, ws,
                            nullptr, nullptr, flags, skip_halo);
       else if constexpr (TM <= 2) {
-        if (op)
+        if (inl)
+          hipLaunchKernelGGL((igemm3x_kernel<TM, TN, false, false, false, true>), gridx, dim3(256), 0, st, p, (const void*)p.src, nullptr,
+                             (unsigned)a_bytes, whi, wlo, (unsigned)w_bytes, p.bias, p.addend, p.mask_src, p.out, (uint2*)ohi, (uint2*)olo,
+                             w_rows, w_ld8, splits, ws, nullptr, nullptr, flags, skip_halo, tk);
+        else if (op)
           hipLaunchKernelGGL((igemm3x_kernel<TM, TN, false, false, true>), gridx, dim3(256), 0, st, p, (const void*)p.src, nullptr,
                              (unsigned)a_bytes, whi, wlo, (unsigned)w_bytes, p.bias, p.addend, p.mask_src, p.out, (uint2*)ohi, (uint2*)olo,
                              w_rows, w_ld8, splits, ws, nullptr, nullptr, flags, skip_halo);
@@ -1358,13 +1471,22 @@
                              wlo, (unsigned)w_bytes, p.bias, p.addend, p.mask_src, p.out, (uint2*)nullptr, (uint2*)nullptr, w_rows, w_ld8, splits,
                              ws, nullptr, nullptr, flags, skip_halo);
       }
-      return;
+      return inl;
     }
   }
   if (chi) split_capture_pass(st, p, chi, clo);
+  void *const f_ohi = ohi, *const f_olo = olo;
   if (splits > 1) ohi = olo = nullptr;
   auto go = [&](auto ap, auto op) {
     constexpr bool AP = decltype(ap)::value, OP = decltype(op)::value;
+    if constexpr (!OP) {
+      if (fast && inl) {
+        hipLaunchKernelGGL((igemm3f_kernel<TM, TN, AP, false, false, false, true>), grid, dim3(256), 0, st, p, AP ? ahi : (const void*)p.src,
+                           AP ? alo : nullptr, (unsigned)a_bytes, whi, wlo, (unsigned)w_bytes, p.bias, p.addend, p.mask_src, p.out, (uint2*)f_ohi,
+                           (uint2*)f_olo, w_rows, w_ld8, splits, ws, (const int*)nullptr, (const unsigned char*)nullptr, tk);
+        return;
+      }
+    }
     if (fast)
       hipLaunchKernelGGL((igemm3f_kernel<TM, TN, AP, OP>), grid, dim3(256), 0, st, p, AP ? ahi : (const void*)p.src, AP ? alo : nullptr,
                          (unsigned)a_bytes, whi, wlo, (unsigned)w_bytes, p.bias, p.addend, p.mask_src, p.out, (uint2*)ohi, (uint2*)olo,
@@ -1378,6 +1500,7 @@
   else if (ahi) go(std::true_type{}, std::false_type{});
   else if (ohi) go(std::false_type{}, std::true_type{});
   else go(std::false_type{}, std::false_type{});
+  return inl && fast;
 }
 
 static void pick_tile3(const pp_ctx* ctx, int M, int Nout, int ld_out, int n_steps, bool may_split, bool x_ok, int* tm, int* tn, int* splits) {
@@ -1467,14 +1590,19 @@
     fprintf(stderr, "igemm3 M %d N %d steps %d -> tile %dx%d splits %d (may_split %d: ws %d planes_out %d out %d)\n", p.M, p.Nout, n_steps, 64 * tm,
             64 * tn, splits, (int)may_split, (int)(ctx->ws != nullptr), (int)(ohi != nullptr), (int)(p.out != nullptr));
   float* ws = splits > 1 ? ctx->ws : nullptr;
-  if (tm == 4) launch_igemm3<4, 2>(ctx->stream, p, ahi, alo, whi, wlo, w_rows, w_ld8, ohi, olo, splits, ws, chi, clo, flags);
+  int* const tk = ctx->ws != nullptr && !p.sc_on ? inline_tickets(ctx, (long long)((p.M + 61) / 62 + 1) * ((p.Nout + 63) / 64)) : nullptr;
+  const int n_cu = ctx->n_cu > 0 ? ctx->n_cu : 256;
+  bool done;
+  if (tm == 4) done = launch_igemm3<4, 2>(ctx->stream, p, ahi, alo, whi, wlo, w_rows, w_ld8, ohi, olo, splits, ws, chi, clo, flags, nullptr, 0, n_cu, tk);
   else if (tm == 2 && tn == 2)
-    launch_igemm3<2, 2>(ctx->stream, p, ahi, alo, whi, wlo, w_rows, w_ld8, ohi, olo, splits, ws, chi, clo, flags, ctx->ws, (size_t)ctx->ws_bytes,
-                        ctx->n_cu > 0 ? ctx->n_cu : 256);
-  else if (tm == 1 && tn == 2) launch_igemm3<1, 2>(ctx->stream, p, ahi, alo, whi, wlo, w_rows, w_ld8, ohi, olo, splits, ws, chi, clo, flags);
-  else if (tm == 2 && tn == 1) launch_igemm3<2, 1>(ctx->stream, p, ahi, alo, whi, wlo, w_rows, w_ld8, ohi, olo, splits, ws, chi, clo, flags);
-  else launch_igemm3<1, 1>(ctx->stream, p, ahi, alo, whi, wlo, w_rows, w_ld8, ohi, olo, splits, ws, chi, clo, flags);
-  if (splits > 1) {
+    done = launch_igemm3<2, 2>(ctx->stream, p, ahi, alo, whi, wlo, w_rows, w_ld8, ohi, olo, splits, ws, chi, clo, flags, ctx->ws, (size_t)ctx->ws_bytes,
+                               n_cu, tk);
+  else if (tm == 1 && tn == 2)
+    done = launch_igemm3<1, 2>(ctx->stream, p, ahi, alo, whi, wlo, w_rows, w_ld8, ohi, olo, splits, ws, chi, clo, flags, nullptr, 0, n_cu, tk);
+  else if (tm == 2 && tn == 1)
+    done = launch_igemm3<2, 1>(ctx->stream, p, ahi, alo, whi, wlo, w_rows, w_ld8, ohi, olo, splits, ws, chi, clo, flags, nullptr, 0, n_cu, tk);
+  else done = launch_igemm3<1, 1>(ctx->stream, p, ahi, alo, whi, wlo, w_rows, w_ld8, ohi, olo, splits, ws, chi, clo, flags, nullptr, 0, n_cu, tk);
+  if (splits > 1 && !done) {
     const long long total = (long long)p.M * ((p.Nout + 3) >> 2);
     long long blocks = (total + 255) / 256;
     const long long cap = (long long)(ctx->n_cu > 0 ? ctx->n_cu : 256) * 8;
@@ -1532,7 +1660,7 @@
     PP_CHECK_ARG(ctx, ok, PP_ERR_SHAPE, "pp_conv2d_nhwc_fwd_bf16x3: out_flags needs a 3x3 stride-1 'same' conv on plane-stored input");
     launch_igemm3_rowlist<2, 2>(ctx->stream, p, x_hi, x_lo, w_hi, w_lo, d->cout, d->cin / 8, y_hi, y_lo, nullptr,
                                 const_cast<unsigned char*>(opts->out_flags) , opts->out_list, ctx->ws,
-                                ctx->ws_bytes, false);
+                                ctx->ws_bytes, false, inline_tickets(ctx, (long long)((p.M + 63) / 64 + 1) * ((p.Nout + 127) / 128)));
     PP_CHECK_LAUNCH(ctx, "pp_conv2d_nhwc_fwd_bf16x3");
     return PP_OK;
   }
@@ -1677,6 +1805,19 @@
     }
     if (ok) {
       if (chi) split_capture_pass(ctx->stream, p, chi, clo);
+      const char* const e_one = getenv("PP_CONV3_INLINE_FINISH");
+      const bool one_fill = !(e_one && e_one[0] == '0');
+      ClassGeo geo = {};
+      const IgemmParams* fill_p = &q;
+      int n_fill = 0;
+      long long fill_blocks = 0;
+      auto fill = [&]() {
+        if (n_fill > 0)
+          hipLaunchKernelGGL(class_fill_kernel, dim3((unsigned)fill_blocks, (unsigned)n_fill), dim3(256), 0, ctx->stream, *fill_p, geo, addend, relu_src, dx,
+                             dx_hi, dx_lo);
+        n_fill = 0;
+        fill_blocks = 0;
+      };
       for (int c = 0; c < 4; ++c) {
         if (cls[c].M <= 0) continue;
         if (cls[c].kh > 0) {
@@ -1686,9 +1827,15 @@
           long long blocks = (total + 255) / 256;
           const long long cap = (long long)(ctx->n_cu > 0 ? ctx->n_cu : 256) * 8;
           if (blocks > cap) blocks = cap;
-          hipLaunchKernelGGL(class_fill_kernel, dim3((unsigned)blocks), dim3(256), 0, ctx->stream, cls[c], addend, relu_src, dx, dx_hi, dx_lo);
+          geo.M[n_fill] = cls[c].M; geo.OH[n_fill] = cls[c].seg[0].OH; geo.OW[n_fill] = cls[c].seg[0].OW;
+          geo.cy[n_fill] = c >> 1; geo.cx[n_fill] = c & 1;
+          fill_p = &cls[c];
+          ++n_fill;
+          fill_blocks = blocks > fill_blocks ? blocks : fill_blocks;
+          if (!one_fill) fill();
         }
       }
+      fill();
       PP_CHECK_LAUNCH(ctx, "pp_conv2d_nhwc_bwd_data_bf16x3");
       return PP_OK;
     }
@@ -1697,12 +1844,13 @@
     const int nb = (p.M + 31) / 32;
     unsigned char* out_flags = skip_flags + nb;
     int* out_list = opts->skip_list + nb + 1;
+    int* const tk = inline_tickets(ctx, (long long)((p.M + 63) / 64 + 1) * ((p.Nout + 127) / 128));
     if (rl_mode == 22)
       launch_igemm3_rowlist<2, 2>(ctx->stream, p, dy_hi, dy_lo, w_hi, w_lo, d->cin, cred / 8, dx_hi, dx_lo, skip_flags, out_flags, out_list, ctx->ws,
-                                  ctx->ws_bytes, !opts->lazy_out);
+                                  ctx->ws_bytes, !opts->lazy_out, tk);
     else
       launch_igemm3_rowlist<1, 2>(ctx->stream, p, dy_hi, dy_lo, w_hi, w_lo, d->cin, cred / 8, dx_hi, dx_lo, skip_flags, out_flags, out_list, ctx->ws,
-                                  ctx->ws_bytes, !opts->lazy_out);
+                                  ctx->ws_bytes, !opts->lazy_out, tk);
     PP_CHECK_LAUNCH(ctx, "pp_conv2d_nhwc_bwd_data_bf16x3");
     return PP_OK;
   }
diff --git a/pyrapose_amd/csrc/ctx.hip b/pyrapose_amd/csrc/ctx.hip
--- a/pyrapose_amd/csrc/ctx.hip
+++ b/pyrapose_amd/csrc/ctx.hip
@@ -28,7 +28,50 @@
   return PP_OK;
 }
 
-extern "C" void pp_ctx_destroy(pp_ctx* ctx) { free(ctx); }
+extern "C" void pp_ctx_destroy(pp_ctx* ctx) {
+  if (ctx && ctx->tickets) (void)hipFree(ctx->tickets);
+  free(ctx);
+}
+
+int* pp_tickets(pp_ctx* ctx, long long n) {
+  if (n <= ctx->n_tickets) return ctx->tickets;
+  if (n > (1ll << 24)) return nullptr;
+  long long cap = 16384;
+  while (cap < n) cap *= 2;
+  int* fresh = nullptr;
+  if (hipStreamSynchronize(ctx->stream) != hipSuccess || hipMalloc((void**)&fresh, (size_t)cap * sizeof(int)) != hipSuccess) {
+    (void)hipGetLastError();
+    return nullptr;
+  }
+  if (hipMemsetAsync(fresh, 0, (size_t)cap * sizeof(int), ctx->stream) != hipSuccess || hipStreamSynchronize(ctx->stream) != hipSuccess) {
+    (void)hipGetLastError();
+    (void)hipFree(fresh);
+    return nullptr;
+  }
+  if (ctx->tickets) (void)hipFree(ctx->tickets);
+  ctx->tickets = fresh;
+  ctx->n_tickets = (int)cap;
+  return fresh;
+}
+
+extern "C" int pp_ctx_tickets(pp_ctx* ctx, int* count, int* nonzero) {
+  PP_REQUIRE_CTX(ctx);
+  PP_CHECK_ARG(ctx, count && nonzero, PP_ERR_ARG, "pp_ctx_tickets: null argument");
+  *count = ctx->n_tickets;
+  *nonzero = 0;
+  if (ctx->n_tickets == 0) return PP_OK;
+  int* host = (int*)malloc((size_t)ctx->n_tickets * sizeof(int));
+  PP_CHECK_ARG(ctx, host != nullptr, PP_ERR_ARG, "pp_ctx_tickets: out of host memory");
+  hipError_t e = hipStreamSynchronize(ctx->stream);
+  if (e == hipSuccess) e = hipMemcpy(host, ctx->tickets, (size_t)ctx->n_tickets * sizeof(int), hipMemcpyDeviceToHost);
+  if (e != hipSuccess) {
+    free(host);
+    return pp_fail(ctx, (int)e, "pp_ctx_tickets: %s", hipGetErrorString(e));
+  }
+  for (int i = 0; i < ctx->n_tickets; ++i) *nonzero += host[i] != 0;
+  free(host);
+  return PP_OK;
+}
 
 extern "C" int pp_ctx_set_stream(pp_ctx* ctx, void* hip_stream) {
   PP_REQUIRE_CTX(ctx);
diff --git a/pyrapose_amd/csrc/pp_internal.h b/pyrapose_amd/csrc/pp_internal.h
--- a/pyrapose_amd/csrc/pp_internal.h
+++ b/pyrapose_amd/csrc/pp_internal.h
@@ -16,7 +16,11 @@
   size_t ws_bytes;
   int planes_fmt;
   const float* grad_scale;
+  int* tickets;
+  int n_tickets;
 };
+
+int* pp_tickets(pp_ctx* ctx, long long n);
 
 static inline int pp_fail(pp_ctx* ctx, int code, const char* fmt, ...) {
   if (ctx) {
diff --git a/pyrapose_amd/ops.py b/pyrapose_amd/ops.py
--- a/pyrapose_amd/ops.py
+++ b/pyrapose_amd/ops.py
@@ -183,6 +183,12 @@
 def set_grad_scale(ctx, scale2):
     ctx._grad_scale_keep = scale2
     check(lib.pp_ctx_set_grad_scale(ctx.handle, _ptr(scale2)), ctx.handle, "pp_ctx_set_grad_scale")
+
+
+def tickets(ctx):
+    n, nz = C.c_int(0), C.c_int(0)
+    check(lib.pp_ctx_tickets(ctx.handle, C.byref(n), C.byref(nz)), ctx.handle, "pp_ctx_tickets")
+    return n.value, nz.value
 
 
 def row_block_list(ctx, x, cols, flags=None, blocks=None):
```

Result: slower. 576.0 (-6.7%).
